# verdurin/pbdagcon

Measured on AMD Instinct MI355X. Metric: consensus bases/sec (whole node), higher is better.
Workload: dtype u8

## Files before the change

pbdagcon_amd/csrc/dagcon_api.hip:

```cpp
#include <hip/hip_runtime.h>
#include <algorithm>
#include <cstdarg>
#include <cstdio>
#include <cstdlib>
#include <cstring>
#include <string>
#include <chrono>
#include <array>
#include <vector>

#include "../../include/dagcon.h"
#include "dagcon_dev.h"
#include "k_build.hip.h"
#include "k_merge.hip.h"
#include "k_merge_q.hip.h"
#include "k_bestpath.hip.h"
#include "k_align.hip.h"
#include "k_align_panels.hip.h"
#include "k_place.hip.h"
#include "k_cigar.hip.h"
#include "k_rate.hip.h"
#include "k_cs.hip.h"

namespace {

struct DevBuf {
    void *p = nullptr;
    size_t cap = 0;
};

struct CigarBufs {
    DevBuf ops, op_begin, tile_begin, totals, ckpt;
    DevBuf q, t, q_off, t_base;
    DevBuf out_off;
    DevBuf piece, cut, wave_piece, wave_begin, piece_out;
    DevBuf rev, q_len;
    DevBuf rate_base, tile_rate, rate;
    std::array<DevBuf *, 20> all() {
        return {&ops, &op_begin, &tile_begin, &totals, &ckpt, &q, &t, &q_off, &t_base, &out_off, &piece, &cut, &wave_piece, &wave_begin, &piece_out, &rev, &q_len,
                &rate_base, &tile_rate, &rate};
    }
};
static_assert(sizeof(CigarBufs) == 20 * sizeof(DevBuf), "CigarBufs::all() must name every member");
struct CsBufs {
    DevBuf text, cs_off, cs_len, totals, n_ops, op_begin, t_base, t_room, q_off, q_len;
    std::array<DevBuf *, 10> all() { return {&text, &cs_off, &cs_len, &totals, &n_ops, &op_begin, &t_base, &t_room, &q_off, &q_len}; }
};
static_assert(sizeof(CsBufs) == 10 * sizeof(DevBuf), "CsBufs::all() must name every member");

#define DQ_KMAX 52u
struct DgPlanIn { uint32_t T; uint64_t n_alns, sum_bb; uint32_t gcuts, max_segments, min_segment_len, seg_env, merge_q; };
struct DgPlan { uint32_t seg_max, seg_min, use_q, bp_max; };
static DgPlan dg_plan_pieces(const DgPlanIn &in) {
    DgPlan pl;
    const uint32_t T = in.T;
    pl.seg_min = in.min_segment_len;
    if (!pl.seg_min) pl.seg_min = (uint32_t)std::min<uint64_t>(768, std::max<uint64_t>(192, in.sum_bb / 8192));
    if (in.max_segments) pl.seg_max = in.max_segments > 64u ? 64u : in.max_segments;
    else if (in.seg_env) pl.seg_max = in.seg_env;
    else if (in.gcuts) pl.seg_max = 64;
    else { uint32_t sm = T ? 8192u / T : 8u; pl.seg_max = sm < 8u ? 8u : sm > 256u ? 256u : sm; }
    if (in.gcuts && !in.min_segment_len) pl.seg_min = 256;
    pl.use_q = 0;
    if (in.merge_q && !in.gcuts && pl.seg_max != 1) {
        const uint32_t slots = 1024u * DQ_WAVES;
        if (in.max_segments || in.seg_env) pl.use_q = 1;
        else if (T && in.n_alns <= (uint64_t)DQ_KMAX * T) {
            const uint64_t avail = std::min<uint64_t>(256, std::max<uint64_t>(1, in.sum_bb / T / 128));
            const uint64_t k = (uint64_t)T * avail / DQ_ROWS / slots;
            if (k >= 1 || (uint64_t)T * avail / DQ_ROWS * 10u >= 6u * slots) {
                const uint64_t sm = std::min<uint64_t>(avail, std::max<uint64_t>(k, 1) * slots * DQ_ROWS / T);
                if (sm >= 2) { pl.seg_max = (uint32_t)sm; pl.use_q = 1; }
            }
        }
    }
    if (pl.seg_max < 1) pl.seg_max = 1;
    if (pl.use_q && !in.min_segment_len) pl.seg_min = 128;
    pl.bp_max = pl.seg_max == 1 ? 1u : std::min(in.gcuts || T >= 256u ? 64u : (uint32_t)DG_BP_PIECES, 3u * pl.seg_max);
    if (pl.bp_max < 1) pl.bp_max = 1;
    return pl;
}

struct Ctx {
    dagcon_opts opts;
    int device = 0;
    hipStream_t stream = nullptr;
    hipEvent_t ev[5] = {nullptr, nullptr, nullptr, nullptr, nullptr};
    std::string err;
    bool uploaded = false, ran = false, fetched = false;

    uint32_t T = 0, A = 0;
    int bp_lane = 1, bl_stk = -1;
    uint32_t align_dropped = 0;
    uint32_t align_n = 0;
    std::vector<uint32_t> h_ends;
    int poison = 0;
    int fold = 1;
    int merge_q = 1, use_q = 0;
    uint32_t max_k = 0, max_tlen = 0;
    uint64_t sum_len = 0, sum_bb = 0, mat_cells = 0, blob_bytes = 0;
    bool have_bb = false;
    std::vector<uint32_t> h_tlen, h_aln_len, h_aln_start, h_aln_tgt;
    std::vector<uint64_t> h_aln_begin, h_aln_off, h_mat_base, h_bbv_base, h_bb_off, h_matc_base;
    std::vector<uint32_t> h_matc_stride;
    uint64_t matc_cells = 0;
    std::vector<uint8_t> h_tactive;
    std::vector<uint32_t> h_ch_base, h_ch_aln;
    std::vector<uint64_t> h_norm_off;
    std::vector<uint32_t> h_ck_base;
    uint64_t n_ckpt = 0;
    uint32_t emit_shift = 9;
    uint32_t n_chunks = 0;
    uint64_t tmp_main = 0, tmp_cap = 0;

    DevBuf d_tfail, d_q, d_t, d_aln_off, d_aln_len, d_aln_start, d_aln_tgt, d_tlen, d_aln_begin, d_tactive,
        d_bb, d_bb_off, d_mat_base, d_bbv_base, d_matc_base, d_matc_stride;
    DevBuf d_nmis, d_norm_off, d_n_lo, d_n_hi, d_n_start, d_n_ins, d_n_del, d_norm;
    DevBuf d_ch_aln, d_ch_base, d_ch_k0, d_ch_next, d_ch_w, d_ch_tb, d_ch_flag, d_ch_src, d_ch_out, d_ch_adv,
        d_n_lb, d_norm_tmp, d_ckpt, d_ck_base;
    DevBuf d_node_base, d_n_nodes, d_pool_base, d_pool_size, d_pool_top, d_t_nins;
    DevBuf d_matA, d_matD, d_matC, d_cov, d_gcount, d_gbase, d_bid;
    DevBuf d_nodes, d_best, d_queue, d_score, d_cns_tmp, d_bp_tt, d_score_b;
    DevBuf d_pool, d_stk, d_cuts, d_cuts_bp, d_bp_stat, d_bp_len, d_worklist, d_rd, d_pro_state, d_sh_cnt, d_seg_done, d_wl_first, d_queue0, d_bp_end, d_bp_ab, d_defer, d_cns_tmp0;
    DevBuf d_al[15];
    DevBuf d_pn[18];
    DevBuf d_pl[14];
    CsBufs cs;
    CigarBufs cg;
    std::vector<uint8_t> h_cig_bad;
    std::string cig_err;
    bool filter_on = false;
    dagcon_record_filter filter = {1000000u, 0u};
    bool rs_valid = false;
    std::vector<uint32_t> rs_match, rs_mismatch, rs_ins, rs_del;
    std::vector<uint8_t> rs_fate;
    DevBuf d_cns, d_cns_off, d_cns_len, d_seg_first, d_n_seg, d_seg_r0, d_seg_r1, d_st;
    DevBuf d_pos_tmp, d_pos_tmp0, d_pos;
    DevBuf d_sup_tmp, d_sup_tmp0, d_sup;

    uint64_t norm_cap = 0, node_cap = 0, pool_cap = 0, cns_cap = 0, seg_cap = 0;
    uint32_t stk_words = 4096, growth_pct = 100, seg_max = 8, bp_max = 16, seg_env = 0, seg_min = 768;
    uint32_t sh_log = 16;
    bool full_span = false;
    uint32_t gcuts = 1;
    uint32_t worklist_cap = 0, list_grid = 8192;

    DgStatus h_st;
    dagcon_timings tm;

    std::vector<uint64_t> r_seg_begin, r_seq_off, r_cns_off, r_seg_first;
    std::vector<int32_t> r_range0, r_range1, r_tmp0, r_tmp1;
    std::vector<uint32_t> r_seq_len, r_cns_len, r_n_seg, r_tfail;
    std::vector<int32_t> r_status;
    char *r_blob = nullptr;
    size_t r_blob_cap = 0;
    uint16_t *r_sup = nullptr;
    size_t r_sup_cap = 0;
    uint64_t r_sup_n = 0;
    std::vector<uint32_t> r_pos;
    bool pos_valid = false;
    bool sup_valid = false;

    std::vector<uint8_t> g_base, g_deleted, g_backbone;
    std::vector<int32_t> g_weight, g_cov, g_bbpos, g_out_dst, g_out_cnt, g_in_src;
    std::vector<uint32_t> g_out_begin, g_in_begin;
};

int fail(Ctx *c, int code, const char *fmt, ...) {
    char buf[512];
    va_list ap;
    va_start(ap, fmt);
    vsnprintf(buf, sizeof buf, fmt, ap);
    va_end(ap);
    if (c) c->err = buf;
    return code;
}

#define HIPCHK(c, call)                                                                    \
    do {                                                                                   \
        hipError_t _e = (call);                                                            \
        if (_e != hipSuccess)                                                              \
            return fail((c), DAGCON_ERR_HIP, "%s failed: %s (%s:%d)", #call,               \
                        hipGetErrorString(_e), __FILE__, __LINE__);                        \
    } while (0)

int ensure(Ctx *c, DevBuf &b, size_t bytes) {
    if (bytes == 0) bytes = 16;
    if (b.cap >= bytes) return DAGCON_OK;
    if (b.p) { (void)hipFree(b.p); b.p = nullptr; b.cap = 0; }
    size_t want = bytes + bytes / 16 + 256;
    const bool dbg = getenv("DAGCON_ALLOC_TIMING") != nullptr;
    const double t0 = dbg ? std::chrono::duration<double>(std::chrono::steady_clock::now().time_since_epoch()).count() : 0;
    hipError_t e = hipMalloc(&b.p, want);
    if (dbg) {
        const double dt = std::chrono::duration<double>(std::chrono::steady_clock::now().time_since_epoch()).count() - t0;
        if (dt > 0.005) fprintf(stderr, "dagcon: hipMalloc(%.1f MB) took %.1f ms\n", want / 1e6, dt * 1e3);
    }
    if (e != hipSuccess) {
        b.p = nullptr;
        return fail(c, DAGCON_ERR_WORKSPACE, "hipMalloc(%zu bytes) failed: %s", want, hipGetErrorString(e));
    }
    b.cap = want;
    return DAGCON_OK;
}

#define ENSURE(c, buf, bytes)                                \
    do {                                                     \
        int _r = ensure((c), (buf), (size_t)(bytes));        \
        if (_r != DAGCON_OK) return _r;                      \
    } while (0)

template <typename T>
int upload_vec(Ctx *c, DevBuf &b, const std::vector<T> &v) {
    ENSURE(c, b, v.size() * sizeof(T));
    if (!v.empty()) HIPCHK(c, hipMemcpyAsync(b.p, v.data(), v.size() * sizeof(T), hipMemcpyHostToDevice, c->stream));
    return DAGCON_OK;
}

void free_buf(DevBuf &b) {
    if (b.p) (void)hipFree(b.p);
    b.p = nullptr; b.cap = 0;
}

int ensure_arenas(Ctx *c) {
    ENSURE(c, c->d_norm, c->norm_cap * sizeof(uint16_t));
    ENSURE(c, c->d_nodes, c->node_cap * sizeof(DgNode));
    ENSURE(c, c->d_best, c->node_cap * 4);
    ENSURE(c, c->d_queue, c->node_cap * 4);
    ENSURE(c, c->d_score, c->node_cap * 8);
    ENSURE(c, c->d_bp_tt, c->node_cap * 4);
    if (c->gcuts) ENSURE(c, c->d_score_b, c->node_cap * 4);
    ENSURE(c, c->d_cns_tmp, c->node_cap);
    ENSURE(c, c->d_pool, c->pool_cap * 4);
    ENSURE(c, c->d_stk, std::max<uint64_t>((uint64_t)c->T * std::max(c->bp_max, c->seg_max), c->gcuts ? c->list_grid : 0) * c->stk_words * 4);
    if (c->gcuts) {
        ENSURE(c, c->d_worklist, (4ull + 3ull * c->worklist_cap) * 4);
        ENSURE(c, c->d_rd, (uint64_t)c->A * 16 + 16);
        ENSURE(c, c->d_pro_state, (uint64_t)c->T * 16 + 16);
        ENSURE(c, c->d_sh_cnt, (uint64_t)c->T * (2 + 2 * DG_SH_MAX) * 4 + 16);
        ENSURE(c, c->d_seg_done, (uint64_t)c->worklist_cap * (DG_SH_MAX + 1) * 4 + 16);
        ENSURE(c, c->d_wl_first, (uint64_t)c->T * 4 + 16);
        ENSURE(c, c->d_queue0, c->node_cap * 4);
        ENSURE(c, c->d_bp_end, (uint64_t)c->T * c->bp_max * 4 + 16);
        ENSURE(c, c->d_bp_ab, (uint64_t)c->T * c->bp_max * 16 + 16);
        ENSURE(c, c->d_defer, (uint64_t)c->T * (DG_DEFER_MAX + 1) * 4 + 16);
        ENSURE(c, c->d_cns_tmp0, c->node_cap);
    }
    ENSURE(c, c->d_cuts, (uint64_t)c->T * (c->seg_max + 2) * 4);
    ENSURE(c, c->d_cuts_bp, (uint64_t)c->T * (c->bp_max + 2) * 4);
    ENSURE(c, c->d_bp_stat, (uint64_t)c->T * c->bp_max * 8);
    ENSURE(c, c->d_bp_len, (uint64_t)c->T * c->bp_max * 4);
    ENSURE(c, c->d_cns, c->cns_cap);
    if (c->opts.flags & DAGCON_FLAG_BASE_SUPPORT) {
        ENSURE(c, c->d_sup_tmp, c->node_cap * 4);
        if (c->gcuts) ENSURE(c, c->d_sup_tmp0, c->node_cap * 4);
        ENSURE(c, c->d_sup, c->cns_cap * 4);
    }
    if (c->opts.flags & DAGCON_FLAG_BASE_POS) {
        ENSURE(c, c->d_pos_tmp, c->node_cap * 4);
        if (c->gcuts) ENSURE(c, c->d_pos_tmp0, c->node_cap * 4);
        ENSURE(c, c->d_pos, c->cns_cap * 4);
    }
    ENSURE(c, c->d_seg_r0, c->seg_cap * 4);
    ENSURE(c, c->d_seg_r1, c->seg_cap * 4);
    return DAGCON_OK;
}

void fill_params(Ctx *c, DgParams &p) {
    memset(&p, 0, sizeof p);
    p.q = (const uint8_t *)c->d_q.p; p.t = (const uint8_t *)c->d_t.p;
    p.aln_off = (const uint64_t *)c->d_aln_off.p;
    p.aln_len = (const uint32_t *)c->d_aln_len.p;
    p.aln_start = (const uint32_t *)c->d_aln_start.p;
    p.aln_tgt = (const uint32_t *)c->d_aln_tgt.p;
    p.tlen = (const uint32_t *)c->d_tlen.p;
    p.aln_begin = (const uint64_t *)c->d_aln_begin.p;
    p.tactive = (const uint8_t *)c->d_tactive.p; p.tfail = (uint32_t *)c->d_tfail.p;
    p.bb = c->have_bb ? (const uint8_t *)c->d_bb.p : nullptr;
    p.bb_off = (const uint64_t *)c->d_bb_off.p;
    p.mat_base = (const uint64_t *)c->d_mat_base.p;
    p.matc_base = (const uint64_t *)c->d_matc_base.p; p.matc_stride = (const uint32_t *)c->d_matc_stride.p;
    p.bbv_base = (const uint64_t *)c->d_bbv_base.p;
    p.T = c->T; p.A = c->A;
    p.trim = c->opts.trim; p.min_len = c->opts.min_len;
    p.min_weight = c->opts.min_weight < 0 ? (int32_t)c->opts.min_cov : c->opts.min_weight;
    p.flags = c->opts.flags;
    p.max_k = c->max_k; p.max_tlen = c->max_tlen;
    p.nmis = (uint32_t *)c->d_nmis.p; p.norm_off = (uint64_t *)c->d_norm_off.p;
    p.n_lo = (uint32_t *)c->d_n_lo.p; p.n_hi = (uint32_t *)c->d_n_hi.p;
    p.n_start = (uint32_t *)c->d_n_start.p; p.n_ins = (uint32_t *)c->d_n_ins.p;
    p.n_del = (uint32_t *)c->d_n_del.p;
    p.norm = (uint16_t *)c->d_norm.p; p.norm_cap = c->norm_cap;
    p.ch_aln = (const uint32_t *)c->d_ch_aln.p; p.ch_base = (const uint32_t *)c->d_ch_base.p;
    p.n_chunks = c->n_chunks;
    p.ch_k0 = (uint32_t *)c->d_ch_k0.p; p.ch_next = (uint32_t *)c->d_ch_next.p;
    p.ch_w = (uint32_t *)c->d_ch_w.p; p.ch_tb = (uint32_t *)c->d_ch_tb.p;
    p.ch_flag = (uint32_t *)c->d_ch_flag.p; p.ch_src = (uint64_t *)c->d_ch_src.p;
    p.ch_out = (uint32_t *)c->d_ch_out.p; p.ch_adv = (uint32_t *)c->d_ch_adv.p;
    p.n_lb = (uint32_t *)c->d_n_lb.p; p.norm_tmp = (uint16_t *)c->d_norm_tmp.p;
    p.tmp_main = c->tmp_main; p.tmp_cap = c->tmp_cap;
    p.ckpt = (uint32_t *)c->d_ckpt.p; p.ck_base = (const uint32_t *)c->d_ck_base.p; p.emit_shift = c->emit_shift;
    p.node_base = (uint64_t *)c->d_node_base.p; p.n_nodes = (uint32_t *)c->d_n_nodes.p;
    p.pool_base = (uint64_t *)c->d_pool_base.p; p.pool_size = (uint32_t *)c->d_pool_size.p;
    p.pool_top = (uint32_t *)c->d_pool_top.p; p.t_nins = (uint32_t *)c->d_t_nins.p;
    p.matA = (uint32_t *)c->d_matA.p; p.matD = (uint32_t *)c->d_matD.p; p.matC = (uint32_t *)c->d_matC.p;
    p.cov = (int32_t *)c->d_cov.p; p.gcount = (uint32_t *)c->d_gcount.p;
    p.gbase = (uint32_t *)c->d_gbase.p; p.bid = (uint32_t *)c->d_bid.p;
    p.nodes = (DgNode *)c->d_nodes.p; p.best = (int32_t *)c->d_best.p;
    p.queue = (int32_t *)c->d_queue.p; p.score = (float2 *)c->d_score.p; p.bp_tt = (float *)c->d_bp_tt.p;
    p.cns_tmp = (uint8_t *)c->d_cns_tmp.p; p.node_cap = c->node_cap;
    p.pool = (uint32_t *)c->d_pool.p; p.pool_cap = c->pool_cap;
    p.stk = (int32_t *)c->d_stk.p; p.stk_words = c->stk_words; p.growth_pct = c->growth_pct;
    p.score_b = (float *)c->d_score_b.p;
    p.bp_lane = c->bp_lane >= 2 || (c->bp_lane && (uint64_t)c->T * c->bp_max >= 32768ull) ? 1u : 0u; p.bl_stk = c->bl_stk >= 0 && c->bl_stk < DG_BL_STK ? (uint32_t)c->bl_stk : (uint32_t)DG_BL_STK;
    p.emit_scan = c->max_k <= 64u ? 1u : 0u;
    p.fold = (c->fold && !(c->opts.flags & DAGCON_FLAG_STOP_AFTER_BUILD)) ? 1u : 0u;
    p.q_kmax = c->use_q && !c->opts.max_segments && !c->seg_env && c->max_k > DQ_KMAX ? DQ_KMAX : 0u;
    p.bp_seg_min = (c->seg_min + 2u) / 3u;
    p.seg_max = c->seg_max; p.seg_min = c->seg_min; p.cuts = (uint32_t *)c->d_cuts.p; p.bp_max = c->bp_max; p.cuts_bp = (uint32_t *)c->d_cuts_bp.p; p.bp_stat = (float *)c->d_bp_stat.p; p.bp_len = (uint32_t *)c->d_bp_len.p;
    p.gcuts = c->gcuts; p.sh_log = c->sh_log;
    p.rd_s = (uint32_t *)c->d_rd.p; p.rd_e = p.rd_s + c->A; p.rd_lead = p.rd_e + c->A; p.rd_trail = p.rd_lead + c->A;
    p.pro_state = (uint32_t *)c->d_pro_state.p; p.sh_cnt = (uint32_t *)c->d_sh_cnt.p;
    p.queue0 = (int32_t *)c->d_queue0.p; p.bp_end = (uint32_t *)c->d_bp_end.p; p.bp_ab = (float *)c->d_bp_ab.p;
    p.defer = (uint32_t *)c->d_defer.p; p.cns_tmp0 = (uint8_t *)c->d_cns_tmp0.p;
    p.seg_done = (uint32_t *)c->d_seg_done.p; p.wl_first = (uint32_t *)c->d_wl_first.p;
    p.worklist = (uint32_t *)c->d_worklist.p; p.worklist_cap = c->worklist_cap;
    p.cns = (uint8_t *)c->d_cns.p; p.cns_cap = c->cns_cap;
    p.cns_off = (uint64_t *)c->d_cns_off.p; p.cns_len = (uint32_t *)c->d_cns_len.p;
    p.seg_first = (uint64_t *)c->d_seg_first.p; p.n_seg = (uint32_t *)c->d_n_seg.p;
    p.seg_r0 = (int32_t *)c->d_seg_r0.p; p.seg_r1 = (int32_t *)c->d_seg_r1.p;
    p.seg_cap = c->seg_cap;
    p.st = (DgStatus *)c->d_st.p;
    if (c->opts.flags & DAGCON_FLAG_BASE_SUPPORT) {
        p.sup_tmp = (uint32_t *)c->d_sup_tmp.p; p.sup_tmp0 = (uint32_t *)c->d_sup_tmp0.p;
        p.sup_w = (uint16_t *)c->d_sup.p; p.sup_d = p.sup_w + c->cns_cap;
    }
    if (c->opts.flags & DAGCON_FLAG_BASE_POS) {
        p.pos_tmp = (uint32_t *)c->d_pos_tmp.p; p.pos_tmp0 = (uint32_t *)c->d_pos_tmp0.p; p.pos_out = (uint32_t *)c->d_pos.p;
    }
}

void launch_normalize(Ctx *c, const DgParams &p) {
    hipStream_t s = c->stream;
    if (c->A == 0) return;
    (void)hipMemsetAsync(c->d_ckpt.p, 0xFF, c->n_ckpt * 4, s);
    hipLaunchKernelGGL((k_norm_chunk<DG_NW, 64, false>), dim3((c->n_chunks + 63) / 64), dim3(64), 0, s, p);
    hipLaunchKernelGGL((k_norm_chunk<DG_NW_BIG, 32, true>), dim3((c->n_chunks + 31) / 32), dim3(32), 0, s, p);
    hipLaunchKernelGGL(k_norm_scan, dim3((c->A + 63) / 64), dim3(64), 0, s, p);
    hipLaunchKernelGGL(k_norm_finish2, dim3((c->n_chunks + 3) / 4), dim3(256), 0, s, p);
    hipLaunchKernelGGL(k_normalize_slow, dim3((c->A + 63) / 64), dim3(64), 0, s, p);
}

int launch_all(Ctx *c) {
    int r = ensure_arenas(c);
    if (r != DAGCON_OK) return r;
    DgParams p;
    fill_params(c, p);
    hipStream_t s = c->stream;
    if (c->poison & 8) {
        DevBuf *work[] = {&c->d_nmis, &c->d_n_lo, &c->d_n_hi, &c->d_n_start, &c->d_n_ins, &c->d_n_del, &c->d_ch_k0, &c->d_ch_next, &c->d_ch_w,
                          &c->d_ch_tb, &c->d_ch_flag, &c->d_ch_src, &c->d_ch_out, &c->d_ch_adv, &c->d_n_lb, &c->d_norm_tmp, &c->d_ckpt,
                          &c->d_node_base, &c->d_n_nodes, &c->d_pool_base, &c->d_pool_size, &c->d_pool_top, &c->d_t_nins, &c->d_cov, &c->d_gcount,
                          &c->d_gbase, &c->d_bid, &c->d_best, &c->d_queue, &c->d_score, &c->d_cns_tmp, &c->d_bp_tt, &c->d_stk, &c->d_cuts,
                          &c->d_cuts_bp, &c->d_bp_stat, &c->d_bp_len, &c->d_rd, &c->d_pro_state, &c->d_sh_cnt, &c->d_wl_first,
                          &c->d_queue0, &c->d_bp_end, &c->d_bp_ab, &c->d_defer, &c->d_cns_tmp0, &c->d_cns, &c->d_cns_off, &c->d_seg_first,
                          &c->d_seg_r0, &c->d_seg_r1, &c->d_worklist, &c->d_seg_done, &c->d_sup_tmp, &c->d_sup_tmp0, &c->d_sup, &c->d_pos_tmp, &c->d_pos_tmp0, &c->d_pos};
        for (DevBuf *b : work)
            if (b->p && b->cap) HIPCHK(c, hipMemsetAsync(b->p, 0xEE, b->cap, s));
    }
    HIPCHK(c, hipMemsetAsync(c->d_st.p, 0, sizeof(DgStatus), s));
    HIPCHK(c, hipMemsetAsync(c->d_tfail.p, 0, (size_t)c->T * 4 + 4, s));
    HIPCHK(c, hipMemsetAsync(c->d_cns_len.p, 0, (size_t)c->T * 4, s));
    HIPCHK(c, hipMemsetAsync(c->d_n_seg.p, 0, (size_t)c->T * 4, s));
    if (c->matc_cells) HIPCHK(c, hipMemsetAsync(c->d_matC.p, 0, c->matc_cells * 4, s));
    if (c->poison) {
        if ((c->poison & 1) && c->d_matA.p) { HIPCHK(c, hipMemsetAsync(c->d_matA.p, 0xEE, c->d_matA.cap, s)); HIPCHK(c, hipMemsetAsync(c->d_matD.p, 0xEE, c->d_matD.cap, s)); }
        if ((c->poison & 2) && c->d_nodes.p) { HIPCHK(c, hipMemsetAsync(c->d_nodes.p, 0xEE, c->d_nodes.cap, s)); HIPCHK(c, hipMemsetAsync(c->d_pool.p, 0xEE, c->d_pool.cap, s)); }
        if ((c->poison & 4) && c->d_score_b.p) HIPCHK(c, hipMemsetAsync(c->d_score_b.p, 0xEE, c->d_score_b.cap, s));
        if ((c->poison & 4) && c->d_norm.p) HIPCHK(c, hipMemsetAsync(c->d_norm.p, 0xEE, c->d_norm.cap, s));
    }
    HIPCHK(c, hipEventRecord(c->ev[0], s));
    launch_normalize(c, p);
    HIPCHK(c, hipEventRecord(c->ev[1], s));
    hipLaunchKernelGGL(k_carve, dim3(1), dim3(1024), 0, s, p);
    if (c->T > 0) {
        const uint32_t rows4 = (c->max_tlen + 2 + 4 * DG_LPW - 1) / (4 * DG_LPW);
        if (c->gcuts && c->A > 0) hipLaunchKernelGGL(k_readspan, dim3((c->A + 63) / 64), dim3(64), 0, s, p);
        if (p.emit_scan) hipLaunchKernelGGL(k_gsum, dim3(c->T, (c->max_tlen + 2 + 255) / 256), dim3(256), 0, s, p);
        else hipLaunchKernelGGL(k_groups, dim3(c->T, (c->max_tlen + 2 + 31) / 32), dim3(256), 0, s, p);
        hipLaunchKernelGGL(k_gscan, dim3(c->T), dim3(1024), 0, s, p);
        if (c->A > 0)
            hipLaunchKernelGGL(k_emit, dim3(c->T, (c->max_k + DG_ERPW - 1) / DG_ERPW, ((c->max_tlen + 2) >> c->emit_shift) + 1),
                               dim3(64), 0, s, p);
        const size_t lds = (size_t)4 * 2 * (c->max_k + 2) * sizeof(int32_t);
        if (lds > 65536)
            HIPCHK(c, hipFuncSetAttribute((const void *)k_lists, hipFuncAttributeMaxDynamicSharedMemorySize, (int)lds));
        hipLaunchKernelGGL(k_lists, dim3(c->T, rows4), dim3(256), lds, s, p);
    }
    HIPCHK(c, hipEventRecord(c->ev[2], s));
    if (c->T > 0 && !(c->opts.flags & DAGCON_FLAG_STOP_AFTER_BUILD)) {
        if (c->gcuts) {
            HIPCHK(c, hipMemsetAsync(c->d_worklist.p, 0, 16, s));
            HIPCHK(c, hipMemsetAsync(c->d_seg_done.p, 0, (size_t)c->worklist_cap * (DG_SH_MAX + 1) * 4, s));
            hipLaunchKernelGGL(k_merge_pro, dim3(c->T), dim3(64), 0, s, p);
            hipLaunchKernelGGL(k_cuts2, dim3(c->T), dim3(64), 0, s, p);
            hipLaunchKernelGGL(k_merge_list, dim3(c->list_grid), dim3(64), 0, s, p);
            hipLaunchKernelGGL(k_merge_fin, dim3(c->T), dim3(64), 0, s, p);
        } else {
            hipLaunchKernelGGL(k_cuts, dim3(c->T), dim3(64), 0, s, p);
            if (c->use_q) {
                hipLaunchKernelGGL(k_merge_q, dim3((c->T * c->seg_max + DQ_ROWS - 1u) / DQ_ROWS), dim3(64), 0, s, p);
                if (p.q_kmax) hipLaunchKernelGGL(k_merge, dim3(c->T * c->seg_max), dim3(64), 0, s, p);
            } else hipLaunchKernelGGL(k_merge, dim3(c->T * c->seg_max), dim3(64), 0, s, p);
        }
    }
    HIPCHK(c, hipEventRecord(c->ev[3], s));
    if (c->T > 0 && !(c->opts.flags & (DAGCON_FLAG_STOP_AFTER_BUILD | DAGCON_FLAG_STOP_AFTER_MERGE))) {
        const bool sup = (c->opts.flags & DAGCON_FLAG_BASE_SUPPORT) != 0;
        const bool pos = (c->opts.flags & DAGCON_FLAG_BASE_POS) != 0;
#define DG_BP_LAUNCH(K, GRID)                                                                          \
        do {                                                                                           \
            if (sup && pos) hipLaunchKernelGGL((K<true, true>), GRID, dim3(64), 0, s, p);              \
            else if (sup) hipLaunchKernelGGL((K<true, false>), GRID, dim3(64), 0, s, p);               \
            else if (pos) hipLaunchKernelGGL((K<false, true>), GRID, dim3(64), 0, s, p);               \
            else hipLaunchKernelGGL((K<false, false>), GRID, dim3(64), 0, s, p);                       \
        } while (0)
        hipLaunchKernelGGL(k_bp_terms, dim3(c->T, 16), dim3(256), 0, s, p);
        if (c->gcuts) {
            hipLaunchKernelGGL(k_bp_xtree, dim3(c->T), dim3(64), 0, s, p);
            hipLaunchKernelGGL(k_bp_sweep_ab, dim3(c->T * c->bp_max), dim3(64), 0, s, p);
            hipLaunchKernelGGL(k_bp_comb, dim3(c->T), dim3(64), 0, s, p);
            hipLaunchKernelGGL(k_bp_abs, dim3(c->T * c->bp_max), dim3(256), 0, s, p);
            hipLaunchKernelGGL(k_bp_choose, dim3(c->T * c->bp_max), dim3(256), 0, s, p);
            hipLaunchKernelGGL(k_bp_sweep_abs_g, dim3(c->T * c->bp_max), dim3(64), 0, s, p);
            hipLaunchKernelGGL(k_bp_defer, dim3(c->T), dim3(64), 0, s, p);
            DG_BP_LAUNCH(k_bp_walk_g, dim3(c->T * c->bp_max));
        } else {
            if (p.bp_lane) hipLaunchKernelGGL(k_bp_sweep_l, dim3((c->T * c->bp_max + 7u) / 8u), dim3(64), 0, s, p);
            hipLaunchKernelGGL(k_bp_sweep, dim3(c->T * c->bp_max), dim3(64), 0, s, p);
            hipLaunchKernelGGL(k_bp_check, dim3(c->T), dim3(64), 0, s, p);
            if (p.bp_lane) DG_BP_LAUNCH(k_bp_walk_r, dim3((c->T * c->bp_max + 7u) / 8u));
            else DG_BP_LAUNCH(k_bp_walk, dim3(c->T * c->bp_max));
        }
        DG_BP_LAUNCH(k_bp_join, dim3(c->T));
#undef DG_BP_LAUNCH
    }
    HIPCHK(c, hipEventRecord(c->ev[4], s));
    HIPCHK(c, hipGetLastError());
    return DAGCON_OK;
}

}

extern "C" {

int dagcon_abi_version(void) { return DAGCON_ABI_VERSION; }

void dagcon_default_opts(dagcon_opts *o) {
    if (!o) return;
    memset(o, 0, sizeof *o);
    o->min_cov = 6; o->min_len = 500; o->trim = 50; o->min_weight = -1; o->device = 0; o->flags = 0;
}

const char *dagcon_last_error(const dagcon_ctx *ctx) {
    return ctx ? reinterpret_cast<const Ctx *>(ctx)->err.c_str() : "null context";
}

int dagcon_create(const dagcon_opts *opts, dagcon_ctx **out) {
    if (!opts || !out) return DAGCON_ERR_INVALID_ARG;
    *out = nullptr;
    int ndev = 0;
    if (hipGetDeviceCount(&ndev) != hipSuccess || ndev <= 0) return DAGCON_ERR_NO_DEVICE;
    if (opts->device < 0 || opts->device >= ndev) return DAGCON_ERR_NO_DEVICE;
    if (opts->flags & ~DAGCON_FLAGS_ALL) return DAGCON_ERR_UNSUPPORTED;
    {
        hipDeviceProp_t prop;
        if (hipGetDeviceProperties(&prop, opts->device) != hipSuccess || strncmp(prop.gcnArchName, "gfx950", 6) != 0)
            return DAGCON_ERR_NO_DEVICE;
    }
    Ctx *c = new Ctx();
    c->opts = *opts;
    c->device = opts->device;
    if (const char *e = getenv("DAGCON_EMIT_SHIFT")) {
        const int v = atoi(e);
        if (v >= 4 && v <= 20) c->emit_shift = (uint32_t)v;
    }
    if (const char *e = getenv("DAGCON_MERGE_SEGS")) {
        const int v = atoi(e);
        if (v >= 1 && v <= 64) c->seg_env = (uint32_t)v;
    }
    if (const char *e = getenv("DAGCON_FOLD")) c->fold = atoi(e) != 0;
    if (const char *e = getenv("DAGCON_POISON")) c->poison = atoi(e);
    if (const char *e = getenv("DAGCON_BP_LANE")) c->bp_lane = atoi(e);
    if (const char *e = getenv("DAGCON_BP_LANE_STACK")) c->bl_stk = atoi(e);
    if (const char *e = getenv("DAGCON_MERGE_Q")) c->merge_q = atoi(e) != 0;
    memset(&c->tm, 0, sizeof c->tm);
    memset(&c->h_st, 0, sizeof c->h_st);
    if (hipSetDevice(c->device) != hipSuccess || hipStreamCreateWithFlags(&c->stream, hipStreamNonBlocking) != hipSuccess) {
        delete c;
        return DAGCON_ERR_NO_DEVICE;
    }
    for (auto &e : c->ev)
        if (hipEventCreate(&e) != hipSuccess) { delete c; return DAGCON_ERR_HIP; }
    if (ensure(c, c->d_st, sizeof(DgStatus)) != DAGCON_OK) { delete c; return DAGCON_ERR_WORKSPACE; }
    *out = reinterpret_cast<dagcon_ctx *>(c);
    return DAGCON_OK;
}

void dagcon_destroy(dagcon_ctx *ctx) {
    if (!ctx) return;
    Ctx *c = reinterpret_cast<Ctx *>(ctx);
    (void)hipSetDevice(c->device);
    if (c->stream) (void)hipStreamSynchronize(c->stream);
    if (c->r_blob) (void)hipHostFree(c->r_blob);
    if (c->r_sup) (void)hipHostFree(c->r_sup);
    DevBuf *all[] = {&c->d_q, &c->d_t, &c->d_aln_off, &c->d_aln_len, &c->d_aln_start, &c->d_aln_tgt,
                     &c->d_tlen, &c->d_aln_begin, &c->d_tactive, &c->d_tfail, &c->d_bb, &c->d_bb_off, &c->d_mat_base, &c->d_matc_base, &c->d_matc_stride,
                     &c->d_bbv_base, &c->d_nmis, &c->d_norm_off, &c->d_n_lo, &c->d_n_hi, &c->d_n_start, &c->d_ch_aln, &c->d_ch_base, &c->d_ch_k0, &c->d_ch_next, &c->d_ch_w, &c->d_ch_tb, &c->d_ch_flag, &c->d_ch_src, &c->d_ch_out, &c->d_ch_adv, &c->d_n_lb, &c->d_norm_tmp, &c->d_ckpt, &c->d_ck_base,
                     &c->d_n_ins, &c->d_n_del, &c->d_norm, &c->d_node_base, &c->d_n_nodes,
                     &c->d_pool_base, &c->d_pool_size, &c->d_pool_top, &c->d_t_nins, &c->d_matA, &c->d_matD,
                     &c->d_matC, &c->d_cov, &c->d_gcount, &c->d_gbase, &c->d_bid, &c->d_nodes,
                     &c->d_best, &c->d_queue, &c->d_score, &c->d_cns_tmp, &c->d_bp_tt, &c->d_score_b, &c->d_pool, &c->d_stk, &c->d_cuts, &c->d_cuts_bp, &c->d_bp_stat, &c->d_bp_len, &c->d_worklist, &c->d_rd, &c->d_pro_state, &c->d_sh_cnt, &c->d_seg_done, &c->d_wl_first, &c->d_queue0, &c->d_bp_end, &c->d_bp_ab, &c->d_defer, &c->d_cns_tmp0, &c->d_cns,
                     &c->d_cns_off, &c->d_cns_len, &c->d_seg_first, &c->d_n_seg, &c->d_seg_r0, &c->d_seg_r1,
                     &c->d_st, &c->d_sup_tmp, &c->d_sup_tmp0, &c->d_sup, &c->d_pos_tmp, &c->d_pos_tmp0, &c->d_pos};
    for (DevBuf *b : all) free_buf(*b);
    for (DevBuf &b : c->d_al) free_buf(b);
    for (DevBuf &b : c->d_pn) free_buf(b);
    for (DevBuf &b : c->d_pl) free_buf(b);
    for (DevBuf *b : c->cg.all()) free_buf(*b);
    for (DevBuf *b : c->cs.all()) free_buf(*b);
    for (auto &e : c->ev) if (e) (void)hipEventDestroy(e);
    if (c->stream) (void)hipStreamDestroy(c->stream);
    delete c;
}

static int upload_impl(dagcon_ctx *ctx, const dagcon_batch *b, const void *dev_q, const void *dev_t) {
    if (!ctx || !b) return DAGCON_ERR_INVALID_ARG;
    Ctx *c = reinterpret_cast<Ctx *>(ctx);
    c->uploaded = c->ran = c->fetched = false;
    c->sup_valid = c->pos_valid = false;
    c->h_cig_bad.clear();
    c->rs_valid = false;
    const uint32_t T = b->n_targets;
    if (T && (!b->tlen || !b->aln_begin)) return fail(c, DAGCON_ERR_INVALID_ARG, "tlen/aln_begin is NULL");
    const uint64_t A_all = T ? b->aln_begin[T] : 0;
    if (A_all && (!b->aln_start || !b->aln_off || !b->aln_len || ((!b->qstr || !b->tstr) && !(dev_q && dev_t))))
        return fail(c, DAGCON_ERR_INVALID_ARG, "alignment arrays are NULL");
    if (b->backbone && !b->backbone_off) return fail(c, DAGCON_ERR_INVALID_ARG, "backbone_off is NULL");
    HIPCHK(c, hipSetDevice(c->device));

    c->T = T;
    c->h_tlen.assign(b->tlen, b->tlen + T);
    c->h_aln_begin.assign(T + 1, 0);
    c->h_tactive.assign(T, 0);
    c->h_mat_base.assign(T, 0);
    c->h_matc_base.assign(T, 0); c->h_matc_stride.assign(T, 0); c->matc_cells = 0;
    c->h_bbv_base.assign(T, 0);
    c->h_bb_off.assign(T, 0);
    c->h_aln_len.clear(); c->h_aln_start.clear(); c->h_aln_tgt.clear(); c->h_aln_off.clear();
    c->max_k = 0; c->max_tlen = 0; c->sum_len = 0; c->sum_bb = 0; c->mat_cells = 0;
    c->have_bb = b->backbone != nullptr;
    uint64_t bb_bytes = 0, n_whole = 0;
    const uint64_t min_cov = c->opts.min_cov;
    for (uint32_t t = 0; t < T; t++) {
        const uint64_t ab = b->aln_begin[t], ae = b->aln_begin[t + 1];
        if (ae < ab) return fail(c, DAGCON_ERR_INVALID_ARG, "aln_begin not monotone at target %u", t);
        const uint64_t k_all = ae - ab;
        const bool active = k_all > 0 && k_all >= min_cov;
        c->h_aln_begin[t] = c->h_aln_len.size();
        if (!active) continue;
        if (b->tlen[t] > 0x3FFFFFFFu) return fail(c, DAGCON_ERR_UNSUPPORTED, "tlen of target %u too large", t);
        c->h_tactive[t] = 1;
        for (uint64_t a = ab; a < ae; a++) {
            const uint32_t len = b->aln_len[a];
            if (b->aln_off[a] > b->blob_bytes || len > b->blob_bytes - b->aln_off[a])
                return fail(c, DAGCON_ERR_INVALID_ARG, "alignment %llu runs past the blob", (unsigned long long)a);
            if (len < c->opts.min_len) continue;
            c->h_aln_len.push_back(len);
            c->h_aln_start.push_back(b->aln_start[a]);
            c->h_aln_off.push_back(b->aln_off[a]);
            c->h_aln_tgt.push_back(t);
            c->sum_len += len;
            n_whole += len >= b->tlen[t] && b->aln_start[a] == 1u;
        }
        const uint64_t k = c->h_aln_len.size() - c->h_aln_begin[t];
        if (k > DAGCON_MAX_COVERAGE)
            return fail(c, DAGCON_ERR_UNSUPPORTED, "target %u has %llu alignments (max %u)", t,
                        (unsigned long long)k, DAGCON_MAX_COVERAGE);
        c->max_k = std::max<uint32_t>(c->max_k, (uint32_t)k);
        c->max_tlen = std::max(c->max_tlen, b->tlen[t]);
        if ((uint64_t)b->tlen[t] + 2 > 4ull * 65535ull)
            return fail(c, DAGCON_ERR_UNSUPPORTED, "tlen of target %u exceeds %u", t, 4u * 65535u - 2u);
        c->h_mat_base[t] = c->mat_cells;
        c->mat_cells += ((uint64_t)b->tlen[t] + 2) * k;
        c->h_matc_stride[t] = (b->tlen[t] + 2 + 7) & ~7u;
        c->h_matc_base[t] = c->matc_cells;
        c->matc_cells += (uint64_t)c->h_matc_stride[t] * k;
        c->h_bbv_base[t] = c->sum_bb;
        c->sum_bb += ((uint64_t)b->tlen[t] + 2 + 3) & ~3ull;
        if (c->have_bb) {
            c->h_bb_off[t] = b->backbone_off[t];
            bb_bytes = std::max<uint64_t>(bb_bytes, b->backbone_off[t] + b->tlen[t]);
        }
    }
    c->full_span = n_whole == (uint64_t)c->h_aln_len.size();
    c->gcuts = c->full_span ? 0u : 1u;
    if (const char *e = getenv("DAGCON_GCUTS")) c->gcuts = atoi(e) ? 1u : 0u;
    {
        DgPlanIn pi;
        pi.T = T; pi.n_alns = c->h_aln_len.size(); pi.sum_bb = c->sum_bb; pi.gcuts = c->gcuts;
        pi.max_segments = c->opts.max_segments; pi.min_segment_len = c->opts.min_segment_len;
        pi.seg_env = c->seg_env; pi.merge_q = c->merge_q ? 1u : 0u;
        const DgPlan pl = dg_plan_pieces(pi);
        c->seg_max = pl.seg_max; c->seg_min = pl.seg_min; c->use_q = (int)pl.use_q; c->bp_max = pl.bp_max;
    }
    if (const char *e = getenv("DAGCON_BP_SEGS")) { const int v = atoi(e); if (v >= 1 && v <= 64) c->bp_max = (uint32_t)v; }
    {
        const uint64_t pieces = std::max<uint64_t>(1, (uint64_t)T * std::max(c->bp_max, c->seg_max));
        const uint32_t fit = (uint32_t)std::min<uint64_t>(4096, (512ull << 20) / pieces);
        const uint32_t base = std::max(256u, fit);
        if (c->stk_words < base || (uint64_t)c->stk_words * pieces > (1024ull << 20)) c->stk_words = base;
    }
    if (c->gcuts) c->worklist_cap = std::max<uint32_t>(c->worklist_cap, (uint32_t)std::min<uint64_t>((uint64_t)T * c->seg_max + 64, 0x0FFFFFFFull));
    c->h_aln_begin[T] = c->h_aln_len.size();
    if (c->h_aln_len.size() > 0xFFFFFFF0ull) return fail(c, DAGCON_ERR_UNSUPPORTED, "too many alignments");
    c->A = (uint32_t)c->h_aln_len.size();
    c->blob_bytes = b->blob_bytes;
    c->h_ch_base.assign((size_t)c->A + 1, 0);
    c->h_ch_aln.clear();
    for (uint32_t a = 0; a < c->A; a++) {
        const uint32_t nw = std::max<uint32_t>(1u, (c->h_aln_len[a] + DG_NCH - 1) / DG_NCH);
        c->h_ch_base[a] = (uint32_t)c->h_ch_aln.size();
        if (c->h_ch_aln.size() + nw > 0xFFFFFFF0ull) return fail(c, DAGCON_ERR_UNSUPPORTED, "too many alignment columns");
        c->h_ch_aln.insert(c->h_ch_aln.end(), nw, a);
    }
    c->h_norm_off.assign((size_t)c->A, 0);
    {
        uint64_t top = 0;
        for (uint32_t a = 0; a < c->A; a++) { c->h_norm_off[a] = top; top += (2ull * c->h_aln_len[a] + 7ull) & ~7ull; }
        c->norm_cap = std::max<uint64_t>(c->norm_cap, top + 64);
    }
    c->h_ck_base.assign((size_t)c->A, 0);
    c->n_ckpt = 0;
    for (uint32_t a = 0; a < c->A; a++) {
        c->h_ck_base[a] = (uint32_t)c->n_ckpt;
        c->n_ckpt += (((uint64_t)c->h_tlen[c->h_aln_tgt[a]] + 2) >> c->emit_shift) + 1;
        if (c->n_ckpt > 0xFFFFFFF0ull) return fail(c, DAGCON_ERR_UNSUPPORTED, "too many alignment columns");
    }
    c->h_ch_base[c->A] = (uint32_t)c->h_ch_aln.size();
    c->n_chunks = (uint32_t)c->h_ch_aln.size();
    c->tmp_main = (2ull * b->blob_bytes + 8ull * c->n_chunks + 15ull) & ~7ull;
    c->tmp_cap = c->tmp_main + std::max<uint64_t>(c->tmp_main / 16, 1ull << 20);

    ENSURE(c, c->d_q, b->blob_bytes);
    ENSURE(c, c->d_t, b->blob_bytes);
    if (b->blob_bytes && !(dev_q == c->d_q.p && dev_t == c->d_t.p)) {
        HIPCHK(c, hipMemcpyAsync(c->d_q.p, dev_q ? dev_q : b->qstr, b->blob_bytes, dev_q ? hipMemcpyDeviceToDevice : hipMemcpyHostToDevice, c->stream));
        HIPCHK(c, hipMemcpyAsync(c->d_t.p, dev_t ? dev_t : b->tstr, b->blob_bytes, dev_t ? hipMemcpyDeviceToDevice : hipMemcpyHostToDevice, c->stream));
    }
    if (c->have_bb) {
        ENSURE(c, c->d_bb, bb_bytes);
        if (bb_bytes) HIPCHK(c, hipMemcpyAsync(c->d_bb.p, b->backbone, bb_bytes, hipMemcpyHostToDevice, c->stream));
    }
    int r;
    if ((r = upload_vec(c, c->d_aln_off, c->h_aln_off))) return r;
    if ((r = upload_vec(c, c->d_aln_len, c->h_aln_len))) return r;
    if ((r = upload_vec(c, c->d_aln_start, c->h_aln_start))) return r;
    if ((r = upload_vec(c, c->d_aln_tgt, c->h_aln_tgt))) return r;
    if ((r = upload_vec(c, c->d_tlen, c->h_tlen))) return r;
    if ((r = upload_vec(c, c->d_aln_begin, c->h_aln_begin))) return r;
    if ((r = upload_vec(c, c->d_tactive, c->h_tactive))) return r;
    if ((r = upload_vec(c, c->d_bb_off, c->h_bb_off))) return r;
    if ((r = upload_vec(c, c->d_mat_base, c->h_mat_base))) return r;
    if ((r = upload_vec(c, c->d_matc_base, c->h_matc_base))) return r;
    if ((r = upload_vec(c, c->d_matc_stride, c->h_matc_stride))) return r;
    if ((r = upload_vec(c, c->d_bbv_base, c->h_bbv_base))) return r;
    if ((r = upload_vec(c, c->d_ch_base, c->h_ch_base))) return r;
    if ((r = upload_vec(c, c->d_ch_aln, c->h_ch_aln))) return r;
    if ((r = upload_vec(c, c->d_ck_base, c->h_ck_base))) return r;
    if ((r = upload_vec(c, c->d_norm_off, c->h_norm_off))) return r;
    ENSURE(c, c->d_ckpt, c->n_ckpt * 4);

    const size_t A4 = (size_t)c->A * 4, T4 = (size_t)T * 4;
    ENSURE(c, c->d_nmis, A4);
    ENSURE(c, c->d_n_lo, A4); ENSURE(c, c->d_n_hi, A4); ENSURE(c, c->d_n_start, A4);
    ENSURE(c, c->d_n_ins, A4); ENSURE(c, c->d_n_del, A4); ENSURE(c, c->d_n_lb, A4);
    {
        const size_t C4 = (size_t)c->n_chunks * 4;
        ENSURE(c, c->d_ch_k0, C4); ENSURE(c, c->d_ch_next, C4); ENSURE(c, c->d_ch_w, C4); ENSURE(c, c->d_ch_tb, C4);
        ENSURE(c, c->d_ch_flag, C4); ENSURE(c, c->d_ch_src, 2 * C4); ENSURE(c, c->d_ch_out, C4); ENSURE(c, c->d_ch_adv, C4);
        ENSURE(c, c->d_norm_tmp, c->tmp_cap * sizeof(uint16_t));
    }
    ENSURE(c, c->d_node_base, (size_t)T * 8); ENSURE(c, c->d_n_nodes, T4);
    ENSURE(c, c->d_pool_base, (size_t)T * 8); ENSURE(c, c->d_pool_size, T4); ENSURE(c, c->d_pool_top, T4);
    ENSURE(c, c->d_t_nins, T4); ENSURE(c, c->d_tfail, T4 + 4);
    ENSURE(c, c->d_matA, c->mat_cells * 4); ENSURE(c, c->d_matD, c->mat_cells * 4);
    ENSURE(c, c->d_matC, c->matc_cells * 4 + 256);
    ENSURE(c, c->d_cov, c->sum_bb * 4); ENSURE(c, c->d_gcount, c->sum_bb * 4);
    ENSURE(c, c->d_gbase, c->sum_bb * 4); ENSURE(c, c->d_bid, c->sum_bb * 4);
    ENSURE(c, c->d_cns_off, (size_t)T * 8); ENSURE(c, c->d_cns_len, T4);
    ENSURE(c, c->d_seg_first, (size_t)T * 8); ENSURE(c, c->d_n_seg, T4);

    c->node_cap = std::max<uint64_t>(c->node_cap, c->sum_bb + c->sum_len / 7 + 1024);
    c->pool_cap = std::max<uint64_t>(c->pool_cap, 8ull * c->node_cap + 80ull * c->sum_bb + 1024ull * T);
    c->cns_cap = std::max<uint64_t>(c->cns_cap, c->sum_bb + c->sum_bb / 4 + 1024);
    c->seg_cap = std::max<uint64_t>(c->seg_cap, (uint64_t)T * 4 + 1024);
    if ((r = ensure_arenas(c))) return r;
    HIPCHK(c, hipStreamSynchronize(c->stream));
    c->uploaded = true;
    c->tm.reruns = 0;
    return DAGCON_OK;
}

int dagcon_upload(dagcon_ctx *ctx, const dagcon_batch *b) { return upload_impl(ctx, b, nullptr, nullptr); }

int dagcon_run(dagcon_ctx *ctx) {
    if (!ctx) return DAGCON_ERR_INVALID_ARG;
    Ctx *c = reinterpret_cast<Ctx *>(ctx);
    if (!c->uploaded) return fail(c, DAGCON_ERR_STATE, "dagcon_run before dagcon_upload");
    HIPCHK(c, hipSetDevice(c->device));
    int r = launch_all(c);
    if (r != DAGCON_OK) return r;
    c->ran = true; c->fetched = false;
    if (const char *e = getenv("DAGCON_DUMP")) {
        const uint32_t t = (uint32_t)atoi(e);
        const char *path = strchr(e, ':');
        if (path && t < c->T) {
            HIPCHK(c, hipStreamSynchronize(c->stream));
            uint64_t nb = 0, pb = 0;
            uint32_t hdr[4] = {0, c->bp_max, 0, c->seg_max};
            (void)hipMemcpy(&nb, (uint64_t *)c->d_node_base.p + t, 8, hipMemcpyDeviceToHost);
            (void)hipMemcpy(&pb, (uint64_t *)c->d_pool_base.p + t, 8, hipMemcpyDeviceToHost);
            (void)hipMemcpy(&hdr[0], (uint32_t *)c->d_n_nodes.p + t, 4, hipMemcpyDeviceToHost);
            (void)hipMemcpy(&hdr[2], (uint32_t *)c->d_pool_top.p + t, 4, hipMemcpyDeviceToHost);
            std::vector<uint32_t> cuts(c->bp_max + 2), pool(hdr[2]), best(hdr[0]);
            std::vector<DgNode> nd(hdr[0]);
            std::vector<float> sc(2 * (size_t)hdr[0]);
            (void)hipMemcpy(cuts.data(), (uint32_t *)c->d_cuts_bp.p + (uint64_t)t * (c->bp_max + 2), cuts.size() * 4, hipMemcpyDeviceToHost);
            (void)hipMemcpy(nd.data(), (DgNode *)c->d_nodes.p + nb, nd.size() * sizeof(DgNode), hipMemcpyDeviceToHost);
            (void)hipMemcpy(pool.data(), (uint32_t *)c->d_pool.p + pb, pool.size() * 4, hipMemcpyDeviceToHost);
            (void)hipMemcpy(sc.data(), (float *)c->d_score.p + 2 * nb, sc.size() * 4, hipMemcpyDeviceToHost);
            (void)hipMemcpy(best.data(), (uint32_t *)c->d_best.p + nb, best.size() * 4, hipMemcpyDeviceToHost);
            if (FILE *f = fopen(path + 1, "wb")) {
                fwrite(hdr, 4, 4, f); fwrite(cuts.data(), 4, cuts.size(), f); fwrite(nd.data(), sizeof(DgNode), nd.size(), f);
                fwrite(pool.data(), 4, pool.size(), f); fwrite(sc.data(), 4, sc.size(), f); fwrite(best.data(), 4, best.size(), f);
                uint32_t nl = 0;
                std::vector<uint32_t> wl;
                if (c->gcuts && c->d_worklist.p) {
                    (void)hipMemcpy(&nl, c->d_worklist.p, 4, hipMemcpyDeviceToHost);
                    if (nl > c->worklist_cap) nl = c->worklist_cap;
                    wl.resize(3 * (size_t)nl);
                    if (nl) (void)hipMemcpy(wl.data(), (uint32_t *)c->d_worklist.p + 4, wl.size() * 4, hipMemcpyDeviceToHost);
                }
                fwrite(&nl, 4, 1, f);
                if (nl) fwrite(wl.data(), 4, wl.size(), f);
                fclose(f);
            }
        }
    }
    return DAGCON_OK;
}

int dagcon_sync(dagcon_ctx *ctx) {
    if (!ctx) return DAGCON_ERR_INVALID_ARG;
    Ctx *c = reinterpret_cast<Ctx *>(ctx);
    HIPCHK(c, hipSetDevice(c->device));
    HIPCHK(c, hipStreamSynchronize(c->stream));
    return DAGCON_OK;
}

static hipError_t d2h(Ctx *c, void *dst, const void *src, size_t bytes) {
    hipError_t e = hipMemcpyAsync(dst, src, bytes, hipMemcpyDeviceToHost, c->stream);
    return e != hipSuccess ? e : hipStreamSynchronize(c->stream);
}

static int read_status(Ctx *c) {
    HIPCHK(c, hipStreamSynchronize(c->stream));
    HIPCHK(c, d2h(c, &c->h_st, c->d_st.p, sizeof(DgStatus)));
    return DAGCON_OK;
}

int dagcon_fetch(dagcon_ctx *ctx, dagcon_results *res) {
    if (!ctx || !res) return DAGCON_ERR_INVALID_ARG;
    Ctx *c = reinterpret_cast<Ctx *>(ctx);
    if (!c->ran) return fail(c, DAGCON_ERR_STATE, "dagcon_fetch before dagcon_run");
    HIPCHK(c, hipSetDevice(c->device));
    int r;
    for (int attempt = 0;; attempt++) {
        if ((r = read_status(c))) return r;
        const uint32_t f = c->h_st.err_flags;
        if (f == 0) break;
        if (f & DG_E_TARGET_MASK)
            return fail(c, DAGCON_ERR_INTERNAL, "unexpected batch-level flag 0x%x", f);
        if (attempt >= 6) return fail(c, DAGCON_ERR_WORKSPACE, "workspace still too small after %d re-runs (flags 0x%x)", attempt, f);
        if (f & DG_E_NORM_OVF) c->norm_cap = c->h_st.norm_top + 1024;
        if (f & DG_E_NODE_OVF) c->node_cap = c->h_st.node_need + 1024;
        if (f & DG_E_POOL_OVF) c->pool_cap = c->h_st.pool_need + 1024;
        if (f & DG_E_POOL_TGT) c->growth_pct *= 3;
        if (f & DG_E_STACK) c->stk_words *= 4;
        if (f & DG_E_LIST_OVF) c->worklist_cap *= 4;
        if (f & DG_E_LOG_OVF) c->sh_log *= 2;
        if (f & DG_E_OUT_OVF) {
            c->cns_cap = std::max<uint64_t>(c->cns_cap, c->h_st.cns_top + 1024);
            c->seg_cap = std::max<uint64_t>(c->seg_cap, c->h_st.seg_top + 1024);
        }
        c->tm.reruns++;
        if ((r = launch_all(c))) return r;
    }
    float ms = 0;
    HIPCHK(c, hipEventElapsedTime(&ms, c->ev[0], c->ev[4])); c->tm.ms_total = ms;
    HIPCHK(c, hipEventElapsedTime(&ms, c->ev[0], c->ev[1])); c->tm.ms_normalize = ms;
    HIPCHK(c, hipEventElapsedTime(&ms, c->ev[1], c->ev[2])); c->tm.ms_build = ms;
    HIPCHK(c, hipEventElapsedTime(&ms, c->ev[2], c->ev[3])); c->tm.ms_merge = ms;
    HIPCHK(c, hipEventElapsedTime(&ms, c->ev[3], c->ev[4])); c->tm.ms_bestpath = ms;

    const uint32_t T = c->T;
    c->r_tfail.assign(T, 0); c->r_status.assign(T, DAGCON_OK);
    if (T) HIPCHK(c, d2h(c, c->r_tfail.data(), c->d_tfail.p, (size_t)T * 4));
    uint32_t n_failed = 0;
    c->err.clear();
    for (uint32_t t = 0; t < T; t++) {
        const uint32_t f = c->r_tfail[t];
        if (!f) continue;
        const int code = (f & (DG_E_BADCHAR | DG_E_NONCONF)) ? DAGCON_ERR_NONCONFORMING
                       : (f & DG_E_TOO_BIG) ? DAGCON_ERR_UNSUPPORTED : DAGCON_ERR_INTERNAL;
        c->r_status[t] = code;
        if (!n_failed++) {
            if (f & DG_E_BADCHAR) fail(c, code, "target %u: an alignment holds a byte outside printable ASCII", t);
            else if (f & DG_E_NONCONF) fail(c, code, "target %u: an alignment (after the min_len filter) leaves the backbone: start < 1 or target bases past tlen", t);
            else if (f & DG_E_TOO_BIG) fail(c, code, "target %u too large (more than 2^25 - 3 vertices or 2^30 pool words)", t);
            else fail(c, code, "device invariant violated in target %u", t);
        }
    }
    for (uint32_t t = 0; t < T && !c->h_cig_bad.empty(); t++) {
        if (!c->h_cig_bad[t] || c->r_status[t] != DAGCON_OK) continue;
        c->r_status[t] = DAGCON_ERR_NONCONFORMING;
        if (!n_failed++) c->err = c->cig_err;
    }
    const uint64_t nseg = c->h_st.seg_top, nb = c->h_st.cns_top;
    c->r_cns_off.assign(T, 0); c->r_cns_len.assign(T, 0); c->r_seg_first.assign(T, 0); c->r_n_seg.assign(T, 0);
    c->r_tmp0.assign(nseg, 0); c->r_tmp1.assign(nseg, 0);
    if (c->r_blob_cap < nb + 1) {
        if (c->r_blob) (void)hipHostFree(c->r_blob);
        c->r_blob = nullptr; c->r_blob_cap = 0;
        const size_t want = (size_t)(nb + 1) + (size_t)(nb / 8) + 4096;
        HIPCHK(c, hipHostMalloc((void **)&c->r_blob, want, hipHostMallocDefault));
        c->r_blob_cap = want;
    }
    c->r_blob[nb] = 0;
    const bool full = !(c->opts.flags & (DAGCON_FLAG_STOP_AFTER_BUILD | DAGCON_FLAG_STOP_AFTER_MERGE));
    if (T && full) {
        HIPCHK(c, d2h(c, c->r_cns_off.data(), c->d_cns_off.p, (size_t)T * 8));
        HIPCHK(c, d2h(c, c->r_cns_len.data(), c->d_cns_len.p, (size_t)T * 4));
        HIPCHK(c, d2h(c, c->r_seg_first.data(), c->d_seg_first.p, (size_t)T * 8));
        HIPCHK(c, d2h(c, c->r_n_seg.data(), c->d_n_seg.p, (size_t)T * 4));
        if (nseg) {
            HIPCHK(c, d2h(c, c->r_tmp0.data(), c->d_seg_r0.p, nseg * 4));
            HIPCHK(c, d2h(c, c->r_tmp1.data(), c->d_seg_r1.p, nseg * 4));
        }
        if (nb) HIPCHK(c, d2h(c, c->r_blob, c->d_cns.p, nb));
    }
    c->sup_valid = c->pos_valid = false;
    if (full && (c->opts.flags & DAGCON_FLAG_BASE_SUPPORT)) {
        if (c->r_sup_cap < nb + 1) {
            if (c->r_sup) (void)hipHostFree(c->r_sup);
            c->r_sup = nullptr; c->r_sup_cap = 0;
            const size_t want = (size_t)(nb + 1) + (size_t)(nb / 8) + 4096;
            HIPCHK(c, hipHostMalloc((void **)&c->r_sup, want * 4, hipHostMallocDefault));
            c->r_sup_cap = want;
        }
        if (nb) {
            HIPCHK(c, hipMemcpyAsync(c->r_sup, c->d_sup.p, nb * 2, hipMemcpyDeviceToHost, c->stream));
            HIPCHK(c, d2h(c, c->r_sup + nb, (const uint16_t *)c->d_sup.p + c->cns_cap, nb * 2));
        }
        c->r_sup_n = nb;
        c->sup_valid = true;
    }
    if (full && (c->opts.flags & DAGCON_FLAG_BASE_POS)) {
        c->r_pos.resize(nb + 1);
        if (nb) HIPCHK(c, d2h(c, c->r_pos.data(), c->d_pos.p, nb * 4));
        c->pos_valid = true;
    }
    c->r_seg_begin.assign(T + 1, 0);
    c->r_range0.clear(); c->r_range1.clear(); c->r_seq_off.clear(); c->r_seq_len.clear();
    uint64_t bases = 0;
    for (uint32_t t = 0; t < T; t++) {
        c->r_seg_begin[t] = c->r_range0.size();
        if (!full || !c->h_tactive[t] || c->r_tfail[t]) continue;
        for (uint32_t i = 0; i < c->r_n_seg[t]; i++) {
            const uint64_t s = c->r_seg_first[t] + i;
            const int32_t r0 = c->r_tmp0[s], r1 = c->r_tmp1[s];
            c->r_range0.push_back(r0); c->r_range1.push_back(r1);
            c->r_seq_off.push_back(c->r_cns_off[t] + (uint64_t)r0);
            c->r_seq_len.push_back((uint32_t)(r1 - r0));
            bases += (uint64_t)(r1 - r0);
        }
    }
    c->r_seg_begin[T] = c->r_range0.size();
    c->tm.consensus_bases = bases;
    c->tm.algorithmic_bytes = 2ull * c->sum_len + bases;
    c->tm.n_alignments = c->A;
    c->tm.n_columns = c->h_st.n_columns;
    c->tm.n_nodes = c->h_st.node_need;
    c->tm.merge_segments = c->h_st.n_mseg;
    res->n_targets = T;
    res->n_segments = c->r_range0.size();
    res->seg_begin = c->r_seg_begin.data();
    res->range0 = c->r_range0.data(); res->range1 = c->r_range1.data();
    res->seq_off = c->r_seq_off.data(); res->seq_len = c->r_seq_len.data();
    res->seq_blob = c->r_blob; res->seq_bytes = nb;
    res->target_status = c->r_status.data(); res->n_failed = n_failed;
    c->fetched = true;
    return DAGCON_OK;
}

int dagcon_fetch_support(dagcon_ctx *ctx, dagcon_support *out) {
    if (!ctx || !out) return DAGCON_ERR_INVALID_ARG;
    Ctx *c = reinterpret_cast<Ctx *>(ctx);
    if (!(c->opts.flags & DAGCON_FLAG_BASE_SUPPORT))
        return fail(c, DAGCON_ERR_STATE, "dagcon_fetch_support on a context created without DAGCON_FLAG_BASE_SUPPORT");
    if (!c->sup_valid)
        return fail(c, DAGCON_ERR_STATE, "dagcon_fetch_support without the results of a consensus (no fetch yet, or stopped before bestPath)");
    out->n = c->r_sup_n;
    out->weight = c->r_sup;
    out->depth = c->r_sup + c->r_sup_n;
    return DAGCON_OK;
}

int dagcon_fetch_positions(dagcon_ctx *ctx, const uint32_t **pos, uint64_t *n) {
    if (!ctx || !pos || !n) return DAGCON_ERR_INVALID_ARG;
    Ctx *c = reinterpret_cast<Ctx *>(ctx);
    if (!(c->opts.flags & DAGCON_FLAG_BASE_POS))
        return fail(c, DAGCON_ERR_STATE, "dagcon_fetch_positions on a context created without DAGCON_FLAG_BASE_POS");
    if (!c->pos_valid)
        return fail(c, DAGCON_ERR_STATE, "dagcon_fetch_positions without the results of a consensus (no fetch yet, or stopped before bestPath)");
    *pos = c->r_pos.data();
    *n = c->r_pos.size() - 1;
    return DAGCON_OK;
}

int dagcon_debug_counters(dagcon_ctx *ctx, unsigned long long *out8) {
    if (!ctx || !out8) return DAGCON_ERR_INVALID_ARG;
    Ctx *c = reinterpret_cast<Ctx *>(ctx);
    HIPCHK(c, hipSetDevice(c->device));
    HIPCHK(c, hipStreamSynchronize(c->stream));
    DgStatus st;
    HIPCHK(c, d2h(c, &st, c->d_st.p, sizeof st));
    for (int i = 0; i < 16; i++) out8[i] = st.dbg[i];
    return DAGCON_OK;
}

uint32_t dagcon_align_dropped(dagcon_ctx *ctx) {
    return ctx ? reinterpret_cast<Ctx *>(ctx)->align_dropped : 0u;
}

int dagcon_debug_plan(uint32_t n_targets, uint64_t n_alignments, uint64_t sum_positions, uint32_t partial_span,
                      uint32_t max_segments, uint32_t min_segment_len, uint32_t out4[4]) {
    if (!out4) return DAGCON_ERR_INVALID_ARG;
    DgPlanIn pi;
    pi.T = n_targets; pi.n_alns = n_alignments; pi.sum_bb = sum_positions; pi.gcuts = partial_span ? 1u : 0u;
    pi.max_segments = max_segments; pi.min_segment_len = min_segment_len; pi.seg_env = 0; pi.merge_q = 1;
    const DgPlan pl = dg_plan_pieces(pi);
    out4[0] = pl.seg_max; out4[1] = pl.seg_min; out4[2] = pl.use_q; out4[3] = pl.bp_max;
    return DAGCON_OK;
}

int dagcon_get_timings(dagcon_ctx *ctx, dagcon_timings *out) {
    if (!ctx || !out) return DAGCON_ERR_INVALID_ARG;
    Ctx *c = reinterpret_cast<Ctx *>(ctx);
    if (!c->ran) return fail(c, DAGCON_ERR_STATE, "no run to report");
    if (!c->fetched) {
        HIPCHK(c, hipSetDevice(c->device));
        HIPCHK(c, hipStreamSynchronize(c->stream));
        float ms = 0;
        HIPCHK(c, hipEventElapsedTime(&ms, c->ev[0], c->ev[4])); c->tm.ms_total = ms;
        HIPCHK(c, hipEventElapsedTime(&ms, c->ev[0], c->ev[1])); c->tm.ms_normalize = ms;
        HIPCHK(c, hipEventElapsedTime(&ms, c->ev[1], c->ev[2])); c->tm.ms_build = ms;
        HIPCHK(c, hipEventElapsedTime(&ms, c->ev[2], c->ev[3])); c->tm.ms_merge = ms;
        HIPCHK(c, hipEventElapsedTime(&ms, c->ev[3], c->ev[4])); c->tm.ms_bestpath = ms;
    }
    *out = c->tm;
    return DAGCON_OK;
}

int dagcon_consensus(dagcon_ctx *ctx, const dagcon_batch *batch, dagcon_results *results) {
    int r = dagcon_upload(ctx, batch);
    if (r != DAGCON_OK) return r;
    if ((r = dagcon_run(ctx)) != DAGCON_OK) return r;
    return dagcon_fetch(ctx, results);
}

static int normalize_impl(Ctx *c, dagcon_ctx *ctx, uint32_t n, const uint32_t *aln_start,
                          const uint64_t *aln_off, const uint32_t *aln_len, const char *qstr,
                          const char *tstr, uint64_t blob_bytes, const uint64_t *out_off, char *qout,
                          char *tout, uint32_t *out_len, uint32_t *out_start) {
    std::vector<uint32_t> tl(1, 0u);
    std::vector<uint64_t> ab = {0, n};
    dagcon_batch b;
    memset(&b, 0, sizeof b);
    b.n_targets = 1; b.tlen = tl.data(); b.aln_begin = ab.data();
    b.aln_start = aln_start; b.aln_off = aln_off; b.aln_len = aln_len;
    b.qstr = qstr; b.tstr = tstr; b.blob_bytes = blob_bytes;
    int r = dagcon_upload(ctx, &b);
    if (r != DAGCON_OK) return r;
    for (int attempt = 0;; attempt++) {
        DgParams p;
        fill_params(c, p);
        p.flags |= DG_F_A1_ONLY;
        HIPCHK(c, hipMemsetAsync(c->d_st.p, 0, sizeof(DgStatus), c->stream));
        HIPCHK(c, hipMemsetAsync(c->d_tfail.p, 0, (size_t)c->T * 4 + 4, c->stream));
        launch_normalize(c, p);
        HIPCHK(c, hipGetLastError());
        if ((r = read_status(c))) return r;
        if ((c->h_st.err_flags & DG_E_NORM_OVF) && attempt < 3) {
            c->norm_cap = c->h_st.norm_top + 1024;
            if ((r = ensure_arenas(c))) return r;
            continue;
        }
        break;
    }
    if (c->h_st.err_flags & DG_E_BADCHAR)
        return fail(c, DAGCON_ERR_NONCONFORMING, "alignment %u holds a byte outside printable ASCII", c->h_st.bad_aln);
    if (c->h_st.err_flags) return fail(c, DAGCON_ERR_INTERNAL, "normalize failed (flags 0x%x)", c->h_st.err_flags);
    std::vector<uint64_t> noff(n);
    std::vector<uint32_t> lo(n), hi(n), st(n);
    if (n) {
        HIPCHK(c, d2h(c, noff.data(), c->d_norm_off.p, (size_t)n * 8));
        HIPCHK(c, d2h(c, lo.data(), c->d_n_lo.p, (size_t)n * 4));
        HIPCHK(c, d2h(c, hi.data(), c->d_n_hi.p, (size_t)n * 4));
        HIPCHK(c, d2h(c, st.data(), c->d_n_start.p, (size_t)n * 4));
    }
    std::vector<uint16_t> cols;
    for (uint32_t a = 0; a < n; a++) {
        const uint32_t m = hi[a] - lo[a];
        cols.resize(m);
        if (m) HIPCHK(c, d2h(c, cols.data(), (const uint16_t *)c->d_norm.p + noff[a] + lo[a], (size_t)m * 2));
        for (uint32_t i = 0; i < m; i++) {
            qout[out_off[a] + i] = (char)(cols[i] & 0xff);
            tout[out_off[a] + i] = (char)(cols[i] >> 8);
        }
        out_len[a] = m;
        out_start[a] = st[a];
    }
    return DAGCON_OK;
}

int dagcon_normalize(dagcon_ctx *ctx, uint32_t n, const uint32_t *aln_start, const uint64_t *aln_off,
                     const uint32_t *aln_len, const char *qstr, const char *tstr, uint64_t blob_bytes,
                     uint32_t trim, uint32_t flags, const uint64_t *out_off, char *qout, char *tout,
                     uint32_t *out_len, uint32_t *out_start) {
    if (!ctx) return DAGCON_ERR_INVALID_ARG;
    Ctx *c = reinterpret_cast<Ctx *>(ctx);
    if (n && (!aln_start || !aln_off || !aln_len || !qstr || !tstr || !out_off || !qout || !tout || !out_len || !out_start))
        return fail(c, DAGCON_ERR_INVALID_ARG, "NULL argument");
    if (n > DAGCON_MAX_COVERAGE)
        return fail(c, DAGCON_ERR_UNSUPPORTED, "dagcon_normalize takes at most %u alignments per call", DAGCON_MAX_COVERAGE);
    const dagcon_opts saved = c->opts;
    c->opts.min_cov = 0; c->opts.min_len = 0; c->opts.trim = trim;
    c->opts.flags = flags & DAGCON_FLAG_RAW_ALIGNMENTS;
    const int r = normalize_impl(c, ctx, n, aln_start, aln_off, aln_len, qstr, tstr, blob_bytes, out_off,
                                 qout, tout, out_len, out_start);
    c->opts = saved;
    c->uploaded = false; c->ran = false;
    return r;
}

extern "C++" {
template <bool LOCAL>
static void launch_align_band(uint32_t cells, uint32_t nk, hipStream_t s, const DgAlignParams &ap) {
    switch (cells) {
        case 2: hipLaunchKernelGGL((k_align_band<2, LOCAL>), dim3(nk), dim3(64), 0, s, ap); break;
        case 4: hipLaunchKernelGGL((k_align_band<4, LOCAL>), dim3(nk), dim3(64), 0, s, ap); break;
        case 6: hipLaunchKernelGGL((k_align_band<6, LOCAL>), dim3(nk), dim3(64), 0, s, ap); break;
        case 8: hipLaunchKernelGGL((k_align_band<8, LOCAL>), dim3(nk), dim3(64), 0, s, ap); break;
        case 12: hipLaunchKernelGGL((k_align_band<12, LOCAL>), dim3(nk), dim3(64), 0, s, ap); break;
        default: hipLaunchKernelGGL((k_align_band<16, LOCAL>), dim3(nk), dim3(64), 0, s, ap); break;
    }
}
}

static int align_device(Ctx *c, uint32_t n, const uint64_t *q_off, const uint32_t *q_len,
                        const uint64_t *t_off, const uint32_t *t_len, const char *q_blob, uint64_t q_bytes,
                        const char *t_blob, uint64_t t_bytes, const uint64_t *out_off, uint32_t *aln_len, uint64_t *out_bytes_ret) {
    HIPCHK(c, hipSetDevice(c->device));
    const bool local = (c->opts.flags & DAGCON_FLAG_LOCAL_ALIGN) != 0;
    c->align_n = 0;
    uint64_t out_bytes = 0;
    std::vector<uint64_t> dir_off(n);
    for (uint32_t a = 0; a < n; a++) {
        if (q_off[a] > q_bytes || q_len[a] > q_bytes - q_off[a] || t_off[a] > t_bytes || t_len[a] > t_bytes - t_off[a])
            return fail(c, DAGCON_ERR_INVALID_ARG, "pair %u runs past its blob", a);
        if ((uint64_t)q_len[a] + t_len[a] > 0x7FFFFFF0ull) return fail(c, DAGCON_ERR_UNSUPPORTED, "pair %u too long", a);
        out_bytes = std::max<uint64_t>(out_bytes, out_off[a] + (uint64_t)q_len[a] + t_len[a]);
    }
    DevBuf &dq = c->d_al[0], &dt = c->d_al[1], &dqo = c->d_al[2], &dto = c->d_al[3], &dql = c->d_al[4], &dtl = c->d_al[5],
           &doo = c->d_al[6], &dqa = c->d_al[7], &dta = c->d_al[8], &dlen = c->d_al[9], &ddir = c->d_al[10], &ddo = c->d_al[11];
    ENSURE(c, dq, q_bytes); ENSURE(c, dt, t_bytes);
    ENSURE(c, dqo, (size_t)n * 8); ENSURE(c, dto, (size_t)n * 8); ENSURE(c, dql, (size_t)n * 4); ENSURE(c, dtl, (size_t)n * 4);
    ENSURE(c, doo, (size_t)n * 8); ENSURE(c, dqa, out_bytes); ENSURE(c, dta, out_bytes); ENSURE(c, dlen, (size_t)n * 4);
    ENSURE(c, ddo, (size_t)n * 8);
    DevBuf &dend = c->d_al[14];
    if (local) ENSURE(c, dend, (size_t)n * 16);
    hipStream_t s = c->stream;
    HIPCHK(c, hipMemcpyAsync(dq.p, q_blob, q_bytes, hipMemcpyHostToDevice, s));
    HIPCHK(c, hipMemcpyAsync(dt.p, t_blob, t_bytes, hipMemcpyHostToDevice, s));
    HIPCHK(c, hipMemcpyAsync(dqo.p, q_off, (size_t)n * 8, hipMemcpyHostToDevice, s));
    HIPCHK(c, hipMemcpyAsync(dto.p, t_off, (size_t)n * 8, hipMemcpyHostToDevice, s));
    HIPCHK(c, hipMemcpyAsync(dql.p, q_len, (size_t)n * 4, hipMemcpyHostToDevice, s));
    HIPCHK(c, hipMemcpyAsync(dtl.p, t_len, (size_t)n * 4, hipMemcpyHostToDevice, s));
    HIPCHK(c, hipMemcpyAsync(doo.p, out_off, (size_t)n * 8, hipMemcpyHostToDevice, s));
    uint64_t budget_rows = (6ull << 30) / 256ull;
    {
        size_t mfree = 0, mtotal = 0;
        if (hipMemGetInfo(&mfree, &mtotal) == hipSuccess) {
            const uint64_t have = (uint64_t)mfree + (uint64_t)ddir.cap;
            budget_rows = std::min<uint64_t>(16ull << 30, std::max<uint64_t>(1ull << 30, have / 4)) / 256ull;
        }
    }
    if (const char *e = getenv("DAGCON_ALIGN_GB")) { const long long v = atoll(e); if (v >= 1 && v <= 200) budget_rows = ((uint64_t)v << 30) / 256ull; }
    if (const char *e = getenv("DAGCON_ALIGN_ROWS")) { const long long v = atoll(e); if (v >= 1) budget_rows = (uint64_t)v; }
    const bool t_dbg = getenv("DAGCON_ALIGN_TIMING") != nullptr;
    if (t_dbg) HIPCHK(c, hipStreamSynchronize(s));
    double t_grp = std::chrono::duration<double>(std::chrono::steady_clock::now().time_since_epoch()).count();
    DevBuf &didx = c->d_al[12], &dhw = c->d_al[13];
    ENSURE(c, didx, (size_t)n * 4); ENSURE(c, dhw, (size_t)n * 4);
    std::vector<uint32_t> todo(n), halfw(n), order(n);
    for (uint32_t a = 0; a < n; a++) todo[a] = a;
    DgAlignParams ap;
    ap.q = (const uint8_t *)dq.p; ap.t = (const uint8_t *)dt.p;
    ap.q_off = (const uint64_t *)dqo.p; ap.t_off = (const uint64_t *)dto.p;
    ap.q_len = (const uint32_t *)dql.p; ap.t_len = (const uint32_t *)dtl.p;
    ap.out_off = (const uint64_t *)doo.p; ap.qaln = (uint8_t *)dqa.p; ap.taln = (uint8_t *)dta.p;
    ap.aln_len = (uint32_t *)dlen.p; ap.dir_off = (const uint64_t *)ddo.p; ap.halfw = (const uint32_t *)dhw.p;
    ap.ends = local ? (uint32_t *)dend.p : nullptr;
    {
        std::vector<uint32_t> ad, rest;
        for (uint32_t a = 0; a < n; a++) (dg_align_halfwidth_first(q_len[a], t_len[a]) > DG_AL_WA ? ad : rest).push_back(a);
        if (getenv("DAGCON_ALIGN_STATIC")) { rest.insert(rest.end(), ad.begin(), ad.end()); ad.clear(); }
        std::stable_sort(ad.begin(), ad.end(), [&](uint32_t x, uint32_t y) { return q_len[x] > q_len[y]; });
        uint64_t all_rows = 0;
        for (uint32_t a : ad) all_rows += dg_align_rows_adapt(q_len[a], t_len[a]);
        const uint64_t ngrp = std::max<uint64_t>(1, (all_rows + budget_rows - 1) / budget_rows);
        const uint64_t grp_rows = std::min<uint64_t>(budget_rows, all_rows / ngrp + 1 + (all_rows / ngrp) / 64);
        size_t first = 0;
        while (first < ad.size()) {
            uint64_t rows = 0;
            size_t cnt = 0;
            while (first + cnt < ad.size()) {
                const uint32_t a = ad[first + cnt];
                const uint64_t r = dg_align_rows_adapt(q_len[a], t_len[a]);
                if (cnt && rows + r > grp_rows) break;
                dir_off[a] = rows;
                rows += r; cnt++;
            }
            ENSURE(c, ddir, rows * 256ull);
            ap.dirs = (uint32_t *)ddir.p;
            HIPCHK(c, hipMemcpyAsync(ddo.p, dir_off.data(), (size_t)n * 8, hipMemcpyHostToDevice, s));
            HIPCHK(c, hipMemcpyAsync((uint32_t *)didx.p + first, ad.data() + first, cnt * 4, hipMemcpyHostToDevice, s));
            ap.idx = (const uint32_t *)didx.p + first; ap.n = (uint32_t)cnt; ap.first_pass = 1u;
            if (local) hipLaunchKernelGGL(k_align_adapt<true>, dim3((uint32_t)cnt), dim3(64), 0, s, ap);
            else hipLaunchKernelGGL(k_align_adapt<false>, dim3((uint32_t)cnt), dim3(64), 0, s, ap);
            HIPCHK(c, hipGetLastError());
            HIPCHK(c, hipStreamSynchronize(s));
            if (t_dbg) {
                const double now = std::chrono::duration<double>(std::chrono::steady_clock::now().time_since_epoch()).count();
                fprintf(stderr, "dagcon_align: following band, group of %zu pairs, %.1f MB of directions: %.2f ms\n", cnt, rows * 256.0 / 1e6, (now - t_grp) * 1e3);
                t_grp = now;
            }
            first += cnt;
        }
        if (!ad.empty()) {
            HIPCHK(c, d2h(c, aln_len, dlen.p, (size_t)n * 4));
            size_t back = 0;
            for (uint32_t a : ad) if (aln_len[a] == DG_AL_RETRY) { rest.push_back(a); back++; }
            if (t_dbg) fprintf(stderr, "dagcon_align: %zu of %zu pairs go on to the static bands\n", back, ad.size());
        }
        std::sort(rest.begin(), rest.end());
        todo.swap(rest);
    }
    for (int pass = 0; pass < 2 && !todo.empty(); pass++) {
        for (uint32_t a : todo) halfw[a] = pass == 0 ? dg_align_halfwidth_first(q_len[a], t_len[a]) : dg_align_halfwidth(q_len[a], t_len[a]);
        HIPCHK(c, hipMemcpyAsync(dhw.p, halfw.data(), (size_t)n * 4, hipMemcpyHostToDevice, s));
        static const uint32_t kinds[6] = {2, 4, 6, 8, 12, 16};
        size_t first = 0;
        while (first < todo.size()) {
            uint64_t rows = 0;
            size_t cnt = 0;
            while (first + cnt < todo.size()) {
                const uint32_t a = todo[first + cnt];
                const uint64_t r = dg_align_rows(q_len[a], t_len[a], dg_align_cells(halfw[a]));
                if (cnt && rows + r > budget_rows) break;
                dir_off[a] = rows;
                rows += r; cnt++;
            }
            ENSURE(c, ddir, rows * 256ull);
            ap.dirs = (uint32_t *)ddir.p;
            HIPCHK(c, hipMemcpyAsync(ddo.p, dir_off.data(), (size_t)n * 8, hipMemcpyHostToDevice, s));
            size_t fill = 0;
            for (int k = 0; k < 6; k++) {
                for (int fin = 0; fin < 2; fin++) {
                    const size_t k0 = fill;
                    for (size_t x = 0; x < cnt; x++) {
                        const uint32_t a = todo[first + x];
                        const bool is_final = pass == 1 || halfw[a] == dg_align_halfwidth(q_len[a], t_len[a]);
                        if (dg_align_cells(halfw[a]) == kinds[k] && (int)is_final == fin) order[first + fill++] = a;
                    }
                    const uint32_t nk = (uint32_t)(fill - k0);
                    if (!nk) continue;
                    std::stable_sort(order.begin() + first + k0, order.begin() + first + fill,
                                     [&](uint32_t x, uint32_t y) { return q_len[x] > q_len[y]; });
                    HIPCHK(c, hipMemcpyAsync((uint32_t *)didx.p + first + k0, order.data() + first + k0, (size_t)nk * 4, hipMemcpyHostToDevice, s));
                    ap.idx = (const uint32_t *)didx.p + first + k0; ap.n = nk; ap.first_pass = fin ? 0u : 1u;
                    if (local) launch_align_band<true>(kinds[k], nk, s, ap);
                    else launch_align_band<false>(kinds[k], nk, s, ap);
                    HIPCHK(c, hipGetLastError());
                }
            }
            HIPCHK(c, hipStreamSynchronize(s));
            if (t_dbg) {
                const double now = std::chrono::duration<double>(std::chrono::steady_clock::now().time_since_epoch()).count();
                fprintf(stderr, "dagcon_align: pass %d, group of %zu pairs, %.1f MB of directions: %.2f ms\n", pass, cnt, rows * 256.0 / 1e6, (now - t_grp) * 1e3);
                t_grp = now;
            }
            first += cnt;
        }
        if (pass == 0) {
            HIPCHK(c, d2h(c, aln_len, dlen.p, (size_t)n * 4));
            std::vector<uint32_t> again;
            for (uint32_t a : todo) if (aln_len[a] == DG_AL_RETRY) again.push_back(a);
            if (t_dbg) fprintf(stderr, "dagcon_align: %zu of %u pairs go to the full band\n", again.size(), n);
            todo.swap(again);
        }
    }
    HIPCHK(c, d2h(c, aln_len, dlen.p, (size_t)n * 4));
    uint32_t dropped = 0;
    for (uint32_t a = 0; a < n; a++) {
        if ((uint64_t)aln_len[a] > (uint64_t)q_len[a] + t_len[a]) return fail(c, DAGCON_ERR_INTERNAL, "pair %u: alignment longer than its room", a);
        dropped += aln_len[a] == 0 && (q_len[a] || t_len[a]);
    }
    c->h_ends.resize((size_t)n * 4);
    if (local) HIPCHK(c, d2h(c, c->h_ends.data(), dend.p, (size_t)n * 16));
    else
        for (uint32_t a = 0; a < n; a++) {
            const bool ok = aln_len[a] != 0;
            uint32_t *e = &c->h_ends[(size_t)a * 4];
            e[0] = 0; e[1] = ok ? q_len[a] : 0u; e[2] = 0; e[3] = ok ? t_len[a] : 0u;
        }
    c->align_n = n;
    c->align_dropped = dropped;
    *out_bytes_ret = out_bytes;
    return DAGCON_OK;
}

int dagcon_align(dagcon_ctx *ctx, uint32_t n, const uint64_t *q_off, const uint32_t *q_len,
                 const uint64_t *t_off, const uint32_t *t_len, const char *q_blob, uint64_t q_bytes,
                 const char *t_blob, uint64_t t_bytes, const uint64_t *out_off, char *qaln, char *taln,
                 uint32_t *aln_len) {
    if (!ctx) return DAGCON_ERR_INVALID_ARG;
    Ctx *c = reinterpret_cast<Ctx *>(ctx);
    c->align_n = 0;
    if (n == 0) return DAGCON_OK;
    if (!q_off || !q_len || !t_off || !t_len || !q_blob || !t_blob || !out_off || !qaln || !taln || !aln_len)
        return fail(c, DAGCON_ERR_INVALID_ARG, "NULL argument");
    uint64_t out_bytes = 0;
    int r = align_device(c, n, q_off, q_len, t_off, t_len, q_blob, q_bytes, t_blob, t_bytes, out_off, aln_len, &out_bytes);
    if (r != DAGCON_OK) return r;
    HIPCHK(c, d2h(c, qaln, c->d_al[7].p, out_bytes));
    HIPCHK(c, d2h(c, taln, c->d_al[8].p, out_bytes));
    return DAGCON_OK;
}

int dagcon_align_ends(dagcon_ctx *ctx, uint32_t n, uint32_t *q_begin, uint32_t *q_end, uint32_t *t_begin, uint32_t *t_end) {
    if (!ctx) return DAGCON_ERR_INVALID_ARG;
    Ctx *c = reinterpret_cast<Ctx *>(ctx);
    if (n != c->align_n) return fail(c, DAGCON_ERR_INVALID_ARG, "dagcon_align_ends: %u pairs asked, the last alignment had %u", n, c->align_n);
    if (n && (!q_begin || !q_end || !t_begin || !t_end)) return fail(c, DAGCON_ERR_INVALID_ARG, "NULL argument");
    for (uint32_t a = 0; a < n; a++) {
        const uint32_t *e = &c->h_ends[(size_t)a * 4];
        q_begin[a] = e[0]; q_end[a] = e[1]; t_begin[a] = e[2]; t_end[a] = e[3];
    }
    return DAGCON_OK;
}

extern "C++" {
template <int C, int R>
static void launch_panels(hipStream_t s, const DgPanelParams &pp) {
    constexpr int per_wave = R * 64 * (C <= 4 ? 1 : 2);
    constexpr int WPB = per_wave >= 65536 ? 1 : 65536 / per_wave > 4 ? 4 : 65536 / per_wave;
    hipLaunchKernelGGL((k_align_panel<C, R, WPB>), dim3((pp.n + WPB - 1) / WPB), dim3(64 * WPB), 0, s, pp);
}
}

int dagcon_align_panels(dagcon_ctx *ctx, uint32_t n, const uint64_t *q_off, const uint32_t *q_len, const uint64_t *t_off,
                        const uint32_t *t_len, const char *q_blob, uint64_t q_bytes, const char *t_blob, uint64_t t_bytes,
                        const uint64_t *panel_begin, const uint32_t *panel_t_len, const uint32_t *panel_q_len,
                        const uint64_t *out_off, char *qaln, char *taln, uint32_t *aln_len, int32_t *panel_dist) {
    if (!ctx) return DAGCON_ERR_INVALID_ARG;
    Ctx *c = reinterpret_cast<Ctx *>(ctx);
    c->align_dropped = 0;
    if (n == 0) return DAGCON_OK;
    if (!q_off || !q_len || !t_off || !t_len || !q_blob || !t_blob || !panel_begin || !out_off || !qaln || !taln || !aln_len)
        return fail(c, DAGCON_ERR_INVALID_ARG, "NULL argument");
    const uint64_t np = panel_begin[n];
    if (np && (!panel_t_len || !panel_q_len)) return fail(c, DAGCON_ERR_INVALID_ARG, "NULL argument");
    if (np > 0xFFFFFFF0ull) return fail(c, DAGCON_ERR_UNSUPPORTED, "too many panels");
    HIPCHK(c, hipSetDevice(c->device));
    std::vector<uint64_t> p_qoff(np), p_toff(np), p_scr(np);
    std::vector<uint32_t> kept, cls[9];
    std::vector<uint8_t> drop(n, 0);
    uint64_t out_bytes = 0, scr_bytes = 0;
    uint32_t dropped = 0;
    for (uint32_t a = 0; a < n; a++) {
        if (q_off[a] > q_bytes || q_len[a] > q_bytes - q_off[a] || t_off[a] > t_bytes || t_len[a] > t_bytes - t_off[a])
            return fail(c, DAGCON_ERR_INVALID_ARG, "pair %u runs past its blob", a);
// ... 918 lines not shown
```

pbdagcon_amd/csrc/dagcon_dev.h:

```cpp
#pragma once
#include <hip/hip_runtime.h>
#include <stdint.h>

#define DG_GAP '-'

#define DG_F_RAW      1u
#define DG_F_A1_ONLY  8u
#define DG_F_RESWEEP  16u

#define DG_E_BADCHAR     0x001u
#define DG_E_NONCONF     0x002u
#define DG_E_NORM_OVF    0x004u
#define DG_E_NODE_OVF    0x008u
#define DG_E_POOL_OVF    0x010u
#define DG_E_POOL_TGT    0x020u
#define DG_E_STACK       0x040u
#define DG_E_INTERNAL    0x080u
#define DG_E_OUT_OVF     0x100u
#define DG_E_TOO_BIG     0x200u
#define DG_E_LOG_OVF     0x800u
#define DG_E_LIST_OVF    0x400u

#define DG_E_TARGET_MASK (DG_E_BADCHAR | DG_E_NONCONF | DG_E_INTERNAL | DG_E_TOO_BIG)

struct DgStatus {
    uint32_t err_flags;
    uint32_t bad_aln;
    uint32_t bad_target;
    uint32_t n_mseg;
    unsigned long long norm_top;
    unsigned long long node_need;
    unsigned long long pool_need;
    unsigned long long cns_top;
    unsigned long long seg_top;
    unsigned long long n_columns;
    unsigned long long ovf_top;
    unsigned long long dbg[16];
};

struct __attribute__((aligned(16))) DgNode {
    uint16_t out_len, in_len;
    uint8_t base, flags;
    uint16_t pad;
    int32_t weight;
    int32_t pending;
    uint32_t out_off, in_off;
    uint16_t out_cap, in_cap;
    int32_t bbpos;
};
#define DG_NF_BACKBONE 1u
#define DG_NF_DELETED  2u
#define DG_NF_DEFER    8u
#define DG_NF_SHARED   4u

#define DG_CELL_ID(c)   ((c) & 0x1FFFFFFu)
#define DG_CELL_DEL     0x1FFFFFFu
#define DG_CELL_BASE(c) ((uint8_t)((c) >> 25))
#define DG_MAX_NODES    0x1FFFFFDu
#define DG_EMIT_SEG     512u
#define DG_CK_NONE      0xFFFFFFFFu
#define DG_DEFER_MAX    64u
#define DG_SH_MAX       8u
#define DG_TOMB         0xFFFFFFFFu

struct DgParams {
    const uint8_t *q, *t;
    const uint64_t *aln_off;
    const uint32_t *aln_len, *aln_start, *aln_tgt;
    const uint32_t *tlen;
    const uint64_t *aln_begin;
    const uint8_t *tactive;
    uint32_t *tfail;
    const uint8_t *bb;
    const uint64_t *bb_off;
    const uint64_t *mat_base;
    const uint64_t *bbv_base;
    uint32_t T, A;
    uint32_t trim, min_len;
    int32_t min_weight;
    uint32_t flags;
    uint32_t max_k, max_tlen;
    uint32_t *nmis;
    uint64_t *norm_off;
    uint32_t *n_lo, *n_hi, *n_start, *n_ins, *n_del;
    uint16_t *norm;
    uint64_t norm_cap;
    const uint32_t *ch_aln;
    const uint32_t *ch_base;
    uint32_t n_chunks;
    uint32_t *ch_k0;
    uint32_t *ch_next;
    uint32_t *ch_w, *ch_tb;
    uint32_t *ch_flag;
    uint64_t *ch_src;
    uint32_t *ch_out, *ch_adv;
    uint32_t *n_lb;
    uint16_t *norm_tmp;
    uint32_t *ckpt;
    const uint32_t *ck_base;
    uint32_t emit_shift;
    uint64_t tmp_main, tmp_cap;
    uint64_t *node_base;
    uint32_t *n_nodes;
    uint64_t *pool_base;
    uint32_t *pool_size, *pool_top;
    uint32_t *t_nins;
    uint32_t *gcount;
    uint32_t *gbase;
    uint32_t *bid;
    int32_t *cov;
    uint32_t *matA, *matD;
    uint32_t *matC;
    const uint64_t *matc_base;
    const uint32_t *matc_stride;
    DgNode *nodes;
    int32_t *best, *queue;
    float2 *score;
    float *bp_tt;
    float *score_b;
    uint32_t bp_seg_min;
    uint32_t bp_lane;
    uint32_t bl_stk;
    uint8_t *cns_tmp;
    uint64_t node_cap;
    uint32_t *pool;
    uint64_t pool_cap;
    int32_t *stk;
    uint32_t stk_words;
    uint32_t growth_pct;
    uint32_t emit_scan;
    uint32_t fold;
    uint32_t q_kmax;
    uint32_t seg_max;
    uint32_t seg_min;
    uint32_t *cuts;
    uint32_t bp_max;
    uint32_t *cuts_bp;
    float *bp_stat;
    uint32_t *bp_len;
    uint32_t *bp_end;
    float *bp_ab;
    uint32_t *defer;
    uint8_t *cns_tmp0;
    uint32_t gcuts;
    uint32_t *rd_s, *rd_e;
    uint32_t *rd_lead, *rd_trail;
    int32_t *queue0;
    uint32_t *pro_state;
    uint32_t *sh_cnt;
    uint32_t *seg_done;
    uint32_t sh_log;
    uint32_t *worklist;
    uint32_t worklist_cap;
    uint32_t *wl_first;
    uint8_t *cns;
    uint64_t cns_cap;
    uint64_t *cns_off;
    uint32_t *cns_len;
    uint64_t *seg_first;
    uint32_t *n_seg;
    int32_t *seg_r0, *seg_r1;
    uint64_t seg_cap;
    DgStatus *st;
    uint32_t *sup_tmp;
    uint32_t *sup_tmp0;
    uint16_t *sup_w, *sup_d;
    uint32_t *pos_tmp;
    uint32_t *pos_tmp0;
    uint32_t *pos_out;
};

__host__ __device__ inline uint32_t dg_capb(uint32_t k) { return k + 2u < 12u ? k + 2u : 12u; }
```

pbdagcon_amd/csrc/k_build.hip.h:

```cpp
#pragma once
#include <hip/hip_runtime.h>
#include "dagcon_dev.h"

#define DG_WAVE 64
#ifndef DG_LPW
#define DG_LPW 8u
#endif

__device__ __forceinline__ bool dg_failed(const DgParams &p) {
    return __hip_atomic_load(&p.st->err_flags, __ATOMIC_RELAXED, __HIP_MEMORY_SCOPE_AGENT) != 0;
}
__device__ __forceinline__ void dg_fail(const DgParams &p, uint32_t bit) {
    atomicOr(&p.st->err_flags, bit);
}
__device__ __forceinline__ void dg_fail_target(const DgParams &p, uint32_t t, uint32_t bit) {
    atomicOr(&p.tfail[t], bit);
}
__device__ __forceinline__ bool dg_tskip(const DgParams &p, uint32_t t) {
    return !p.tactive[t] || __hip_atomic_load(&p.tfail[t], __ATOMIC_RELAXED, __HIP_MEMORY_SCOPE_AGENT) != 0;
}
__device__ __forceinline__ bool dg_askip(const DgParams &p, uint32_t a) {
    return !(p.flags & DG_F_A1_ONLY) && __hip_atomic_load(&p.tfail[p.aln_tgt[a]], __ATOMIC_RELAXED, __HIP_MEMORY_SCOPE_AGENT) != 0;
}
__device__ __forceinline__ void dg_fail_aln(const DgParams &p, uint32_t a, uint32_t bit) {
    if (p.flags & DG_F_A1_ONLY) dg_fail(p, bit);
    else dg_fail_target(p, p.aln_tgt[a], bit);
    p.st->bad_aln = a;
}

#define DG_COL(qb, tb) ((uint16_t)((uint16_t)(qb) | ((uint16_t)(tb) << 8)))
#define DG_Q(c) ((uint8_t)((c) & 0xff))
#define DG_T(c) ((uint8_t)((c) >> 8))
#define DG_NW 64u
#define DG_NW_BIG 512u
#define DG_REDO 0xFFFFFFFFu

__device__ inline void dg_finish_alignment(const DgParams &p, uint32_t a, uint16_t *buf, uint32_t m) {
    const uint32_t trim = p.trim;
    uint32_t lbases = 0, rbases = 0, lo = 0, hi = m;
    uint32_t start = p.aln_start[a];
    while (lbases < trim && lo < m) {
        if (DG_T(buf[lo++]) != DG_GAP) lbases++;
    }
    while (rbases < trim && hi > lo) {
        if (DG_T(buf[--hi]) != DG_GAP) rbases++;
    }
    start += lbases;
    const bool graph = !(p.flags & DG_F_A1_ONLY);
    uint32_t t_idx = 0, r = 0;
    uint32_t *Cm = nullptr;
    if (graph) {
        t_idx = p.aln_tgt[a];
        if (p.tactive[t_idx]) {
            const uint64_t ab = p.aln_begin[t_idx];
            r = (uint32_t)(a - ab);
            Cm = p.matC + p.matc_base[t_idx] + (uint64_t)r * p.matc_stride[t_idx];
        }
    }
    const uint32_t tlen = graph ? p.tlen[t_idx] : 0xFFFFFFFFu;
    uint32_t n_ins = 0, n_del = 0, adv = 0, run = 0;
    bool conf = start >= 1;
    uint32_t i = lo;
#define DG_FIN_COL(c, ci_)                                                                \
    do {                                                                                  \
        const uint8_t qb_ = DG_Q(c), tb_ = DG_T(c);                                       \
        if (qb_ == tb_ || qb_ == DG_GAP) {                                                \
            if (Cm && conf && ((start + adv) & ((1u << p.emit_shift) - 1u)) == 0 && start + adv <= tlen + 1) \
                ck[(start + adv) >> p.emit_shift] = ci_ - run;                            \
            if (run) { if (Cm && conf && start + adv <= tlen + 1) Cm[start + adv] = run; run = 0; } \
            adv++; n_del += (qb_ != tb_);                                                 \
            if ((uint64_t)start - 1 + adv > (uint64_t)tlen) conf = false;                 \
        } else if (tb_ == DG_GAP) { n_ins++; run++; }                                     \
    } while (0)
    uint32_t *ck = p.ckpt + p.ck_base[a];
    while (i < hi && (i & 7u)) { const uint16_t c = buf[i]; DG_FIN_COL(c, i); i++; }
    while (i + 8 <= hi) {
        const uint4 v = *reinterpret_cast<const uint4 *>(buf + i);
        const uint32_t w4[4] = {v.x, v.y, v.z, v.w};
#pragma unroll
        for (int k = 0; k < 4; k++) {
            const uint16_t c0 = (uint16_t)(w4[k] & 0xffffu), c1 = (uint16_t)(w4[k] >> 16);
            DG_FIN_COL(c0, i + 2 * k);
            DG_FIN_COL(c1, i + 2 * k + 1);
        }
        i += 8;
    }
    while (i < hi) { const uint16_t c = buf[i]; DG_FIN_COL(c, i); i++; }
    if (run && Cm && conf && ((start + adv) & ((1u << p.emit_shift) - 1u)) == 0 && start + adv <= tlen + 1)
        ck[(start + adv) >> p.emit_shift] = hi - run;
    if (run && Cm && conf && start + adv <= tlen + 1) Cm[start + adv] = run;
#undef DG_FIN_COL
    p.n_lo[a] = lo; p.n_hi[a] = hi; p.n_start[a] = start;
    p.n_ins[a] = n_ins; p.n_del[a] = n_del;
    atomicAdd(&p.st->n_columns, (unsigned long long)(hi - lo));
    if (graph && hi > lo && !conf) dg_fail_aln(p, a, DG_E_NONCONF);
}

#ifndef DG_NCH
#define DG_NCH 512u
#endif
#define DG_CH_NONE 0xFFFFFFFFu

__device__ __forceinline__ bool dg_match_col(uint8_t qb, uint8_t tb) { return qb == tb && qb != DG_GAP && qb != '.'; }

__device__ inline uint32_t dg_chunk_start(const uint8_t *q, const uint8_t *t, uint32_t len, uint32_t c) {
    if (c == 0) return 0;
    const uint64_t w0 = (uint64_t)c * DG_NCH;
    if (w0 >= len) return DG_CH_NONE;
    const uint32_t hi = (uint64_t)len < w0 + DG_NCH ? len : (uint32_t)(w0 + DG_NCH);
    for (uint32_t k = (uint32_t)w0; k < hi; k++) {
        const uint8_t b = q[k];
        if (dg_match_col(b, t[k]) && b != q[k - 1] && dg_match_col(q[k - 1], t[k - 1]) && dg_match_col(q[k - 2], t[k - 2]))
            return k;
    }
    return DG_CH_NONE;
}

struct DgChunkRun { uint32_t w, tb; bool dirty, overflow, badchar; };

template <uint32_t NW>
__device__ inline DgChunkRun dg_norm_run(const uint8_t *q, const uint8_t *t, const uint32_t len, const uint32_t k0,
                                         const uint32_t k1, uint16_t *win, uint16_t *out) {
#define DG_W(x) win[(x) & (NW - 1u)]
    DgChunkRun r;
    r.w = 0; r.tb = 0; r.dirty = false; r.overflow = false; r.badchar = false;
    if (k0 >= k1) return r;
    uint32_t badw = 0;
    uint32_t ip = k0, e = 0, i = 0, w = 0, tb = 0, jt = 0, jq = 0;
    uint32_t e_end = 0xFFFFFFFFu;
    uint32_t o0 = 0, o1 = 0, o2 = 0, o3 = 0;
    uint32_t in_done = 0, dirty = 0, overflow = 0;
    for (;;) {
        asm volatile("" : "+v"(in_done), "+v"(dirty));
        if (!in_done && (e - i) + 32u > NW) { overflow = 1; break; }
        if (!in_done) {
            uint32_t take = len - ip;
            if (take > 16u) take = 16u;
            if (ip < k1 && take > k1 - ip) take = k1 - ip;
#define DG_EXPAND(QB, TB)                                                      \
            do {                                                               \
                uint8_t qb_ = (QB), tb_ = (TB);                                \
                if (qb_ == '.') qb_ = DG_GAP;                                  \
                if (tb_ == '.') tb_ = DG_GAP;                                  \
                 \
                                   \
                const bool mm_ = qb_ != tb_ && qb_ != DG_GAP && tb_ != DG_GAP; \
                DG_W(e) = mm_ ? DG_COL(DG_GAP, tb_) : DG_COL(qb_, tb_);        \
                DG_W(e + 1u) = DG_COL(qb_, DG_GAP);                            \
                e += mm_ ? 2u : 1u;                                            \
            } while (0)
            if (take == 16u && (((uintptr_t)(q + ip)) & 15u) == 0) {
                const uint4 qv = *reinterpret_cast<const uint4 *>(q + ip);
                const uint4 tv = *reinterpret_cast<const uint4 *>(t + ip);
                const uint32_t qw[4] = {qv.x, qv.y, qv.z, qv.w}, tw[4] = {tv.x, tv.y, tv.z, tv.w};
#pragma unroll
                for (int k = 0; k < 4; k++) {
                    badw |= ((qw[k] - 0x21212121u) & ~qw[k]) | ((qw[k] + 0x01010101u) | qw[k]);
                    badw |= ((tw[k] - 0x21212121u) & ~tw[k]) | ((tw[k] + 0x01010101u) | tw[k]);
                }
#pragma unroll
                for (int k = 0; k < 16; k++)
                    DG_EXPAND((uint8_t)(qw[k >> 2] >> (8 * (k & 3))), (uint8_t)(tw[k >> 2] >> (8 * (k & 3))));
            } else {
                const uint32_t to_align = (uint32_t)((16u - (((uintptr_t)(q + ip)) & 15u)) & 15u);
                if (to_align && take > to_align) take = to_align;
                for (uint32_t k = 0; k < take; k++) {
                    const uint8_t qb0 = q[ip + k], tb0 = t[ip + k];
                    if (qb0 < 33 || qb0 > 126 || tb0 < 33 || tb0 > 126) badw = 0x80u;
                    DG_EXPAND(qb0, tb0);
                }
            }
#undef DG_EXPAND
            ip += take;
            if (ip == k1) e_end = e;
            if (ip == len) in_done = 1;
        }
        while (i < e && i < e_end) {
            if (i + 1 == e && !in_done) break;
            const uint16_t c = DG_W(i);
            uint8_t qi = DG_Q(c), ti = DG_T(c);
            uint32_t more = 0;
            if (i + 1 < e) {
                if (ti == DG_GAP) {
                    if (jt <= i) jt = i + 1;
                    while (jt < e && DG_T(DG_W(jt)) == DG_GAP) jt++;
                    if (jt < e) {
                        const uint16_t cj = DG_W(jt);
                        if (DG_T(cj) == qi) { ti = qi; DG_W(jt) = DG_COL(DG_Q(cj), DG_GAP); dirty |= (uint32_t)(jt >= e_end); }
                    } else if (!in_done) more = 2;
                }
                if (!more && qi == DG_GAP) {
                    if (jq <= i) jq = i + 1;
                    while (jq < e && DG_Q(DG_W(jq)) == DG_GAP) jq++;
                    if (jq < e) {
                        const uint16_t cj = DG_W(jq);
                        if (DG_Q(cj) == ti) { qi = ti; DG_W(jq) = DG_COL(DG_GAP, DG_T(cj)); dirty |= (uint32_t)(jq >= e_end); }
                    } else if (!in_done) more = 2;
                }
            }
            if (more) { DG_W(i) = DG_COL(qi, ti); break; }
            if (qi != DG_GAP || ti != DG_GAP) {
                o0 = (o0 >> 16) | (o1 << 16); o1 = (o1 >> 16) | (o2 << 16); o2 = (o2 >> 16) | (o3 << 16);
                o3 = (o3 >> 16) | ((uint32_t)DG_COL(qi, ti) << 16);
                w++;
                tb += (ti != DG_GAP);
                if ((w & 7u) == 0) *reinterpret_cast<uint4 *>(out + w - 8) = make_uint4(o0, o1, o2, o3);
            }
            i++;
        }
        if (i == e_end) break;
    }
#undef DG_W
    for (uint32_t k = w & 7u, x = w - (w & 7u); k > 0; k--, x++) {
        const uint32_t sh = 8u - k;
        const uint32_t word = sh >> 1;
        const uint32_t v = word == 0 ? o0 : word == 1 ? o1 : word == 2 ? o2 : o3;
        out[x] = (uint16_t)((sh & 1u) ? v >> 16 : v & 0xffffu);
    }
    r.w = w; r.tb = tb; r.dirty = dirty != 0; r.overflow = overflow != 0; r.badchar = (badw & 0x80808080u) != 0;
    return r;
}

template <uint32_t NW, uint32_t LANES, bool RETRY>
__global__ __launch_bounds__(LANES) void k_norm_chunk(DgParams p) {
    __shared__ uint16_t s_win[LANES * (NW + 2u)];
    const uint32_t g = threadIdx.x * gridDim.x + blockIdx.x;
    if (g >= p.n_chunks) return;
    if (dg_failed(p)) return;
    if (RETRY && p.ch_flag[g] != 2u) return;
    const uint32_t a = p.ch_aln[g];
    if (dg_askip(p, a)) { if (!RETRY) p.ch_flag[g] = 0; return; }
    const uint32_t c = g - p.ch_base[a], nwin = p.ch_base[a + 1] - p.ch_base[a];
    const uint64_t off = p.aln_off[a];
    const uint32_t len = p.aln_len[a];
    const uint8_t *q = p.q + off, *t = p.t + off;
    uint32_t flag = 0;
    DgChunkRun r;
    r.w = 0; r.tb = 0; r.dirty = false; r.overflow = false; r.badchar = false;
    uint32_t k0 = DG_CH_NONE, cn = c + 1;
    uint64_t src = 0;
    if (p.flags & DG_F_RAW) {
        if (c == 0) { k0 = 0; cn = nwin; flag = 1; }
    } else {
        k0 = dg_chunk_start(q, t, len, c);
        if (k0 != DG_CH_NONE) {
            uint16_t *win = s_win + threadIdx.x * (NW + 2u);
            src = (2ull * (off + k0) + 8ull * g + 7ull) & ~7ull;
            for (;;) {
                uint32_t k1 = len;
                for (; cn < nwin; cn++) {
                    const uint32_t s = dg_chunk_start(q, t, len, cn);
                    if (s != DG_CH_NONE) { k1 = s; break; }
                }
                r = dg_norm_run<NW>(q, t, len, k0, k1, win, p.norm_tmp + src);
                if (r.badchar) dg_fail_aln(p, a, DG_E_BADCHAR);
                if (r.overflow) { flag = RETRY ? 1u : 2u; break; }
                if (!r.dirty) break;
                cn++;
                uint32_t k2 = len;
                for (uint32_t x = cn; x < nwin; x++) {
                    const uint32_t s = dg_chunk_start(q, t, len, x);
                    if (s != DG_CH_NONE) { k2 = s; break; }
                }
                const unsigned long long need = (2ull * (k2 - k0) + 15ull) & ~7ull;
                const unsigned long long o = atomicAdd(&p.st->ovf_top, need);
                if (p.tmp_main + o + need > p.tmp_cap) { flag = 1; break; }
                src = p.tmp_main + o;
            }
        }
    }
    p.ch_k0[g] = k0; p.ch_next[g] = cn; p.ch_w[g] = r.w; p.ch_tb[g] = r.tb;
    p.ch_flag[g] = flag; p.ch_src[g] = src;
}

__global__ __launch_bounds__(64) void k_norm_scan(DgParams p) {
    const uint32_t a = blockIdx.x * 64 + threadIdx.x;
    if (a >= p.A) return;
    if (dg_failed(p)) return;
    if (dg_askip(p, a)) return;
    const uint32_t g0 = p.ch_base[a], g1 = p.ch_base[a + 1];
    bool redo = false;
    uint32_t m = 0, tbt = 0;
    for (uint32_t g = g0; g < g1;) {
        if (p.ch_k0[g] == DG_CH_NONE) { p.ch_out[g] = DG_CH_NONE; g++; continue; }
        redo |= p.ch_flag[g] != 0;
        p.ch_out[g] = m; p.ch_adv[g] = tbt;
        m += p.ch_w[g]; tbt += p.ch_tb[g];
        uint32_t nx = g0 + p.ch_next[g];
        if (nx > g1) nx = g1;
        for (uint32_t x = g + 1; x < nx; x++) p.ch_out[x] = DG_CH_NONE;
        g = nx;
    }
    if (redo) { p.n_hi[a] = DG_REDO; return; }
    const uint32_t trim = p.trim;
    uint32_t lbases = 0, rbases = 0, lo = 0, hi = m;
    for (uint32_t g = g0; g < g1 && lbases < trim && lo < m; g++) {
        if (p.ch_out[g] == DG_CH_NONE) continue;
        const uint32_t w = p.ch_w[g], tb = p.ch_tb[g];
        if (lbases + tb < trim) { lo += w; lbases += tb; continue; }
        const uint16_t *src = p.norm_tmp + p.ch_src[g];
        for (uint32_t x = 0; x < w && lbases < trim; x++) {
            if (DG_T(src[x]) != DG_GAP) lbases++;
            lo++;
        }
    }
    for (uint32_t g = g1; g > g0 && rbases < trim && hi > lo;) {
        g--;
        const uint32_t o = p.ch_out[g];
        if (o == DG_CH_NONE) continue;
        const uint32_t tb = p.ch_tb[g];
        if (o >= lo && rbases + tb < trim) { hi = o; rbases += tb; continue; }
        const uint16_t *src = p.norm_tmp + p.ch_src[g];
        while (rbases < trim && hi > lo && hi > o) {
            if (DG_T(src[--hi - o]) != DG_GAP) rbases++;
        }
    }
    p.n_lo[a] = lo; p.n_hi[a] = hi; p.n_start[a] = p.aln_start[a] + lbases; p.n_lb[a] = lbases;
    p.n_ins[a] = 0; p.n_del[a] = 0;
    atomicAdd(&p.st->n_columns, (unsigned long long)(hi - lo));
}

__device__ __forceinline__ uint4 dg_funnel_cols(const uint4 A, const uint4 B, const uint32_t h) {
    const bool w1 = (h >> 1) & 1u, w2 = (h >> 2) & 1u, half = h & 1u;
    const uint32_t u0 = w1 ? A.y : A.x, u1 = w1 ? A.z : A.y, u2 = w1 ? A.w : A.z, u3 = w1 ? B.x : A.w,
                   u4 = w1 ? B.y : B.x, u5 = w1 ? B.z : B.y, u6 = w1 ? B.w : B.z;
    const uint32_t t0 = w2 ? u2 : u0, t1 = w2 ? u3 : u1, t2 = w2 ? u4 : u2, t3 = w2 ? u5 : u3, t4 = w2 ? u6 : u4;
    uint4 r;
    r.x = half ? __builtin_amdgcn_alignbit(t1, t0, 16) : t0;
    r.y = half ? __builtin_amdgcn_alignbit(t2, t1, 16) : t1;
    r.z = half ? __builtin_amdgcn_alignbit(t3, t2, 16) : t2;
    r.w = half ? __builtin_amdgcn_alignbit(t4, t3, 16) : t3;
    return r;
}

__device__ __forceinline__ uint32_t dg_wave_excl(const uint32_t v, const int lane) {
    int incl = (int)v;
    incl += __builtin_amdgcn_update_dpp(0, incl, 0x111, 0xf, 0xf, false);
    incl += __builtin_amdgcn_update_dpp(0, incl, 0x112, 0xf, 0xf, false);
    incl += __builtin_amdgcn_update_dpp(0, incl, 0x114, 0xf, 0xf, false);
    incl += __builtin_amdgcn_update_dpp(0, incl, 0x118, 0xf, 0xf, false);
    incl += __builtin_amdgcn_update_dpp(0, incl, 0x142, 0xa, 0xf, false);
    incl += __builtin_amdgcn_update_dpp(0, incl, 0x143, 0xc, 0xf, false);
    (void)lane;
    return (uint32_t)incl - v;
}

__global__ __launch_bounds__(256) void k_norm_finish2(DgParams p) {
    const uint32_t g = blockIdx.x * 4u + (threadIdx.x >> 6);
    if (g >= p.n_chunks) return;
    if (dg_failed(p)) return;
    const int lane = threadIdx.x & 63;
    const uint32_t a = p.ch_aln[g];
    if (dg_askip(p, a)) return;
    const uint32_t o = p.ch_out[g];
    if (o == DG_CH_NONE) return;
    const uint32_t hi = p.n_hi[a];
    if (hi == DG_REDO) return;
    const uint32_t lo = p.n_lo[a], start = p.n_start[a], lb = p.n_lb[a];
    const uint32_t w = p.ch_w[g], adv0 = p.ch_adv[g];
    const uint16_t *src = p.norm_tmp + p.ch_src[g];
    const uint4 *src4 = reinterpret_cast<const uint4 *>(src);
    uint16_t *dst = p.norm + p.norm_off[a] + o;
    const bool graph = !(p.flags & DG_F_A1_ONLY);
    uint32_t t_idx = 0;
    uint32_t *Cm = nullptr;
    if (graph) {
        t_idx = p.aln_tgt[a];
        if (p.tactive[t_idx]) Cm = p.matC + p.matc_base[t_idx] + (uint64_t)(a - p.aln_begin[t_idx]) * p.matc_stride[t_idx];
    }
    const uint32_t tlen = graph ? p.tlen[t_idx] : 0xFFFFFFFFu;
    uint32_t *ck = p.ckpt + p.ck_base[a];
    const uint32_t ck_mask = (1u << p.emit_shift) - 1u;
    const uint32_t adv_init = adv0 > lb ? adv0 - lb : 0u;
    const uint32_t f0 = lo > o ? lo - o : 0u;
    const uint32_t f1 = hi > o ? (hi - o < w ? hi - o : w) : 0u;
    const bool any = f1 > f0;
    const uint32_t fspan = any ? f1 - f0 : 0u;
#define DG_FIN_CONF(A) (start >= 1u && ((A) == 0u || (uint64_t)start - 1u + (A) <= (uint64_t)tlen))
    const uint32_t h0 = (8u - (o & 7u)) & 7u;
    const uint32_t h = h0 < w ? h0 : w;
    const uint32_t nb = (w - h) / 8u, nvec = (w + 7u) / 8u;
    if ((uint32_t)lane < h) dst[lane] = src[lane];
    { const uint32_t x = h + 8u * nb + (uint32_t)lane; if (lane < 8 && x < w) dst[x] = src[x]; }
    uint4 *dst4 = reinterpret_cast<uint4 *>(dst + h);
    uint32_t adv_tile = adv_init, run_tile = 0, n_ins = 0, n_del = 0;
    for (uint32_t v0 = 0; v0 < nvec; v0 += 64u) {
        const uint32_t vl = v0 + (uint32_t)lane;
        const uint4 pc = vl < nvec ? src4[vl] : make_uint4(0, 0, 0, 0);
        const uint4 pn = vl + 1 < nvec ? src4[vl + 1] : make_uint4(0, 0, 0, 0);
        if (vl < nb) dst4[vl] = dg_funnel_cols(pc, pn, h);
        if (!any || 8u * v0 >= f1) continue;
        uint32_t advm = 0, insm = 0, delm = 0;
#pragma unroll
        for (uint32_t k = 0; k < 8u; k++) {
            const uint32_t wd = ((k >> 1) & 3u) == 0 ? pc.x : ((k >> 1) & 3u) == 1 ? pc.y : ((k >> 1) & 3u) == 2 ? pc.z : pc.w;
            const uint16_t c = (uint16_t)((k & 1u) ? wd >> 16 : wd & 0xffffu);
            const bool inw = 8u * vl + k < 8u * nvec && 8u * vl + k - f0 < fspan;
            const uint8_t qb = DG_Q(c), tb = DG_T(c);
            const bool adv = inw && (qb == tb || qb == DG_GAP);
            advm |= adv ? 1u << k : 0u;
            delm |= (adv && qb != tb) ? 1u << k : 0u;
            insm |= (inw && !adv && tb == DG_GAP) ? 1u << k : 0u;
        }
        const uint32_t nadv = (uint32_t)__popc(advm), nI = (uint32_t)__popc(insm);
        n_ins += nI; n_del += (uint32_t)__popc(delm);
        const uint32_t adv_lane = adv_tile + dg_wave_excl(nadv, lane);
        uint32_t sf = advm ? 1u : 0u;
        uint32_t sv = advm ? (uint32_t)__popc(insm & ~((2u << (31 - __clz((int)advm))) - 1u)) : nI;
#pragma unroll
        for (int d = 1; d < 64; d <<= 1) {
            const uint32_t pf = (uint32_t)__shfl_up((int)sf, d), pv = (uint32_t)__shfl_up((int)sv, d);
            if (lane >= d) { sv = sf ? sv : pv + sv; sf |= pf; }
        }
        uint32_t ef = (uint32_t)__shfl_up((int)sf, 1), ev = (uint32_t)__shfl_up((int)sv, 1);
        if (lane == 0) { ef = 0; ev = 0; }
        uint32_t run = ef ? ev : ev + run_tile;
        const uint32_t lf = (uint32_t)__builtin_amdgcn_readlane((int)sf, 63), lv = (uint32_t)__builtin_amdgcn_readlane((int)sv, 63);
        run_tile = lf ? lv : lv + run_tile;
        adv_tile += (uint32_t)__builtin_amdgcn_readlane((int)(adv_lane - adv_tile + nadv), 63);
        uint32_t adv = adv_lane;
        if (Cm && (advm | insm)) {
#pragma unroll
            for (uint32_t k = 0; k < 8u; k++) {
                if ((advm >> k) & 1u) {
                    const bool conf = DG_FIN_CONF(adv);
                    const uint32_t x = 8u * vl + k;
                    if (conf && ((start + adv) & ck_mask) == 0 && start + adv <= tlen + 1 && !(x == 0 && o > lo))
                        ck[(start + adv) >> p.emit_shift] = o + x - run;
                    if (run && conf && start + adv <= tlen + 1) Cm[start + adv] = run;
                    run = 0;
                    adv++;
                } else if ((insm >> k) & 1u) run++;
            }
        }
    }
    {
        const uint32_t adv = adv_tile, run = run_tile;
        const bool conf = DG_FIN_CONF(adv);
        if (lane == 0) {
            if (any && Cm && conf && ((start + adv) & ck_mask) == 0 && start + adv <= tlen + 1 && (o + f1 < hi || run))
                ck[(start + adv) >> p.emit_shift] = o + f1 - run;
            if (run && Cm && conf && start + adv <= tlen + 1) Cm[start + adv] = run;
            if (graph && any && !conf) dg_fail_aln(p, a, DG_E_NONCONF);
        }
    }
    {
        const uint32_t ti = dg_wave_excl(n_ins, lane) + n_ins, td = dg_wave_excl(n_del, lane) + n_del;
        if (lane == 63) { if (ti) atomicAdd(&p.n_ins[a], ti); if (td) atomicAdd(&p.n_del[a], td); }
    }
#undef DG_FIN_CONF
}

__global__ __launch_bounds__(64) void k_normalize_slow(DgParams p) {
    const uint32_t a = blockIdx.x * 64 + threadIdx.x;
    if (a >= p.A) return;
    if (dg_failed(p)) return;
    if (dg_askip(p, a)) return;
    if (p.n_hi[a] != DG_REDO) return;
    const uint64_t off = p.aln_off[a];
    const uint32_t len = p.aln_len[a];
    const uint8_t *q = p.q + off, *t = p.t + off;
    uint16_t *buf = p.norm + p.norm_off[a];
    const bool raw = (p.flags & DG_F_RAW) != 0;
    uint32_t n = 0;
    for (uint32_t i = 0; i < len; i++) {
        uint8_t qb = q[i], tb = t[i];
        if (qb < 33 || qb > 126 || tb < 33 || tb > 126) dg_fail_aln(p, a, DG_E_BADCHAR);
        if (!raw) {
            if (qb == '.') qb = DG_GAP;
            if (tb == '.') tb = DG_GAP;
            if (qb != tb && qb != DG_GAP && tb != DG_GAP) {
                buf[n++] = DG_COL(DG_GAP, tb);
                buf[n++] = DG_COL(qb, DG_GAP);
                continue;
            }
        }
        buf[n++] = DG_COL(qb, tb);
    }
    uint32_t m = n;
    if (!raw) {
        uint32_t w = 0, jt = 0, jq = 0;
        for (uint32_t i = 0; i < n; i++) {
            uint16_t c = buf[i];
            uint8_t qi = DG_Q(c), ti = DG_T(c);
            if (i + 1 < n) {
                if (ti == DG_GAP) {
                    if (jt <= i) jt = i + 1;
                    while (jt < n && DG_T(buf[jt]) == DG_GAP) jt++;
                    if (jt < n) {
                        uint16_t cj = buf[jt];
                        if (DG_T(cj) == qi) { ti = qi; buf[jt] = DG_COL(DG_Q(cj), DG_GAP); }
                    }
                }
                if (qi == DG_GAP) {
                    if (jq <= i) jq = i + 1;
                    while (jq < n && DG_Q(buf[jq]) == DG_GAP) jq++;
                    if (jq < n) {
                        uint16_t cj = buf[jq];
                        if (DG_Q(cj) == ti) { qi = ti; buf[jq] = DG_COL(DG_GAP, DG_T(cj)); }
                    }
                }
            }
            if (qi != DG_GAP || ti != DG_GAP) buf[w++] = DG_COL(qi, ti);
        }
        m = w;
    }
    dg_finish_alignment(p, a, buf, m);
}

__device__ __forceinline__ uint32_t dg_pool_words(uint32_t tlen, uint32_t n_ins, uint32_t n_del,
                                                  uint32_t k, uint32_t growth_pct, uint32_t *fixed_words) {
    const uint64_t capb = dg_capb(k);
    const uint64_t fixed = 3ull * n_ins + (uint64_t)(tlen + 2) * 3ull * capb;
    const uint64_t spill = 3ull * ((uint64_t)n_ins + n_del + 2ull * k) + 64ull;
    const uint64_t growth = (fixed * growth_pct) / 100ull + spill + 256ull;
    *fixed_words = (uint32_t)fixed;
    const uint64_t tot = fixed + growth;
    return tot > 0xFFFFFFF0ull ? 0xFFFFFFF0u : (uint32_t)tot;
}

__global__ __launch_bounds__(1024) void k_carve(DgParams p) {
    __shared__ unsigned long long s_scan[1024];
    __shared__ unsigned long long s_carry_nodes, s_carry_pool;
    if (dg_failed(p)) return;
    const uint32_t tid = threadIdx.x;
    if (tid == 0) { s_carry_nodes = 0; s_carry_pool = 0; }
    __syncthreads();
    for (uint32_t t0 = 0; t0 < p.T; t0 += 1024) {
        const uint32_t t = t0 + tid;
        unsigned long long nodes = 0, poolw = 0;
        uint32_t fixed_words = 0, ins = 0;
        if (t < p.T && !dg_tskip(p, t)) {
            uint32_t del = 0;
            const uint64_t b = p.aln_begin[t], e = p.aln_begin[t + 1];
            for (uint64_t a = b; a < e; a++) { ins += p.n_ins[a]; del += p.n_del[a]; }
            nodes = (unsigned long long)p.tlen[t] + 2ull + ins;
            poolw = dg_pool_words(p.tlen[t], ins, del, (uint32_t)(e - b), p.growth_pct, &fixed_words);
            if (nodes > DG_MAX_NODES || poolw > 0x3FFFFFFFull) {
                dg_fail_target(p, t, DG_E_TOO_BIG);
                nodes = 0; poolw = 0; fixed_words = 0;
            }
        }
        s_scan[tid] = nodes;
        __syncthreads();
        for (uint32_t o = 1; o < 1024; o <<= 1) {
            unsigned long long v = tid >= o ? s_scan[tid - o] : 0;
            __syncthreads();
            s_scan[tid] += v;
            __syncthreads();
        }
        unsigned long long node_excl = s_scan[tid] - nodes + s_carry_nodes;
        unsigned long long node_tot = s_scan[1023];
        __syncthreads();
        s_scan[tid] = poolw;
        __syncthreads();
        for (uint32_t o = 1; o < 1024; o <<= 1) {
            unsigned long long v = tid >= o ? s_scan[tid - o] : 0;
            __syncthreads();
            s_scan[tid] += v;
            __syncthreads();
        }
        unsigned long long pool_excl = s_scan[tid] - poolw + s_carry_pool;
        unsigned long long pool_tot = s_scan[1023];
        __syncthreads();
        if (t < p.T) {
            p.node_base[t] = node_excl;
            p.n_nodes[t] = (uint32_t)nodes;
            p.pool_base[t] = pool_excl;
            p.pool_size[t] = (uint32_t)poolw;
            p.pool_top[t] = fixed_words;
            p.t_nins[t] = ins;
        }
        if (tid == 0) { s_carry_nodes += node_tot; s_carry_pool += pool_tot; }
        __syncthreads();
    }
    if (tid == 0) {
        p.st->node_need = s_carry_nodes;
        p.st->pool_need = s_carry_pool;
        if (s_carry_nodes > p.node_cap) dg_fail(p, DG_E_NODE_OVF);
        if (s_carry_pool > p.pool_cap) dg_fail(p, DG_E_POOL_OVF);
    }
}

__global__ __launch_bounds__(64) void k_readspan(DgParams p) {
    const uint32_t a = blockIdx.x * 64 + threadIdx.x;
    if (a >= p.A) return;
    if (dg_failed(p)) return;
    const uint32_t t = p.aln_tgt[a];
    uint32_t s = 0, e = 0, lead = 0, trail = 0;
    if (!dg_tskip(p, t)) {
        const uint32_t lo = p.n_lo[a], hi = p.n_hi[a];
        if (hi > lo && hi != DG_REDO) {
            const uint16_t *col = p.norm + p.norm_off[a];
            const uint32_t ins = p.n_ins[a];
            uint32_t i = lo, dels = 0;
            for (; i < hi; i++) {
                const uint8_t qb = DG_Q(col[i]), tb = DG_T(col[i]);
                if (qb == tb) break;
                if (tb == DG_GAP) lead++; else if (qb == DG_GAP) dels++;
            }
            s = p.n_start[a] + dels;
            if (i < hi) {
                uint32_t k = hi, tdels = 0;
                while (k > i + 1) {
                    const uint8_t qb = DG_Q(col[k - 1]), tb = DG_T(col[k - 1]);
                    if (qb == tb) break;
                    if (tb == DG_GAP) trail++; else if (qb == DG_GAP) tdels++;
                    k--;
                }
                e = p.n_start[a] + (hi - lo - ins) - 1u - tdels;
            } else { e = 0; s = 0; }
        }
    }
    p.rd_s[a] = s; p.rd_e[a] = e; p.rd_lead[a] = lead; p.rd_trail[a] = trail;
}

__global__ __launch_bounds__(256) void k_groups(DgParams p) {
    const uint32_t t = blockIdx.x;
    if (dg_failed(p) || dg_tskip(p, t)) return;
    const int lane = threadIdx.x & 63, wave = threadIdx.x >> 6;
    const uint32_t blen = p.tlen[t];
    const uint32_t K = (uint32_t)(p.aln_begin[t + 1] - p.aln_begin[t]);
    uint32_t *col0 = p.matC + p.matc_base[t];
    const uint32_t cstride = p.matc_stride[t];
    uint32_t *gcount = p.gcount + p.bbv_base[t];
    const uint32_t pos0 = (blockIdx.y * 4 + wave) * 8u;
    if (pos0 >= blen + 2) return;
    uint32_t carry[8];
#pragma unroll
    for (int j = 0; j < 8; j++) carry[j] = 0;
    for (uint32_t r0 = 0; r0 < K; r0 += DG_WAVE) {
        const uint32_t r = r0 + lane;
        uint4 *cell = reinterpret_cast<uint4 *>(col0 + (uint64_t)r * cstride + pos0);
        uint4 a = make_uint4(0, 0, 0, 0), b = a;
        if (r < K) { a = cell[0]; b = cell[1]; }
        uint32_t v[8] = {a.x, a.y, a.z, a.w, b.x, b.y, b.z, b.w};
        uint32_t ex[8];
#pragma unroll
        for (int j = 0; j < 8; j++) {
            uint32_t incl = v[j];
            for (int o = 1; o < DG_WAVE; o <<= 1) {
                const uint32_t up = __shfl_up(incl, o);
                if (lane >= o) incl += up;
            }
            ex[j] = carry[j] + incl - v[j];
            carry[j] += __shfl(incl, DG_WAVE - 1);
        }
        if (r < K) {
            cell[0] = make_uint4(ex[0], ex[1], ex[2], ex[3]);
            cell[1] = make_uint4(ex[4], ex[5], ex[6], ex[7]);
        }
    }
#pragma unroll
    for (int j = 0; j < 8; j++)
        if (lane == j && pos0 + j < blen + 2) gcount[pos0 + j] = carry[j];
}

__global__ __launch_bounds__(1024) void k_gscan(DgParams p) {
    __shared__ uint32_t s_scan[1024];
    __shared__ uint32_t s_carry;
    const uint32_t t = blockIdx.x;
    if (dg_failed(p) || dg_tskip(p, t)) return;
    const uint32_t tid = threadIdx.x;
    const uint32_t np = p.tlen[t] + 2;
    const uint64_t bv = p.bbv_base[t];
    if (tid == 0) s_carry = 0;
    __syncthreads();
    for (uint32_t p0 = 0; p0 < np; p0 += 1024) {
        const uint32_t pos = p0 + tid;
        const uint32_t gc = pos < np ? p.gcount[bv + pos] : 0u;
        const uint32_t v = pos < np ? gc + 1u : 0u;
        s_scan[tid] = v;
        __syncthreads();
        for (uint32_t o = 1; o < 1024; o <<= 1) {
            uint32_t x = tid >= o ? s_scan[tid - o] : 0;
            __syncthreads();
            s_scan[tid] += x;
            __syncthreads();
        }
        const uint32_t excl = s_scan[tid] - v + s_carry;
        const uint32_t tot = s_scan[1023];
        __syncthreads();
        if (pos < np) { p.gbase[bv + pos] = excl; p.bid[bv + pos] = excl + gc; }
        if (tid == 0) s_carry += tot;
        __syncthreads();
    }
    if (tid == 0 && s_carry != p.n_nodes[t]) dg_fail_target(p, t, DG_E_INTERNAL);
}

#define DG_CELL_DUP 0x1FFFFFEu
#define DG_EDONE 0xFFFFFFFFu
#define DG_EF_BB 1u
#define DG_EF_OWN 2u
__device__ __forceinline__ uint32_t dg_emit_fold(unsigned long long em, const uint32_t key, const uint32_t first, const uint32_t pos,
                                                 DgNode *ndt, uint32_t *pool, uint32_t *n_out, const int lane) {
    uint32_t victim = 0;
    *n_out = 0;
    while (em & (em - 1ull)) {
        const int f = __ffsll((long long)em) - 1;
        const uint32_t kf = (uint32_t)__builtin_amdgcn_readlane((int)key, f);
        const unsigned long long same = __ballot(key == kf);
        em &= ~same;
        const uint32_t n = (uint32_t)__popcll(same);
        if (n < 2 || !((same >> lane) & 1ull)) continue;
        const uint32_t nins = (key & 0xFF0000u) ? 3u : (key & 0xFF00u) ? 2u : 1u;
        if (lane == f) {
            *n_out = n;
            for (uint32_t k = 0; k < nins; k++) {
                const uint32_t id = first + k, rk = id - pos;
                reinterpret_cast<DgNode *>(reinterpret_cast<char *>(ndt) + (id << 5))->weight = (int32_t)n;
                pool[3u * rk + 1u] = n;
            }
        } else {
            victim = 1;
            for (uint32_t k = 0; k < nins; k++) {
                const uint32_t base = (key >> (8u * (nins - 1u - k))) & 0xFFu;
                *reinterpret_cast<uint2 *>(reinterpret_cast<char *>(ndt) + ((first + k) << 5)) = make_uint2(0u, base | (DG_NF_DELETED << 8));
            }
        }
    }
    return victim;
}

__global__ __launch_bounds__(256) void k_gsum(DgParams p) {
    const uint32_t t = blockIdx.x;
    if (dg_failed(p) || dg_tskip(p, t)) return;
    const uint32_t pos = blockIdx.y * 256u + threadIdx.x;
    if (pos >= p.tlen[t] + 2u) return;
    const uint32_t K = (uint32_t)(p.aln_begin[t + 1] - p.aln_begin[t]);
    const uint32_t *col = p.matC + p.matc_base[t] + pos;
    const uint32_t stride = p.matc_stride[t];
    uint32_t sum = 0;
    for (uint32_t r = 0; r < K; r++) sum += col[(uint64_t)r * stride];
    p.gcount[p.bbv_base[t] + pos] = sum;
}

#ifndef DG_EB
#define DG_EB 8
#endif
#ifndef DG_ERPW
#define DG_ERPW 64
#endif
#ifndef DG_ECOLS
#define DG_ECOLS 40u
#define DG_ECOLS_STRIDE 42u
#define DG_ENEED 16u
#endif
__global__ __launch_bounds__(64) void k_emit(DgParams p) {
    __shared__ uint32_t s_D[DG_EB * 64];
    __shared__ uint16_t s_col[64 * DG_ECOLS_STRIDE];
    if (dg_failed(p)) return;
    const uint32_t t = blockIdx.x;
    if (dg_tskip(p, t)) return;
    const int lane = threadIdx.x;
    uint16_t *colw = s_col + lane * DG_ECOLS_STRIDE;
    const uint64_t ab = p.aln_begin[t];
    const uint32_t K = (uint32_t)(p.aln_begin[t + 1] - ab);
    const uint32_t r = blockIdx.y * DG_ERPW + lane;
    if (blockIdx.y * DG_ERPW >= K) return;
    const bool idle = r >= K || lane >= DG_ERPW;
    const uint32_t a = (uint32_t)(ab + (idle ? 0 : r));
    const uint32_t blen = p.tlen[t];
    const uint32_t exitpos = blen + 1;
    if ((blockIdx.z << p.emit_shift) > exitpos) return;
    const uint64_t nb = p.node_base[t];
    const uint64_t bv = p.bbv_base[t];
    const uint32_t *bid = p.bid + bv, *gbase = p.gbase + bv;
    uint32_t *Am = p.matA + p.mat_base[t];
    uint32_t *Dm = p.matD + p.mat_base[t];
    const uint32_t *Cm = p.matC + p.matc_base[t] + (uint64_t)(idle ? 0 : r) * p.matc_stride[t];
    uint32_t *pool = p.pool + p.pool_base[t];
    DgNode *ndt = p.nodes + nb;
#define DG_EPW(OFF) (*reinterpret_cast<uint32_t *>(reinterpret_cast<char *>(pool) + (((uint32_t)(OFF)) << 2)))
#define DG_ECELL(M, POS) (*reinterpret_cast<uint32_t *>(reinterpret_cast<char *>((M) + (uint64_t)(POS) * K) + (r << 2)))
    const uint16_t *buf = p.norm + p.norm_off[a];
    const uint32_t lo = idle ? 0 : p.n_lo[a], hi = idle ? 0 : p.n_hi[a];
    uint32_t bbpos = idle ? DG_EDONE : p.n_start[a];
    uint32_t prev = 0;
    uint32_t prev_pos = 0;
    uint32_t fl = DG_EF_BB | DG_EF_OWN;
    uint32_t i = lo;
    const uint32_t P0 = blockIdx.z << p.emit_shift, P1 = P0 + (1u << p.emit_shift);
    const bool rvalid = !idle;
    bool pfx_entry = false;
    if (!idle) {
        if (bbpos >= P1) bbpos = DG_EDONE;
        else if (bbpos < P0) {
            const uint32_t ck = p.ckpt[p.ck_base[a] + blockIdx.z];
            if (ck == DG_CK_NONE || ck >= hi) bbpos = DG_EDONE;
            else {
                i = ck; bbpos = P0; fl = DG_EF_BB;
                uint32_t x = ck, d = 0;
                while (x > lo) {
                    const uint16_t c = buf[--x];
                    const uint8_t qb = DG_Q(c), tb = DG_T(c);
                    if (qb == tb) { prev_pos = P0 - 1u - d; prev = bid[prev_pos]; break; }
                    if (qb == DG_GAP) { d++; continue; }
                    if (tb == DG_GAP) {
                        prev_pos = P0 - d;
                        if (p.emit_scan) pfx_entry = true;
                        else {
                            const uint32_t c1 = r + 1 < K ? Cm[p.matc_stride[t] + prev_pos] : p.gcount[bv + prev_pos];
                            prev = gbase[prev_pos] + c1 - 1u;
                        }
                        fl = 0;
                        break;
                    }
                }
            }
        }
    }
    if (p.emit_scan) {
        for (unsigned long long m = __ballot(pfx_entry); m; m = __ballot(pfx_entry)) {
            const uint32_t pp = (uint32_t)__builtin_amdgcn_readlane((int)prev_pos, __ffsll((long long)m) - 1);
            const uint32_t x = rvalid ? Cm[pp] : 0u;
            const uint32_t e = dg_wave_excl(x, lane);
            if (pfx_entry && prev_pos == pp) { prev = gbase[pp] + e + x - 1u; pfx_entry = false; }
        }
    }
    uint32_t c_base = 0x80000000u;
#define DG_STAGE(I)                                                                         \
    do {                                                                                    \
        c_base = (I) & ~7u;                                                                 \
        const uint4 *src_ = reinterpret_cast<const uint4 *>(buf + c_base);                  \
        uint4 v_[DG_ECOLS / 8];                                                             \
        _Pragma("unroll") for (int k_ = 0; k_ < (int)(DG_ECOLS / 8); k_++)                  \
            v_[k_] = (c_base + 8u * k_ < hi) ? src_[k_] : make_uint4(0, 0, 0, 0);           \
        _Pragma("unroll") for (int k_ = 0; k_ < (int)(DG_ECOLS / 8); k_++) {                \
            uint32_t *dst_ = reinterpret_cast<uint32_t *>(colw) + 4 * k_;                   \
            dst_[0] = v_[k_].x; dst_[1] = v_[k_].y; dst_[2] = v_[k_].z; dst_[3] = v_[k_].w; \
        }                                                                                   \
    } while (0)
#define DG_COLUMN(I, OUT)                                                                   \
    do {                                                                                    \
        if ((I) - c_base >= DG_ECOLS) DG_STAGE(I);                                          \
        OUT = colw[(I) - c_base];                                                           \
    } while (0)
#define DG_DEPART(NXT)                                                       \
    do {                                                                     \
        if (!(fl & DG_EF_OWN)) break;                                        \
        if (fl & DG_EF_BB) {                                                 \
            if (prev_pos >= pos0) s_D[(prev_pos - pos0) * 64 + lane] = (NXT) + 1u;   \
            else DG_ECELL(Dm, prev_pos) = (NXT) + 1u;                \
        } else {                                                             \
            const uint32_t _rk = prev - prev_pos;                            \
            DG_EPW(3u * _rk) = (NXT);                                        \
            DG_EPW(3u * _rk + 1u) = 1u;                                      \
        }                                                                    \
    } while (0)

    uint32_t pos0 = P0;
    while (pos0 < P1 && (pos0 <= blen || (!__all(bbpos == DG_EDONE) && pos0 <= blen + 2u * DG_EB))) {
        uint32_t bidv[DG_EB];
        {
            const uint4 *bp = reinterpret_cast<const uint4 *>(bid + pos0);
#pragma unroll
            for (int k = 0; k < DG_EB / 4; k++) {
                const uint4 v = bp[k];
                bidv[4 * k] = v.x; bidv[4 * k + 1] = v.y; bidv[4 * k + 2] = v.z; bidv[4 * k + 3] = v.w;
            }
        }
        uint32_t gbv[DG_EB], cmv[DG_EB];
        {
            const uint4 *gp = reinterpret_cast<const uint4 *>(gbase + pos0);
#pragma unroll
            for (int k = 0; k < DG_EB / 4; k++) {
                const uint4 v = gp[k];
                gbv[4 * k] = v.x; gbv[4 * k + 1] = v.y; gbv[4 * k + 2] = v.z; gbv[4 * k + 3] = v.w;
            }
            const uint4 *cp = reinterpret_cast<const uint4 *>(Cm + pos0);
#pragma unroll
            for (int k = 0; k < DG_EB / 4; k++) {
                const uint4 v = cp[k];
                cmv[4 * k] = v.x; cmv[4 * k + 1] = v.y; cmv[4 * k + 2] = v.z; cmv[4 * k + 3] = v.w;
            }
        }
        if (p.emit_scan) {
#pragma unroll
            for (int j = 0; j < DG_EB; j++) {
                const uint32_t x = rvalid ? cmv[j] : 0u;
                cmv[j] = __ballot(x != 0u) ? dg_wave_excl(x, lane) : 0u;
            }
        }
        if (bbpos != DG_EDONE && i < hi && (i - c_base) + DG_ENEED > DG_ECOLS) DG_STAGE(i);
        uint32_t acell[DG_EB];
#pragma unroll
        for (int j = 0; j < DG_EB; j++) { acell[j] = 0; s_D[j * 64 + lane] = 0; }
        uint32_t exit_val = 0;
#pragma unroll
        for (int j = 0; j < DG_EB; j++) {
            const uint32_t pos = pos0 + j;
            uint32_t f_apos = 0, f_key = 0, f_first = 0;
            asm volatile("" : "+v"(fl));
            if (bbpos == pos && pos < P1) {
                uint32_t ins_id = 0;
                uint32_t kacc = 0;
                uint16_t c = 0;
                f_apos = prev_pos;
                const bool f_anc_ok = fl == (DG_EF_BB | DG_EF_OWN) && pos - prev_pos < 16u;
                for (;;) {
                    if (i < hi) DG_COLUMN(i, c);
                    const uint8_t qb = DG_Q(c), tb = DG_T(c);
                    if (i >= hi || qb == tb || qb == DG_GAP) break;
                    if (tb == DG_GAP) {
                        if (!ins_id) { ins_id = gbv[j] + cmv[j]; f_first = ins_id; }
                        kacc = (kacc << 8) | qb;
                        const uint32_t id = ins_id++;
                        const uint32_t rk = id - bbpos;
                        DgNode nd;
                        nd.out_len = 1; nd.in_len = 1; nd.base = qb; nd.flags = 0; nd.pad = 0;
                        nd.weight = 1; nd.pending = 1;
                        nd.out_off = 3u * rk; nd.in_off = 3u * rk + 2u; nd.out_cap = 1; nd.in_cap = 1;
                        nd.bbpos = (int32_t)bbpos;
                        *reinterpret_cast<DgNode *>(reinterpret_cast<char *>(ndt) + (id << 5)) = nd;
                        DG_EPW(3u * rk + 2u) = prev;
                        DG_DEPART(id);
                        prev = id; prev_pos = bbpos; fl = DG_EF_OWN;
                    }
                    i++;
                }
                if (i >= hi) {
                    exit_val = (fl & DG_EF_OWN) ? prev + 1u : 0u;
                    const uint32_t ex = bid[exitpos];
                    DG_DEPART(ex);
                    bbpos = DG_EDONE;
                } else {
                    const uint8_t qb = DG_Q(c), tb = DG_T(c);
                    if (qb == tb) {
                        const uint32_t cur = bidv[j];
                        acell[j] = ((uint32_t)tb << 25) | (prev + 1u);
                        if (f_anc_ok && kacc != 0u && kacc < (1u << 24)) f_key = kacc | ((pos - f_apos) << 24);
                        DG_DEPART(cur);
                        prev = cur; prev_pos = bbpos; fl = DG_EF_BB | DG_EF_OWN;
                    } else {
                        acell[j] = ((uint32_t)tb << 25) | DG_CELL_DEL;
                    }
                    bbpos++;
                    i++;
                }
            }
            if (p.fold) {
                const unsigned long long em = __ballot(f_key != 0u);
                if (em & (em - 1ull)) {
                    uint32_t fn;
                    const uint32_t vic = dg_emit_fold(em, f_key, f_first, pos, ndt, pool, &fn, lane);
                    if (vic | fn) {
                        const uint32_t dv = vic ? 0u : (f_first + 1u) | ((fn - 1u) << 25);
                        if (f_apos >= pos0) s_D[(f_apos - pos0) * 64 + lane] = dv;
                        if (f_apos < pos0 || f_apos == 0u) DG_ECELL(Dm, f_apos) = dv;
                        if (vic) acell[j] = (acell[j] & 0xFE000000u) | DG_CELL_DUP;
                    }
                }
            }
        }
        if (r < K && lane < DG_ERPW) {
#pragma unroll
            for (int j = 0; j < DG_EB; j++) {
                const uint32_t pos = pos0 + j;
                if (pos <= blen && pos >= P0 && pos < P1) {
                    DG_ECELL(Am, pos) = acell[j];
                    const uint32_t dv = s_D[j * 64 + lane];
                    if (pos > 0 || dv) DG_ECELL(Dm, pos) = dv;
                }
            }
            if (exit_val) DG_ECELL(Am, exitpos) = exit_val;
        }
        pos0 += DG_EB;
    }
    {
        const bool ahead = bbpos != DG_EDONE && (fl & DG_EF_OWN);
        uint32_t q = bbpos, nxt = 0;
        bool found = false, pfx_next = false;
        if (ahead) {
            while (i < hi) {
                const uint16_t c = buf[i];
                const uint8_t qb = DG_Q(c), tb = DG_T(c);
                if (qb == tb) { nxt = bid[q]; found = true; break; }
                if (qb == DG_GAP) { q++; i++; continue; }
                if (tb == DG_GAP) {
                    if (p.emit_scan) pfx_next = true; else nxt = gbase[q] + Cm[q];
                    found = true; break;
                }
                i++;
            }
        }
        if (p.emit_scan) {
            for (unsigned long long m = __ballot(pfx_next); m; m = __ballot(pfx_next)) {
                const uint32_t pp = (uint32_t)__builtin_amdgcn_readlane((int)q, __ffsll((long long)m) - 1);
                const uint32_t x = rvalid ? Cm[pp] : 0u;
                const uint32_t e = dg_wave_excl(x, lane);
                if (pfx_next && q == pp) { nxt = gbase[pp] + e; pfx_next = false; }
            }
        }
        if (ahead) {
            if (!found) {
                nxt = bid[exitpos];
                Am[(uint64_t)exitpos * K + r] = prev + 1u;
            }
            const uint32_t pos0 = 0xFFFFFFFFu;
            DG_DEPART(nxt);
        }
    }
#undef DG_EPW
#undef DG_ECELL
#undef DG_DEPART
#undef DG_COLUMN
#undef DG_STAGE
}

__device__ __forceinline__ int dg_lds_find(volatile int32_t *vals, int n, int x, int lane) {
    for (int b = 0; b < n; b += DG_WAVE) {
        int i = b + lane;
        bool hit = (i < n) && (vals[i] == x);
        unsigned long long m = __ballot(hit);
        if (m) return b + (__ffsll((long long)m) - 1);
    }
    return -1;
}

__device__ __forceinline__ uint32_t dg_pool_alloc(const DgParams &p, uint32_t t, uint32_t words, int lane) {
    uint32_t off = 0;
    if (lane == 0) {
        t = (uint32_t)__builtin_amdgcn_readfirstlane((int)t);
        off = atomicAdd(&p.pool_top[t], words);
        if ((uint64_t)off + words > p.pool_size[t]) { dg_fail(p, DG_E_POOL_TGT); p.st->bad_target = t; off = 0xFFFFFFFFu; }
    }
    return (uint32_t)__builtin_amdgcn_readlane((int)off, 0);
}

__device__ __forceinline__ unsigned long long dg_list_row(int32_t val, int32_t extra, int32_t chain, int32_t ulo, int32_t uhi,
                                                          int lane, int32_t &cnt, unsigned long long &cm) {
    cm = __ballot(val == chain);
    const bool uniq = val >= ulo && val < uhi;
    unsigned long long firsts = __ballot(uniq);
    cnt = 1 + extra;
    unsigned long long rem = __ballot(val != 0 && !uniq) & ~cm;
    while (rem) {
        const int first = __ffsll((long long)rem) - 1;
        const int32_t x = __builtin_amdgcn_readlane(val, first);
        const unsigned long long same = __ballot(val == x);
        rem &= ~same;
        if (lane == first) cnt = __popcll(same) + extra;
        firsts |= 1ull << first;
    }
    return firsts;
}

__device__ __forceinline__ void dg_lists_wave(const DgParams &p, uint32_t t, uint32_t pos0, uint32_t blen, uint32_t K,
                                              int lane) {
    const uint32_t npos = min(DG_LPW, blen + 2 - pos0);
    const uint64_t nb = p.node_base[t];
    const uint64_t bv = p.bbv_base[t];
    const uint32_t capb = dg_capb(K);
    const uint32_t fixed0 = 3u * p.t_nins[t];
    uint32_t *pool = p.pool + p.pool_base[t];
#define DG_LPOOL(OFF) (*reinterpret_cast<uint32_t *>(reinterpret_cast<char *>(pool) + (((uint32_t)(OFF)) << 2)))
    const uint32_t qb = pos0 - 1u + (uint32_t)lane;
    const uint32_t bidl = (lane < (int)DG_LPW + 2 && qb <= blen + 1) ? p.bid[bv + qb] : 0u;
    const uint32_t gbl = (lane <= (int)DG_LPW && pos0 + lane <= blen + 1) ? p.gbase[bv + pos0 + lane] : 0u;
    const uint32_t rb = (uint32_t)lane << 2;
    const bool rl = (uint32_t)lane < K;
    const uint32_t *Ar = p.matA + p.mat_base[t] + (uint64_t)pos0 * K, *Dr = p.matD + p.mat_base[t] + (uint64_t)pos0 * K;
#define DG_LROW(R) (rl ? *reinterpret_cast<const uint32_t *>(reinterpret_cast<const char *>(R) + rb) : 0u)
    uint32_t dcell = DG_LROW(Dr), acell = DG_LROW(Ar);
    const uint32_t lpos = pos0 + (uint32_t)lane;
    uint32_t r_lens = 0;
    uint32_t r_cov = 0;
    uint32_t r_out = fixed0 + lpos * 3u * capb, r_in = r_out + 2u * capb;
    uint32_t r_caps = capb | capb << 16;
    uint32_t pi = 0;
    for (; pi < npos; pi++) {
        const uint32_t pos = pos0 + pi;
        const uint32_t dep = dcell, arr = acell;
        if (pi + 1 < npos) {
            Ar += K; Dr += K;
            dcell = DG_LROW(Dr); acell = DG_LROW(Ar);
        }
        const bool mine = (uint32_t)lane == pi;
        const int32_t v1 = __builtin_amdgcn_readlane((int)bidl, pi + 1) + 1;
        uint32_t out_len = 0, in_len = 0;
        if (pos <= blen) {
            const int32_t val = (int32_t)DG_CELL_ID(dep), extra = (int32_t)(dep >> 25);
            const int32_t chain = __builtin_amdgcn_readlane((int)bidl, pi + 2) + 1;
            const int32_t ulo = __builtin_amdgcn_readlane((int)gbl, pi + 1) + 1;
            int32_t cnt;
            unsigned long long cm;
            const unsigned long long firsts = dg_list_row(val, extra, chain, ulo, chain, lane, cnt, cm);
            const uint32_t n = 1u + (uint32_t)__popcll(firsts);
            uint32_t off = fixed0 + pos * 3u * capb;
            if (n > capb) {
                const uint32_t cap = n + 2u;
                off = dg_pool_alloc(p, t, 2u * cap, lane);
                if (off == 0xFFFFFFFFu) break;
                if (mine) { r_out = off; r_caps = (r_caps & 0xFFFF0000u) | cap; }
            }
            const uint32_t idx = 1u + (uint32_t)__popcll(firsts & ((1ull << lane) - 1ull));
            if (lane == 0) { DG_LPOOL(off) = (uint32_t)(chain - 1); DG_LPOOL(off + 1) = (uint32_t)__popcll(cm); }
            if ((firsts >> lane) & 1ull) { DG_LPOOL(off + 2 * idx) = (uint32_t)(val - 1); DG_LPOOL(off + 2 * idx + 1) = (uint32_t)cnt; }
            out_len = n;
        }
        if (pos >= 1) {
            const uint32_t idf = DG_CELL_ID(arr);
            if (pos <= blen) {
                const unsigned long long covered = __ballot(arr != 0u);
                const uint32_t n_cov = (uint32_t)__popcll(covered);
                const uint32_t n_match = (uint32_t)__popcll(__ballot(arr != 0u && idf != DG_CELL_DEL));
                const uint32_t last_base = covered ? DG_CELL_BASE((uint32_t)__builtin_amdgcn_readlane((int)arr, 63 - __clzll((long long)covered))) : 0u;
                if (mine) r_cov = n_cov | n_match << 8 | last_base << 16;
            }
            const int32_t val = (arr != 0u && idf != DG_CELL_DEL && idf != DG_CELL_DUP) ? (int32_t)idf : 0;
            const int32_t chain = __builtin_amdgcn_readlane((int)bidl, pi) + 1;
            const int32_t ulo = __builtin_amdgcn_readlane((int)gbl, pi) + 1;
            int32_t cnt;
            unsigned long long cm;
            const unsigned long long firsts = dg_list_row(val, 0, chain, ulo, v1, lane, cnt, cm);
            const uint32_t n = 1u + (uint32_t)__popcll(firsts);
            uint32_t off = fixed0 + pos * 3u * capb + 2u * capb;
            if (n > capb) {
                const uint32_t cap = n + 2u;
                off = dg_pool_alloc(p, t, cap, lane);
                if (off == 0xFFFFFFFFu) break;
                if (mine) { r_in = off; r_caps = (r_caps & 0xFFFFu) | cap << 16; }
            }
            const uint32_t idx = 1u + (uint32_t)__popcll(firsts & ((1ull << lane) - 1ull));
            if (lane == 0) DG_LPOOL(off) = (uint32_t)(chain - 1);
            if ((firsts >> lane) & 1ull) DG_LPOOL(off + idx) = (uint32_t)(val - 1);
            in_len = n;
        }
        if (mine) r_lens = out_len | in_len << 16;
    }
    const uint32_t v = __shfl_down(bidl, 1);
    if ((uint32_t)lane < pi) {
        const bool inner = lpos >= 1 && lpos <= blen;
        const uint32_t n_cov = r_cov & 0xFFu, n_match = (r_cov >> 8) & 0xFFu;
        uint32_t base;
        if (lpos == 0) base = '^';
        else if (lpos == blen + 1) base = '$';
        else if (n_cov) base = r_cov >> 16;
        else base = p.bb ? p.bb[p.bb_off[t] + (lpos - 1)] : (uint8_t)'N';
        uint4 *rec = reinterpret_cast<uint4 *>(p.nodes + nb + v);
        rec[0] = make_uint4(r_lens, base | DG_NF_BACKBONE << 8,
                            inner ? 1u + n_match : 0u,
                            r_lens >> 16);
        rec[1] = make_uint4(r_out, r_in, r_caps, inner ? lpos : 0u);
        p.cov[bv + lpos] = inner ? (int32_t)n_cov : 0;
    }
#undef DG_LROW
#undef DG_LPOOL
}

__global__ __launch_bounds__(256) void k_lists(DgParams p) {
    extern __shared__ int32_t s_tmp[];
    const uint32_t t = blockIdx.x;
    if (dg_failed(p) || dg_tskip(p, t)) return;
    const int lane = threadIdx.x & 63, wave = threadIdx.x >> 6;
    const uint32_t blen = p.tlen[t];
    const uint32_t K = (uint32_t)(p.aln_begin[t + 1] - p.aln_begin[t]);
    if (K > DG_WAVE) {
    const uint32_t stride = p.max_k + 2;
    volatile int32_t *vals = s_tmp + (size_t)wave * 2 * stride;
    volatile int32_t *cnts = vals + stride;
    const uint64_t nb = p.node_base[t];
    const uint64_t bv = p.bbv_base[t];
    uint32_t *pool = p.pool + p.pool_base[t];
    const uint32_t *Am0 = p.matA + p.mat_base[t], *Dm0 = p.matD + p.mat_base[t];
    const uint32_t capb = dg_capb(K);
    const uint32_t fixed0 = 3u * p.t_nins[t];
    for (uint32_t pi = 0; pi < DG_LPW; pi++) {
    const uint32_t pos = (blockIdx.y * 4 + wave) * DG_LPW + pi;
    if (pos >= blen + 2) return;
    const uint32_t v = p.bid[bv + pos];
    const uint32_t *Am = Am0 + (uint64_t)pos * K;
    const uint32_t *Dm = Dm0 + (uint64_t)pos * K;
    const uint32_t fixed = fixed0 + pos * 3u * capb;
    uint32_t out_off = fixed, in_off = fixed + 2u * capb;
    uint32_t out_cap = capb, in_cap = capb;
    uint32_t out_len = 0, in_len = 0;
// ... 107 lines not shown
```

Measured before the change: 339.4 million.

## Store insertion-run matrix as bytes and batch status readback into one block

The per-alignment insertion-run matrix matC is stored as uint8 when max_k is at most 64 and no run overflows, and falls back to uint32 otherwise. This cuts the memset, the writes in normalize, and the reads in gsum and emit by four times, and gsum now sums four packed byte columns per thread. Per-target status arrays (tfail, cns_len, n_seg, cns_off, seg_first, DgStatus) are merged into one device block with a pinned host mirror, so a single memset clears them and a single copy fetches them. Segment ranges move into one buffer with pinned host staging. The risk is overflow handling for byte cells, which relies on a wide_cells fallback path not fully shown.

```diff
diff --git a/pbdagcon_amd/csrc/dagcon_api.hip b/pbdagcon_amd/csrc/dagcon_api.hip
--- a/pbdagcon_amd/csrc/dagcon_api.hip
+++ b/pbdagcon_amd/csrc/dagcon_api.hip
@@ -81,6 +81,16 @@
     return pl;
 }
 
+struct StatBlock {
+    DevBuf dev;
+    char *host = nullptr;
+    size_t host_cap = 0;
+    size_t o_tfail = 0, o_cns_len = 0, o_n_seg = 0, o_cns_off = 0, o_seg_first = 0;
+    size_t zero_bytes = 0, bytes = 0;
+    template <typename X> X *d(size_t off) const { return reinterpret_cast<X *>(static_cast<char *>(dev.p) + off); }
+    template <typename X> const X *h(size_t off) const { return reinterpret_cast<const X *>(host + off); }
+};
+
 struct Ctx {
     dagcon_opts opts;
     int device = 0;
@@ -104,6 +114,7 @@
     std::vector<uint64_t> h_aln_begin, h_aln_off, h_mat_base, h_bbv_base, h_bb_off, h_matc_base;
     std::vector<uint32_t> h_matc_stride;
     uint64_t matc_cells = 0;
+    bool wide_cells = false;
     std::vector<uint8_t> h_tactive;
     std::vector<uint32_t> h_ch_base, h_ch_aln;
     std::vector<uint64_t> h_norm_off;
@@ -113,7 +124,7 @@
     uint32_t n_chunks = 0;
     uint64_t tmp_main = 0, tmp_cap = 0;
 
-    DevBuf d_tfail, d_q, d_t, d_aln_off, d_aln_len, d_aln_start, d_aln_tgt, d_tlen, d_aln_begin, d_tactive,
+    DevBuf d_q, d_t, d_aln_off, d_aln_len, d_aln_start, d_aln_tgt, d_tlen, d_aln_begin, d_tactive,
         d_bb, d_bb_off, d_mat_base, d_bbv_base, d_matc_base, d_matc_stride;
     DevBuf d_nmis, d_norm_off, d_n_lo, d_n_hi, d_n_start, d_n_ins, d_n_del, d_norm;
     DevBuf d_ch_aln, d_ch_base, d_ch_k0, d_ch_next, d_ch_w, d_ch_tb, d_ch_flag, d_ch_src, d_ch_out, d_ch_adv,
@@ -134,7 +145,9 @@
     bool rs_valid = false;
     std::vector<uint32_t> rs_match, rs_mismatch, rs_ins, rs_del;
     std::vector<uint8_t> rs_fate;
-    DevBuf d_cns, d_cns_off, d_cns_len, d_seg_first, d_n_seg, d_seg_r0, d_seg_r1, d_st;
+    DevBuf d_cns;
+    StatBlock sb;
+    DevBuf d_seg;
     DevBuf d_pos_tmp, d_pos_tmp0, d_pos;
     DevBuf d_sup_tmp, d_sup_tmp0, d_sup;
 
@@ -148,9 +161,11 @@
     DgStatus h_st;
     dagcon_timings tm;
 
-    std::vector<uint64_t> r_seg_begin, r_seq_off, r_cns_off, r_seg_first;
-    std::vector<int32_t> r_range0, r_range1, r_tmp0, r_tmp1;
-    std::vector<uint32_t> r_seq_len, r_cns_len, r_n_seg, r_tfail;
+    std::vector<uint64_t> r_seg_begin, r_seq_off;
+    std::vector<int32_t> r_range0, r_range1;
+    std::vector<uint32_t> r_seq_len;
+    int32_t *r_seg = nullptr;
+    size_t r_seg_cap = 0;
     std::vector<int32_t> r_status;
     char *r_blob = nullptr;
     size_t r_blob_cap = 0;
@@ -220,6 +235,32 @@
 void free_buf(DevBuf &b) {
     if (b.p) (void)hipFree(b.p);
     b.p = nullptr; b.cap = 0;
+}
+
+size_t seg_stride(const Ctx *c) { return ((size_t)c->seg_cap + 3) & ~(size_t)3; }
+
+bool matc_wide(const Ctx *c) { return c->max_k > 64u || c->wide_cells; }
+size_t matc_bytes(const Ctx *c) { return (size_t)c->matc_cells * (matc_wide(c) ? 4u : 1u); }
+
+int ensure_stat(Ctx *c, uint32_t T) {
+    StatBlock &b = c->sb;
+    auto up16 = [](size_t x) { return (x + 15) & ~(size_t)15; };
+    b.o_tfail = up16(sizeof(DgStatus));
+    b.o_cns_len = b.o_tfail + up16(((size_t)T + 1) * 4);
+    b.o_n_seg = b.o_cns_len + up16((size_t)T * 4);
+    b.zero_bytes = b.o_n_seg + up16((size_t)T * 4);
+    b.o_cns_off = b.zero_bytes;
+    b.o_seg_first = b.o_cns_off + up16((size_t)T * 8);
+    b.bytes = b.o_seg_first + up16((size_t)T * 8);
+    ENSURE(c, b.dev, b.bytes);
+    if (b.host_cap < b.bytes) {
+        if (b.host) (void)hipHostFree(b.host);
+        b.host = nullptr; b.host_cap = 0;
+        const size_t want = b.bytes + b.bytes / 8 + 4096;
+        HIPCHK(c, hipHostMalloc((void **)&b.host, want, hipHostMallocDefault));
+        b.host_cap = want;
+    }
+    return DAGCON_OK;
 }
 
 int ensure_arenas(Ctx *c) {
@@ -261,8 +302,15 @@
         if (c->gcuts) ENSURE(c, c->d_pos_tmp0, c->node_cap * 4);
         ENSURE(c, c->d_pos, c->cns_cap * 4);
     }
-    ENSURE(c, c->d_seg_r0, c->seg_cap * 4);
-    ENSURE(c, c->d_seg_r1, c->seg_cap * 4);
+    ENSURE(c, c->d_seg, 2 * seg_stride(c) * 4);
+    if (c->r_seg_cap < c->seg_cap) {
+        if (c->r_seg) (void)hipHostFree(c->r_seg);
+        c->r_seg = nullptr; c->r_seg_cap = 0;
+        const size_t want = (size_t)c->seg_cap + (size_t)(c->seg_cap / 8) + 1024;
+        HIPCHK(c, hipHostMalloc((void **)&c->r_seg, 2 * want * 4, hipHostMallocDefault));
+        c->r_seg_cap = want;
+    }
+    ENSURE(c, c->d_matC, matc_bytes(c) + 256);
     return DAGCON_OK;
 }
 
@@ -275,7 +323,7 @@
     p.aln_tgt = (const uint32_t *)c->d_aln_tgt.p;
     p.tlen = (const uint32_t *)c->d_tlen.p;
     p.aln_begin = (const uint64_t *)c->d_aln_begin.p;
-    p.tactive = (const uint8_t *)c->d_tactive.p; p.tfail = (uint32_t *)c->d_tfail.p;
+    p.tactive = (const uint8_t *)c->d_tactive.p; p.tfail = c->sb.d<uint32_t>(c->sb.o_tfail);
     p.bb = c->have_bb ? (const uint8_t *)c->d_bb.p : nullptr;
     p.bb_off = (const uint64_t *)c->d_bb_off.p;
     p.mat_base = (const uint64_t *)c->d_mat_base.p;
@@ -303,7 +351,7 @@
     p.node_base = (uint64_t *)c->d_node_base.p; p.n_nodes = (uint32_t *)c->d_n_nodes.p;
     p.pool_base = (uint64_t *)c->d_pool_base.p; p.pool_size = (uint32_t *)c->d_pool_size.p;
     p.pool_top = (uint32_t *)c->d_pool_top.p; p.t_nins = (uint32_t *)c->d_t_nins.p;
-    p.matA = (uint32_t *)c->d_matA.p; p.matD = (uint32_t *)c->d_matD.p; p.matC = (uint32_t *)c->d_matC.p;
+    p.matA = (uint32_t *)c->d_matA.p; p.matD = (uint32_t *)c->d_matD.p; p.matC = c->d_matC.p;
     p.cov = (int32_t *)c->d_cov.p; p.gcount = (uint32_t *)c->d_gcount.p;
     p.gbase = (uint32_t *)c->d_gbase.p; p.bid = (uint32_t *)c->d_bid.p;
     p.nodes = (DgNode *)c->d_nodes.p; p.best = (int32_t *)c->d_best.p;
@@ -326,11 +374,11 @@
     p.seg_done = (uint32_t *)c->d_seg_done.p; p.wl_first = (uint32_t *)c->d_wl_first.p;
     p.worklist = (uint32_t *)c->d_worklist.p; p.worklist_cap = c->worklist_cap;
     p.cns = (uint8_t *)c->d_cns.p; p.cns_cap = c->cns_cap;
-    p.cns_off = (uint64_t *)c->d_cns_off.p; p.cns_len = (uint32_t *)c->d_cns_len.p;
-    p.seg_first = (uint64_t *)c->d_seg_first.p; p.n_seg = (uint32_t *)c->d_n_seg.p;
-    p.seg_r0 = (int32_t *)c->d_seg_r0.p; p.seg_r1 = (int32_t *)c->d_seg_r1.p;
+    p.cns_off = c->sb.d<uint64_t>(c->sb.o_cns_off); p.cns_len = c->sb.d<uint32_t>(c->sb.o_cns_len);
+    p.seg_first = c->sb.d<uint64_t>(c->sb.o_seg_first); p.n_seg = c->sb.d<uint32_t>(c->sb.o_n_seg);
+    p.seg_r0 = (int32_t *)c->d_seg.p; p.seg_r1 = p.seg_r0 + seg_stride(c);
     p.seg_cap = c->seg_cap;
-    p.st = (DgStatus *)c->d_st.p;
+    p.st = c->sb.d<DgStatus>(0);
     if (c->opts.flags & DAGCON_FLAG_BASE_SUPPORT) {
         p.sup_tmp = (uint32_t *)c->d_sup_tmp.p; p.sup_tmp0 = (uint32_t *)c->d_sup_tmp0.p;
         p.sup_w = (uint16_t *)c->d_sup.p; p.sup_d = p.sup_w + c->cns_cap;
@@ -340,15 +388,20 @@
     }
 }
 
-void launch_normalize(Ctx *c, const DgParams &p) {
+void launch_normalize(Ctx *c, const DgParams &p, const bool wide) {
     hipStream_t s = c->stream;
     if (c->A == 0) return;
     (void)hipMemsetAsync(c->d_ckpt.p, 0xFF, c->n_ckpt * 4, s);
     hipLaunchKernelGGL((k_norm_chunk<DG_NW, 64, false>), dim3((c->n_chunks + 63) / 64), dim3(64), 0, s, p);
     hipLaunchKernelGGL((k_norm_chunk<DG_NW_BIG, 32, true>), dim3((c->n_chunks + 31) / 32), dim3(32), 0, s, p);
     hipLaunchKernelGGL(k_norm_scan, dim3((c->A + 63) / 64), dim3(64), 0, s, p);
-    hipLaunchKernelGGL(k_norm_finish2, dim3((c->n_chunks + 3) / 4), dim3(256), 0, s, p);
-    hipLaunchKernelGGL(k_normalize_slow, dim3((c->A + 63) / 64), dim3(64), 0, s, p);
+    if (wide) {
+        hipLaunchKernelGGL(k_norm_finish2<uint32_t>, dim3((c->n_chunks + 3) / 4), dim3(256), 0, s, p);
+        hipLaunchKernelGGL(k_normalize_slow<uint32_t>, dim3((c->A + 63) / 64), dim3(64), 0, s, p);
+    } else {
+        hipLaunchKernelGGL(k_norm_finish2<uint8_t>, dim3((c->n_chunks + 3) / 4), dim3(256), 0, s, p);
+        hipLaunchKernelGGL(k_normalize_slow<uint8_t>, dim3((c->A + 63) / 64), dim3(64), 0, s, p);
+    }
 }
 
 int launch_all(Ctx *c) {
@@ -357,22 +410,21 @@
     DgParams p;
     fill_params(c, p);
     hipStream_t s = c->stream;
+    const bool wide = matc_wide(c);
     if (c->poison & 8) {
         DevBuf *work[] = {&c->d_nmis, &c->d_n_lo, &c->d_n_hi, &c->d_n_start, &c->d_n_ins, &c->d_n_del, &c->d_ch_k0, &c->d_ch_next, &c->d_ch_w,
                           &c->d_ch_tb, &c->d_ch_flag, &c->d_ch_src, &c->d_ch_out, &c->d_ch_adv, &c->d_n_lb, &c->d_norm_tmp, &c->d_ckpt,
                           &c->d_node_base, &c->d_n_nodes, &c->d_pool_base, &c->d_pool_size, &c->d_pool_top, &c->d_t_nins, &c->d_cov, &c->d_gcount,
                           &c->d_gbase, &c->d_bid, &c->d_best, &c->d_queue, &c->d_score, &c->d_cns_tmp, &c->d_bp_tt, &c->d_stk, &c->d_cuts,
                           &c->d_cuts_bp, &c->d_bp_stat, &c->d_bp_len, &c->d_rd, &c->d_pro_state, &c->d_sh_cnt, &c->d_wl_first,
-                          &c->d_queue0, &c->d_bp_end, &c->d_bp_ab, &c->d_defer, &c->d_cns_tmp0, &c->d_cns, &c->d_cns_off, &c->d_seg_first,
-                          &c->d_seg_r0, &c->d_seg_r1, &c->d_worklist, &c->d_seg_done, &c->d_sup_tmp, &c->d_sup_tmp0, &c->d_sup, &c->d_pos_tmp, &c->d_pos_tmp0, &c->d_pos};
+                          &c->d_queue0, &c->d_bp_end, &c->d_bp_ab, &c->d_defer, &c->d_cns_tmp0, &c->d_cns,
+                          &c->d_seg, &c->d_worklist, &c->d_seg_done, &c->d_sup_tmp, &c->d_sup_tmp0, &c->d_sup, &c->d_pos_tmp, &c->d_pos_tmp0, &c->d_pos};
         for (DevBuf *b : work)
             if (b->p && b->cap) HIPCHK(c, hipMemsetAsync(b->p, 0xEE, b->cap, s));
-    }
-    HIPCHK(c, hipMemsetAsync(c->d_st.p, 0, sizeof(DgStatus), s));
-    HIPCHK(c, hipMemsetAsync(c->d_tfail.p, 0, (size_t)c->T * 4 + 4, s));
-    HIPCHK(c, hipMemsetAsync(c->d_cns_len.p, 0, (size_t)c->T * 4, s));
-    HIPCHK(c, hipMemsetAsync(c->d_n_seg.p, 0, (size_t)c->T * 4, s));
-    if (c->matc_cells) HIPCHK(c, hipMemsetAsync(c->d_matC.p, 0, c->matc_cells * 4, s));
+        if (c->sb.bytes > c->sb.zero_bytes) HIPCHK(c, hipMemsetAsync(c->sb.d<char>(c->sb.zero_bytes), 0xEE, c->sb.bytes - c->sb.zero_bytes, s));
+    }
+    HIPCHK(c, hipMemsetAsync(c->sb.dev.p, 0, c->sb.zero_bytes, s));
+    if (c->matc_cells) HIPCHK(c, hipMemsetAsync(c->d_matC.p, 0, matc_bytes(c), s));
     if (c->poison) {
         if ((c->poison & 1) && c->d_matA.p) { HIPCHK(c, hipMemsetAsync(c->d_matA.p, 0xEE, c->d_matA.cap, s)); HIPCHK(c, hipMemsetAsync(c->d_matD.p, 0xEE, c->d_matD.cap, s)); }
         if ((c->poison & 2) && c->d_nodes.p) { HIPCHK(c, hipMemsetAsync(c->d_nodes.p, 0xEE, c->d_nodes.cap, s)); HIPCHK(c, hipMemsetAsync(c->d_pool.p, 0xEE, c->d_pool.cap, s)); }
@@ -380,18 +432,21 @@
         if ((c->poison & 4) && c->d_norm.p) HIPCHK(c, hipMemsetAsync(c->d_norm.p, 0xEE, c->d_norm.cap, s));
     }
     HIPCHK(c, hipEventRecord(c->ev[0], s));
-    launch_normalize(c, p);
+    launch_normalize(c, p, wide);
     HIPCHK(c, hipEventRecord(c->ev[1], s));
     hipLaunchKernelGGL(k_carve, dim3(1), dim3(1024), 0, s, p);
     if (c->T > 0) {
         const uint32_t rows4 = (c->max_tlen + 2 + 4 * DG_LPW - 1) / (4 * DG_LPW);
         if (c->gcuts && c->A > 0) hipLaunchKernelGGL(k_readspan, dim3((c->A + 63) / 64), dim3(64), 0, s, p);
-        if (p.emit_scan) hipLaunchKernelGGL(k_gsum, dim3(c->T, (c->max_tlen + 2 + 255) / 256), dim3(256), 0, s, p);
+        if (p.emit_scan && wide) hipLaunchKernelGGL(k_gsum<uint32_t>, dim3(c->T, (c->max_tlen + 2 + 255) / 256), dim3(256), 0, s, p);
+        else if (p.emit_scan) hipLaunchKernelGGL(k_gsum<uint8_t>, dim3(c->T, (c->max_tlen + 2 + 1023) / 1024), dim3(256), 0, s, p);
         else hipLaunchKernelGGL(k_groups, dim3(c->T, (c->max_tlen + 2 + 31) / 32), dim3(256), 0, s, p);
         hipLaunchKernelGGL(k_gscan, dim3(c->T), dim3(1024), 0, s, p);
-        if (c->A > 0)
-            hipLaunchKernelGGL(k_emit, dim3(c->T, (c->max_k + DG_ERPW - 1) / DG_ERPW, ((c->max_tlen + 2) >> c->emit_shift) + 1),
-                               dim3(64), 0, s, p);
+        if (c->A > 0) {
+            const dim3 eg(c->T, (c->max_k + DG_ERPW - 1) / DG_ERPW, ((c->max_tlen + 2) >> c->emit_shift) + 1);
+            if (wide) hipLaunchKernelGGL(k_emit<uint32_t>, eg, dim3(64), 0, s, p);
+            else hipLaunchKernelGGL(k_emit<uint8_t>, eg, dim3(64), 0, s, p);
+        }
         const size_t lds = (size_t)4 * 2 * (c->max_k + 2) * sizeof(int32_t);
         if (lds > 65536)
             HIPCHK(c, hipFuncSetAttribute((const void *)k_lists, hipFuncAttributeMaxDynamicSharedMemorySize, (int)lds));
@@ -502,7 +557,7 @@
     }
     for (auto &e : c->ev)
         if (hipEventCreate(&e) != hipSuccess) { delete c; return DAGCON_ERR_HIP; }
-    if (ensure(c, c->d_st, sizeof(DgStatus)) != DAGCON_OK) { delete c; return DAGCON_ERR_WORKSPACE; }
+    if (ensure_stat(c, 0) != DAGCON_OK) { dagcon_destroy(reinterpret_cast<dagcon_ctx *>(c)); return DAGCON_ERR_WORKSPACE; }
     *out = reinterpret_cast<dagcon_ctx *>(c);
     return DAGCON_OK;
 }
@@ -514,15 +569,16 @@
     if (c->stream) (void)hipStreamSynchronize(c->stream);
     if (c->r_blob) (void)hipHostFree(c->r_blob);
     if (c->r_sup) (void)hipHostFree(c->r_sup);
+    if (c->r_seg) (void)hipHostFree(c->r_seg);
+    if (c->sb.host) (void)hipHostFree(c->sb.host);
     DevBuf *all[] = {&c->d_q, &c->d_t, &c->d_aln_off, &c->d_aln_len, &c->d_aln_start, &c->d_aln_tgt,
-                     &c->d_tlen, &c->d_aln_begin, &c->d_tactive, &c->d_tfail, &c->d_bb, &c->d_bb_off, &c->d_mat_base, &c->d_matc_base, &c->d_matc_stride,
+                     &c->d_tlen, &c->d_aln_begin, &c->d_tactive, &c->sb.dev, &c->d_bb, &c->d_bb_off, &c->d_mat_base, &c->d_matc_base, &c->d_matc_stride,
                      &c->d_bbv_base, &c->d_nmis, &c->d_norm_off, &c->d_n_lo, &c->d_n_hi, &c->d_n_start, &c->d_ch_aln, &c->d_ch_base, &c->d_ch_k0, &c->d_ch_next, &c->d_ch_w, &c->d_ch_tb, &c->d_ch_flag, &c->d_ch_src, &c->d_ch_out, &c->d_ch_adv, &c->d_n_lb, &c->d_norm_tmp, &c->d_ckpt, &c->d_ck_base,
                      &c->d_n_ins, &c->d_n_del, &c->d_norm, &c->d_node_base, &c->d_n_nodes,
                      &c->d_pool_base, &c->d_pool_size, &c->d_pool_top, &c->d_t_nins, &c->d_matA, &c->d_matD,
                      &c->d_matC, &c->d_cov, &c->d_gcount, &c->d_gbase, &c->d_bid, &c->d_nodes,
                      &c->d_best, &c->d_queue, &c->d_score, &c->d_cns_tmp, &c->d_bp_tt, &c->d_score_b, &c->d_pool, &c->d_stk, &c->d_cuts, &c->d_cuts_bp, &c->d_bp_stat, &c->d_bp_len, &c->d_worklist, &c->d_rd, &c->d_pro_state, &c->d_sh_cnt, &c->d_seg_done, &c->d_wl_first, &c->d_queue0, &c->d_bp_end, &c->d_bp_ab, &c->d_defer, &c->d_cns_tmp0, &c->d_cns,
-                     &c->d_cns_off, &c->d_cns_len, &c->d_seg_first, &c->d_n_seg, &c->d_seg_r0, &c->d_seg_r1,
-                     &c->d_st, &c->d_sup_tmp, &c->d_sup_tmp0, &c->d_sup, &c->d_pos_tmp, &c->d_pos_tmp0, &c->d_pos};
+                     &c->d_seg, &c->d_sup_tmp, &c->d_sup_tmp0, &c->d_sup, &c->d_pos_tmp, &c->d_pos_tmp0, &c->d_pos};
     for (DevBuf *b : all) free_buf(*b);
     for (DevBuf &b : c->d_al) free_buf(b);
     for (DevBuf &b : c->d_pn) free_buf(b);
@@ -541,6 +597,7 @@
     c->sup_valid = c->pos_valid = false;
     c->h_cig_bad.clear();
     c->rs_valid = false;
+    c->wide_cells = false;
     const uint32_t T = b->n_targets;
     if (T && (!b->tlen || !b->aln_begin)) return fail(c, DAGCON_ERR_INVALID_ARG, "tlen/aln_begin is NULL");
     const uint64_t A_all = T ? b->aln_begin[T] : 0;
@@ -693,13 +750,11 @@
     }
     ENSURE(c, c->d_node_base, (size_t)T * 8); ENSURE(c, c->d_n_nodes, T4);
     ENSURE(c, c->d_pool_base, (size_t)T * 8); ENSURE(c, c->d_pool_size, T4); ENSURE(c, c->d_pool_top, T4);
-    ENSURE(c, c->d_t_nins, T4); ENSURE(c, c->d_tfail, T4 + 4);
+    ENSURE(c, c->d_t_nins, T4);
     ENSURE(c, c->d_matA, c->mat_cells * 4); ENSURE(c, c->d_matD, c->mat_cells * 4);
-    ENSURE(c, c->d_matC, c->matc_cells * 4 + 256);
     ENSURE(c, c->d_cov, c->sum_bb * 4); ENSURE(c, c->d_gcount, c->sum_bb * 4);
     ENSURE(c, c->d_gbase, c->sum_bb * 4); ENSURE(c, c->d_bid, c->sum_bb * 4);
-    ENSURE(c, c->d_cns_off, (size_t)T * 8); ENSURE(c, c->d_cns_len, T4);
-    ENSURE(c, c->d_seg_first, (size_t)T * 8); ENSURE(c, c->d_n_seg, T4);
+    if ((r = ensure_stat(c, T))) return r;
 
     c->node_cap = std::max<uint64_t>(c->node_cap, c->sum_bb + c->sum_len / 7 + 1024);
     c->pool_cap = std::max<uint64_t>(c->pool_cap, 8ull * c->node_cap + 80ull * c->sum_bb + 1024ull * T);
@@ -776,7 +831,7 @@
 
 static int read_status(Ctx *c) {
     HIPCHK(c, hipStreamSynchronize(c->stream));
-    HIPCHK(c, d2h(c, &c->h_st, c->d_st.p, sizeof(DgStatus)));
+    HIPCHK(c, d2h(c, &c->h_st, c->sb.dev.p, sizeof(DgStatus)));
     return DAGCON_OK;
 }
 
@@ -786,8 +841,10 @@
     if (!c->ran) return fail(c, DAGCON_ERR_STATE, "dagcon_fetch before dagcon_run");
     HIPCHK(c, hipSetDevice(c->device));
     int r;
+    const StatBlock &sb = c->sb;
     for (int attempt = 0;; attempt++) {
-        if ((r = read_status(c))) return r;
+        HIPCHK(c, d2h(c, sb.host, sb.dev.p, sb.bytes));
+        memcpy(&c->h_st, sb.host, sizeof(DgStatus));
         const uint32_t f = c->h_st.err_flags;
         if (f == 0) break;
         if (f & DG_E_TARGET_MASK)
@@ -800,6 +857,7 @@
         if (f & DG_E_STACK) c->stk_words *= 4;
         if (f & DG_E_LIST_OVF) c->worklist_cap *= 4;
         if (f & DG_E_LOG_OVF) c->sh_log *= 2;
+        if (f & DG_E_RUN_WIDE) c->wide_cells = true;
         if (f & DG_E_OUT_OVF) {
             c->cns_cap = std::max<uint64_t>(c->cns_cap, c->h_st.cns_top + 1024);
             c->seg_cap = std::max<uint64_t>(c->seg_cap, c->h_st.seg_top + 1024);
@@ -815,12 +873,13 @@
     HIPCHK(c, hipEventElapsedTime(&ms, c->ev[3], c->ev[4])); c->tm.ms_bestpath = ms;
 
     const uint32_t T = c->T;
-    c->r_tfail.assign(T, 0); c->r_status.assign(T, DAGCON_OK);
-    if (T) HIPCHK(c, d2h(c, c->r_tfail.data(), c->d_tfail.p, (size_t)T * 4));
+    const uint32_t *m_tfail = sb.h<uint32_t>(sb.o_tfail), *m_n_seg = sb.h<uint32_t>(sb.o_n_seg);
+    const uint64_t *m_cns_off = sb.h<uint64_t>(sb.o_cns_off), *m_seg_first = sb.h<uint64_t>(sb.o_seg_first);
+    c->r_status.assign(T, DAGCON_OK);
     uint32_t n_failed = 0;
     c->err.clear();
     for (uint32_t t = 0; t < T; t++) {
-        const uint32_t f = c->r_tfail[t];
+        const uint32_t f = m_tfail[t];
         if (!f) continue;
         const int code = (f & (DG_E_BADCHAR | DG_E_NONCONF)) ? DAGCON_ERR_NONCONFORMING
                        : (f & DG_E_TOO_BIG) ? DAGCON_ERR_UNSUPPORTED : DAGCON_ERR_INTERNAL;
@@ -838,8 +897,7 @@
         if (!n_failed++) c->err = c->cig_err;
     }
     const uint64_t nseg = c->h_st.seg_top, nb = c->h_st.cns_top;
-    c->r_cns_off.assign(T, 0); c->r_cns_len.assign(T, 0); c->r_seg_first.assign(T, 0); c->r_n_seg.assign(T, 0);
-    c->r_tmp0.assign(nseg, 0); c->r_tmp1.assign(nseg, 0);
+    if (nseg > c->r_seg_cap || nseg > c->seg_cap) return fail(c, DAGCON_ERR_INTERNAL, "%llu segments in an arena of %llu", (unsigned long long)nseg, (unsigned long long)c->seg_cap);
     if (c->r_blob_cap < nb + 1) {
         if (c->r_blob) (void)hipHostFree(c->r_blob);
         c->r_blob = nullptr; c->r_blob_cap = 0;
@@ -849,49 +907,44 @@
     }
     c->r_blob[nb] = 0;
     const bool full = !(c->opts.flags & (DAGCON_FLAG_STOP_AFTER_BUILD | DAGCON_FLAG_STOP_AFTER_MERGE));
-    if (T && full) {
-        HIPCHK(c, d2h(c, c->r_cns_off.data(), c->d_cns_off.p, (size_t)T * 8));
-        HIPCHK(c, d2h(c, c->r_cns_len.data(), c->d_cns_len.p, (size_t)T * 4));
-        HIPCHK(c, d2h(c, c->r_seg_first.data(), c->d_seg_first.p, (size_t)T * 8));
-        HIPCHK(c, d2h(c, c->r_n_seg.data(), c->d_n_seg.p, (size_t)T * 4));
-        if (nseg) {
-            HIPCHK(c, d2h(c, c->r_tmp0.data(), c->d_seg_r0.p, nseg * 4));
-            HIPCHK(c, d2h(c, c->r_tmp1.data(), c->d_seg_r1.p, nseg * 4));
-        }
-        if (nb) HIPCHK(c, d2h(c, c->r_blob, c->d_cns.p, nb));
-    }
+    const bool want_sup = full && (c->opts.flags & DAGCON_FLAG_BASE_SUPPORT), want_pos = full && (c->opts.flags & DAGCON_FLAG_BASE_POS);
     c->sup_valid = c->pos_valid = false;
-    if (full && (c->opts.flags & DAGCON_FLAG_BASE_SUPPORT)) {
-        if (c->r_sup_cap < nb + 1) {
-            if (c->r_sup) (void)hipHostFree(c->r_sup);
-            c->r_sup = nullptr; c->r_sup_cap = 0;
-            const size_t want = (size_t)(nb + 1) + (size_t)(nb / 8) + 4096;
-            HIPCHK(c, hipHostMalloc((void **)&c->r_sup, want * 4, hipHostMallocDefault));
-            c->r_sup_cap = want;
-        }
-        if (nb) {
-            HIPCHK(c, hipMemcpyAsync(c->r_sup, c->d_sup.p, nb * 2, hipMemcpyDeviceToHost, c->stream));
-            HIPCHK(c, d2h(c, c->r_sup + nb, (const uint16_t *)c->d_sup.p + c->cns_cap, nb * 2));
-        }
-        c->r_sup_n = nb;
-        c->sup_valid = true;
-    }
-    if (full && (c->opts.flags & DAGCON_FLAG_BASE_POS)) {
-        c->r_pos.resize(nb + 1);
-        if (nb) HIPCHK(c, d2h(c, c->r_pos.data(), c->d_pos.p, nb * 4));
-        c->pos_valid = true;
-    }
+    if (want_sup && c->r_sup_cap < nb + 1) {
+        if (c->r_sup) (void)hipHostFree(c->r_sup);
+        c->r_sup = nullptr; c->r_sup_cap = 0;
+        const size_t want = (size_t)(nb + 1) + (size_t)(nb / 8) + 4096;
+        HIPCHK(c, hipHostMalloc((void **)&c->r_sup, want * 4, hipHostMallocDefault));
+        c->r_sup_cap = want;
+    }
+    if (want_pos) c->r_pos.resize(nb + 1);
+    int32_t *m_r0 = c->r_seg, *m_r1 = c->r_seg + nseg;
+    bool queued = false;
+    if (T && full && nseg) {
+        HIPCHK(c, hipMemcpyAsync(m_r0, c->d_seg.p, nseg * 4, hipMemcpyDeviceToHost, c->stream));
+        HIPCHK(c, hipMemcpyAsync(m_r1, (const int32_t *)c->d_seg.p + seg_stride(c), nseg * 4, hipMemcpyDeviceToHost, c->stream));
+        queued = true;
+    }
+    if (T && full && nb) { HIPCHK(c, hipMemcpyAsync(c->r_blob, c->d_cns.p, nb, hipMemcpyDeviceToHost, c->stream)); queued = true; }
+    if (want_sup && nb) {
+        HIPCHK(c, hipMemcpyAsync(c->r_sup, c->d_sup.p, nb * 2, hipMemcpyDeviceToHost, c->stream));
+        HIPCHK(c, hipMemcpyAsync(c->r_sup + nb, (const uint16_t *)c->d_sup.p + c->cns_cap, nb * 2, hipMemcpyDeviceToHost, c->stream));
+        queued = true;
+    }
+    if (want_pos && nb) { HIPCHK(c, hipMemcpyAsync(c->r_pos.data(), c->d_pos.p, nb * 4, hipMemcpyDeviceToHost, c->stream)); queued = true; }
+    if (queued) HIPCHK(c, hipStreamSynchronize(c->stream));
+    if (want_sup) { c->r_sup_n = nb; c->sup_valid = true; }
+    if (want_pos) c->pos_valid = true;
     c->r_seg_begin.assign(T + 1, 0);
     c->r_range0.clear(); c->r_range1.clear(); c->r_seq_off.clear(); c->r_seq_len.clear();
     uint64_t bases = 0;
     for (uint32_t t = 0; t < T; t++) {
         c->r_seg_begin[t] = c->r_range0.size();
-        if (!full || !c->h_tactive[t] || c->r_tfail[t]) continue;
-        for (uint32_t i = 0; i < c->r_n_seg[t]; i++) {
-            const uint64_t s = c->r_seg_first[t] + i;
-            const int32_t r0 = c->r_tmp0[s], r1 = c->r_tmp1[s];
+        if (!full || !c->h_tactive[t] || m_tfail[t]) continue;
+        for (uint32_t i = 0; i < m_n_seg[t]; i++) {
+            const uint64_t s = m_seg_first[t] + i;
+            const int32_t r0 = m_r0[s], r1 = m_r1[s];
             c->r_range0.push_back(r0); c->r_range1.push_back(r1);
-            c->r_seq_off.push_back(c->r_cns_off[t] + (uint64_t)r0);
+            c->r_seq_off.push_back(m_cns_off[t] + (uint64_t)r0);
             c->r_seq_len.push_back((uint32_t)(r1 - r0));
             bases += (uint64_t)(r1 - r0);
         }
@@ -945,7 +998,7 @@
     HIPCHK(c, hipSetDevice(c->device));
     HIPCHK(c, hipStreamSynchronize(c->stream));
     DgStatus st;
-    HIPCHK(c, d2h(c, &st, c->d_st.p, sizeof st));
+    HIPCHK(c, d2h(c, &st, c->sb.dev.p, sizeof st));
     for (int i = 0; i < 16; i++) out8[i] = st.dbg[i];
     return DAGCON_OK;
 }
@@ -1007,9 +1060,8 @@
         DgParams p;
         fill_params(c, p);
         p.flags |= DG_F_A1_ONLY;
-        HIPCHK(c, hipMemsetAsync(c->d_st.p, 0, sizeof(DgStatus), c->stream));
-        HIPCHK(c, hipMemsetAsync(c->d_tfail.p, 0, (size_t)c->T * 4 + 4, c->stream));
-        launch_normalize(c, p);
+        HIPCHK(c, hipMemsetAsync(c->sb.dev.p, 0, c->sb.zero_bytes, c->stream));
+        launch_normalize(c, p, true);
         HIPCHK(c, hipGetLastError());
         if ((r = read_status(c))) return r;
         if ((c->h_st.err_flags & DG_E_NORM_OVF) && attempt < 3) {
diff --git a/pbdagcon_amd/csrc/dagcon_dev.h b/pbdagcon_amd/csrc/dagcon_dev.h
--- a/pbdagcon_amd/csrc/dagcon_dev.h
+++ b/pbdagcon_amd/csrc/dagcon_dev.h
@@ -20,6 +20,7 @@
 #define DG_E_TOO_BIG     0x200u
 #define DG_E_LOG_OVF     0x800u
 #define DG_E_LIST_OVF    0x400u
+#define DG_E_RUN_WIDE    0x1000u
 
 #define DG_E_TARGET_MASK (DG_E_BADCHAR | DG_E_NONCONF | DG_E_INTERNAL | DG_E_TOO_BIG)
 
@@ -110,7 +111,7 @@
     uint32_t *bid;
     int32_t *cov;
     uint32_t *matA, *matD;
-    uint32_t *matC;
+    void *matC;
     const uint64_t *matc_base;
     const uint32_t *matc_stride;
     DgNode *nodes;
diff --git a/pbdagcon_amd/csrc/k_build.hip.h b/pbdagcon_amd/csrc/k_build.hip.h
--- a/pbdagcon_amd/csrc/k_build.hip.h
+++ b/pbdagcon_amd/csrc/k_build.hip.h
@@ -35,6 +35,15 @@
 #define DG_NW_BIG 512u
 #define DG_REDO 0xFFFFFFFFu
 
+template <typename CT>
+__device__ __forceinline__ void dg_store_run(const DgParams &p, CT *cell, const uint32_t run) {
+    if constexpr (sizeof(CT) == 1) {
+        if (run > 255u) { dg_fail(p, DG_E_RUN_WIDE); return; }
+    }
+    *cell = (CT)run;
+}
+
+template <typename CT>
 __device__ inline void dg_finish_alignment(const DgParams &p, uint32_t a, uint16_t *buf, uint32_t m) {
     const uint32_t trim = p.trim;
     uint32_t lbases = 0, rbases = 0, lo = 0, hi = m;
@@ -48,13 +57,13 @@
     start += lbases;
     const bool graph = !(p.flags & DG_F_A1_ONLY);
     uint32_t t_idx = 0, r = 0;
-    uint32_t *Cm = nullptr;
+    CT *Cm = nullptr;
     if (graph) {
         t_idx = p.aln_tgt[a];
         if (p.tactive[t_idx]) {
             const uint64_t ab = p.aln_begin[t_idx];
             r = (uint32_t)(a - ab);
-            Cm = p.matC + p.matc_base[t_idx] + (uint64_t)r * p.matc_stride[t_idx];
+            Cm = static_cast<CT *>(p.matC) + p.matc_base[t_idx] + (uint64_t)r * p.matc_stride[t_idx];
         }
     }
     const uint32_t tlen = graph ? p.tlen[t_idx] : 0xFFFFFFFFu;
@@ -67,7 +76,7 @@
         if (qb_ == tb_ || qb_ == DG_GAP) {                                                \
             if (Cm && conf && ((start + adv) & ((1u << p.emit_shift) - 1u)) == 0 && start + adv <= tlen + 1) \
                 ck[(start + adv) >> p.emit_shift] = ci_ - run;                            \
-            if (run) { if (Cm && conf && start + adv <= tlen + 1) Cm[start + adv] = run; run = 0; } \
+            if (run) { if (Cm && conf && start + adv <= tlen + 1) dg_store_run(p, Cm + (start + adv), run); run = 0; } \
             adv++; n_del += (qb_ != tb_);                                                 \
             if ((uint64_t)start - 1 + adv > (uint64_t)tlen) conf = false;                 \
         } else if (tb_ == DG_GAP) { n_ins++; run++; }                                     \
@@ -88,7 +97,7 @@
     while (i < hi) { const uint16_t c = buf[i]; DG_FIN_COL(c, i); i++; }
     if (run && Cm && conf && ((start + adv) & ((1u << p.emit_shift) - 1u)) == 0 && start + adv <= tlen + 1)
         ck[(start + adv) >> p.emit_shift] = hi - run;
-    if (run && Cm && conf && start + adv <= tlen + 1) Cm[start + adv] = run;
+    if (run && Cm && conf && start + adv <= tlen + 1) dg_store_run(p, Cm + (start + adv), run);
 #undef DG_FIN_COL
     p.n_lo[a] = lo; p.n_hi[a] = hi; p.n_start[a] = start;
     p.n_ins[a] = n_ins; p.n_del[a] = n_del;
@@ -345,6 +354,7 @@
     return (uint32_t)incl - v;
 }
 
+template <typename CT>
 __global__ __launch_bounds__(256) void k_norm_finish2(DgParams p) {
     const uint32_t g = blockIdx.x * 4u + (threadIdx.x >> 6);
     if (g >= p.n_chunks) return;
@@ -363,10 +373,10 @@
     uint16_t *dst = p.norm + p.norm_off[a] + o;
     const bool graph = !(p.flags & DG_F_A1_ONLY);
     uint32_t t_idx = 0;
-    uint32_t *Cm = nullptr;
+    CT *Cm = nullptr;
     if (graph) {
         t_idx = p.aln_tgt[a];
-        if (p.tactive[t_idx]) Cm = p.matC + p.matc_base[t_idx] + (uint64_t)(a - p.aln_begin[t_idx]) * p.matc_stride[t_idx];
+        if (p.tactive[t_idx]) Cm = static_cast<CT *>(p.matC) + p.matc_base[t_idx] + (uint64_t)(a - p.aln_begin[t_idx]) * p.matc_stride[t_idx];
     }
     const uint32_t tlen = graph ? p.tlen[t_idx] : 0xFFFFFFFFu;
     uint32_t *ck = p.ckpt + p.ck_base[a];
@@ -427,7 +437,7 @@
                     const uint32_t x = 8u * vl + k;
                     if (conf && ((start + adv) & ck_mask) == 0 && start + adv <= tlen + 1 && !(x == 0 && o > lo))
                         ck[(start + adv) >> p.emit_shift] = o + x - run;
-                    if (run && conf && start + adv <= tlen + 1) Cm[start + adv] = run;
+                    if (run && conf && start + adv <= tlen + 1) dg_store_run(p, Cm + (start + adv), run);
                     run = 0;
                     adv++;
                 } else if ((insm >> k) & 1u) run++;
@@ -440,7 +450,7 @@
         if (lane == 0) {
             if (any && Cm && conf && ((start + adv) & ck_mask) == 0 && start + adv <= tlen + 1 && (o + f1 < hi || run))
                 ck[(start + adv) >> p.emit_shift] = o + f1 - run;
-            if (run && Cm && conf && start + adv <= tlen + 1) Cm[start + adv] = run;
+            if (run && Cm && conf && start + adv <= tlen + 1) dg_store_run(p, Cm + (start + adv), run);
             if (graph && any && !conf) dg_fail_aln(p, a, DG_E_NONCONF);
         }
     }
@@ -451,6 +461,7 @@
 #undef DG_FIN_CONF
 }
 
+template <typename CT>
 __global__ __launch_bounds__(64) void k_normalize_slow(DgParams p) {
     const uint32_t a = blockIdx.x * 64 + threadIdx.x;
     if (a >= p.A) return;
@@ -505,7 +516,7 @@
         }
         m = w;
     }
-    dg_finish_alignment(p, a, buf, m);
+    dg_finish_alignment<CT>(p, a, buf, m);
 }
 
 __device__ __forceinline__ uint32_t dg_pool_words(uint32_t tlen, uint32_t n_ins, uint32_t n_del,
@@ -621,7 +632,7 @@
     const int lane = threadIdx.x & 63, wave = threadIdx.x >> 6;
     const uint32_t blen = p.tlen[t];
     const uint32_t K = (uint32_t)(p.aln_begin[t + 1] - p.aln_begin[t]);
-    uint32_t *col0 = p.matC + p.matc_base[t];
+    uint32_t *col0 = static_cast<uint32_t *>(p.matC) + p.matc_base[t];
     const uint32_t cstride = p.matc_stride[t];
     uint32_t *gcount = p.gcount + p.bbv_base[t];
     const uint32_t pos0 = (blockIdx.y * 4 + wave) * 8u;
@@ -722,17 +733,32 @@
     return victim;
 }
 
+template <typename CT> struct DgGsum { static constexpr uint32_t PPT = sizeof(CT) == 1 ? 4u : 1u; };
+template <typename CT>
 __global__ __launch_bounds__(256) void k_gsum(DgParams p) {
     const uint32_t t = blockIdx.x;
     if (dg_failed(p) || dg_tskip(p, t)) return;
-    const uint32_t pos = blockIdx.y * 256u + threadIdx.x;
-    if (pos >= p.tlen[t] + 2u) return;
+    const uint32_t pos = (blockIdx.y * 256u + threadIdx.x) * DgGsum<CT>::PPT;
+    const uint32_t np = p.tlen[t] + 2u;
+    if (pos >= np) return;
     const uint32_t K = (uint32_t)(p.aln_begin[t + 1] - p.aln_begin[t]);
-    const uint32_t *col = p.matC + p.matc_base[t] + pos;
+    const CT *col = static_cast<const CT *>(p.matC) + p.matc_base[t] + pos;
     const uint32_t stride = p.matc_stride[t];
-    uint32_t sum = 0;
-    for (uint32_t r = 0; r < K; r++) sum += col[(uint64_t)r * stride];
-    p.gcount[p.bbv_base[t] + pos] = sum;
+    uint32_t *gc = p.gcount + p.bbv_base[t] + pos;
+    if constexpr (sizeof(CT) == 1) {
+        uint32_t even = 0, odd = 0;
+        for (uint32_t r = 0; r < K; r++) {
+            const uint32_t w = *reinterpret_cast<const uint32_t *>(col + (uint64_t)r * stride);
+            even += w & 0x00FF00FFu; odd += (w >> 8) & 0x00FF00FFu;
+        }
+        const uint32_t s[4] = {even & 0xFFFFu, odd & 0xFFFFu, even >> 16, odd >> 16};
+        if (pos + 3u < np) *reinterpret_cast<uint4 *>(gc) = make_uint4(s[0], s[1], s[2], s[3]);
+        else for (uint32_t j = 0; pos + j < np; j++) gc[j] = s[j];
+    } else {
+        uint32_t sum = 0;
+        for (uint32_t r = 0; r < K; r++) sum += col[(uint64_t)r * stride];
+        *gc = sum;
+    }
 }
 
 #ifndef DG_EB
@@ -746,7 +772,9 @@
 #define DG_ECOLS_STRIDE 42u
 #define DG_ENEED 16u
 #endif
+template <typename CT>
 __global__ __launch_bounds__(64) void k_emit(DgParams p) {
+    static_assert(sizeof(CT) == 4 || DG_EB == 8, "a batch of byte cells is one 8-byte load");
     __shared__ uint32_t s_D[DG_EB * 64];
     __shared__ uint16_t s_col[64 * DG_ECOLS_STRIDE];
     if (dg_failed(p)) return;
@@ -768,7 +796,7 @@
     const uint32_t *bid = p.bid + bv, *gbase = p.gbase + bv;
     uint32_t *Am = p.matA + p.mat_base[t];
     uint32_t *Dm = p.matD + p.mat_base[t];
-    const uint32_t *Cm = p.matC + p.matc_base[t] + (uint64_t)(idle ? 0 : r) * p.matc_stride[t];
+    const CT *Cm = static_cast<const CT *>(p.matC) + p.matc_base[t] + (uint64_t)(idle ? 0 : r) * p.matc_stride[t];
     uint32_t *pool = p.pool + p.pool_base[t];
     DgNode *ndt = p.nodes + nb;
 #define DG_EPW(OFF) (*reinterpret_cast<uint32_t *>(reinterpret_cast<char *>(pool) + (((uint32_t)(OFF)) << 2)))
@@ -868,11 +896,17 @@
                 const uint4 v = gp[k];
                 gbv[4 * k] = v.x; gbv[4 * k + 1] = v.y; gbv[4 * k + 2] = v.z; gbv[4 * k + 3] = v.w;
             }
-            const uint4 *cp = reinterpret_cast<const uint4 *>(Cm + pos0);
-#pragma unroll
-            for (int k = 0; k < DG_EB / 4; k++) {
-                const uint4 v = cp[k];
-                cmv[4 * k] = v.x; cmv[4 * k + 1] = v.y; cmv[4 * k + 2] = v.z; cmv[4 * k + 3] = v.w;
+            if constexpr (sizeof(CT) == 1) {
+                const uint2 v = *reinterpret_cast<const uint2 *>(Cm + pos0);
+#pragma unroll
+                for (int k = 0; k < 8; k++) cmv[k] = ((k < 4 ? v.x : v.y) >> (8 * (k & 3))) & 0xFFu;
+            } else {
+                const uint4 *cp = reinterpret_cast<const uint4 *>(Cm + pos0);
+#pragma unroll
+                for (int k = 0; k < DG_EB / 4; k++) {
+                    const uint4 v = cp[k];
+                    cmv[4 * k] = v.x; cmv[4 * k + 1] = v.y; cmv[4 * k + 2] = v.z; cmv[4 * k + 3] = v.w;
+                }
             }
         }
         if (p.emit_scan) {
```

Measured after the change: 349.5 million, median of 6. +3.0%, better.
